# HengyiWang/spann3r

Measured on AMD Instinct MI355X. Metric: frames/sec/GPU (224px, 10-frame seq) + mem-bank cross-attn HBM GB/s, higher is better.
Workload: dtype bf16

## Files before the change

include/spann3r_hip.h:

```cpp
#ifndef SPANN3R_HIP_H
#define SPANN3R_HIP_H

#include <stdint.h>

#ifdef __cplusplus
extern "C" {
#endif

enum { SP3_F32 = 0, SP3_BF16 = 1 };
enum { SP3_ACT_NONE = 0, SP3_ACT_GELU = 1, SP3_ACT_RELU = 2 };
enum { SP3_EPI_PLAIN = 0, SP3_EPI_ROPE_VT = 1, SP3_EPI_PIXSHUF = 2, SP3_EPI_PARTIAL = 3 };
enum { SP3_LOAD_PLAIN = 0, SP3_LOAD_CONV3X3 = 1, SP3_LOAD_SOFTMAX = 2 };

const char* sp3_last_error(void);
int sp3_version(void);

typedef struct sp3_gemm_desc {
  const float* A;
  const float* A2;
  const void* W;
  void* C;
  const float* bias;
  const float* res1;
  const float* res2;
// ... 1 lines not shown
  int32_t batch;
  int32_t K1;
  int64_t lda, lda2, ldw, ldc, ldr1, ldr2;
  int64_t strideA, strideW, strideC;
  float alpha;
  int32_t wdtype;
  int32_t act;
  int32_t out_bf16;
  int32_t relu_in;
  int32_t loader;
  int32_t conv_H, conv_W, conv_C, conv_OH, conv_OW, conv_stride;
  int32_t epi;
  const float* rope_cos;
  const float* rope_sin;
  const int32_t* pos;
  int32_t rope_cols;
  void* vt;
  int32_t tokens;
  int32_t heads;
  int64_t vt_ld;
  int32_t ps_k, ps_H, ps_W, ps_C;
  int32_t tile;
  int32_t a_bf16;
  int32_t splitk;
  int32_t a_packed;
  const float* ln_stats;
  const float* ln_s;
  int32_t ln_nt;
  int32_t ln_C;
  float ln_eps;
  float* stats_out;
  void* c2;
  int32_t qkv_packed;
  int32_t out_packed;
  int32_t w_packed;
  int64_t sb_A2, sb_bias, sb_ln_stats, sb_ln_s, sb_stats_out, sb_c2, sb_vt;
  int64_t* trace;
  float* sm_stats_out;
  const float* sm_stats;
  int32_t sm_nt;
  float sm_thresh;
  float* sm_zout;
  int32_t f32x3;
  int32_t res_bf16;
  const int32_t* dyn_n;
  int32_t res2_up_H, res2_up_W;
} sp3_gemm_desc;
int sp3_gemm(const sp3_gemm_desc* desc_host, void* stream);
int sp3_gemm_n(const sp3_gemm_desc* const* descs, int n, void* stream);
int sp3_gemm_plan_n(const sp3_gemm_desc* const* descs, int n, int* tiles);
int sp3_gemm_plan(const sp3_gemm_desc* desc_host);

int sp3_layernorm(const float* x, int64_t ldx, const float* gamma, const float* beta, float eps,
                  void* out, int64_t ldo, int out_bf16, int rows, int C, void* stream);
int sp3_layernorm_packed(const float* x, int64_t ldx, const float* gamma, const float* beta, float eps,
                         void* out, int out_bf16, int rows, int C, void* stream);
int sp3_layernorm_dual(const float* x, int64_t ldx, const float* gamma, const float* beta, float eps, float* out, int64_t ldo,
                       void* out_packed_bf16, int rows, int C, int group_rows, int group_rows_pad, void* stream);
int sp3_layernorm_t(const float* x, int64_t ldx, const float* gamma, const float* beta, float eps,
                    void* out, int64_t ldo, int out_bf16, int rows, int C, void* stream);

typedef struct sp3_reduce_ln_desc {
  const float* partial;
  int64_t split_stride;
  const float* bias;
  const float* res;
  int64_t ldres;
  float* x_out;
  int64_t ldx;
  const float* g1; const float* b1; void* out1; int64_t ld1; int32_t out1_bf16;
  const float* g2; const float* b2; void* out2; int64_t ld2; int32_t out2_bf16;
  float eps;
  int32_t splits, rows, C;
  int32_t out1_packed, out2_packed;
  int32_t act;
  const float* res2;
  int64_t ldres2;
} sp3_reduce_ln_desc;
int sp3_reduce_ln(const sp3_reduce_ln_desc* desc_host, void* stream);

int sp3_rope_2d(void* tokens, int dtype, int B, int N, int H, int D, int64_t sB, int64_t sN, int64_t sH,
                const int64_t* positions, float base, float fwd, void* stream);

int sp3_attention(const void* q, int64_t sq, int64_t ldq, const void* k, int64_t sk, int64_t ldk,
                  const void* vt, int64_t vt_ld, void* out, int64_t ldo, int out_bf16,
                  int B, int heads, int Nq, int Nk, float scale, int dtype, void* stream);
int sp3_attention_ex(const void* q, int64_t sq, int64_t ldq, const void* k, int64_t sk, int64_t ldk,
                     const void* vt, int64_t vt_ld, void* out, int64_t ldo, int out_bf16, int out_packed,
                     int B, int heads, int Nq, int Nk, float scale, int dtype, void* stream);

int sp3_attention_packed(const void* qp, int q_cols, int q_col0, int npad_q, const void* kp, int k_cols, int k_col0, int npad_k,
                         const void* vtp, void* out, int64_t ldo, int out_bf16, int out_packed,
                         int B, int heads, int Nq, int Nk, float scale, int o_group, int o_group_rows, void* stream);

typedef struct sp3_attn_qproj_desc {
  const void* x_packed; int64_t x_group_stride;
  const float* ln_stats; int64_t stats_group_stride;
  const void* w_packed; int64_t w_group_stride;
  const float* ln_s; const float* bias; int64_t vec_group_stride;
  const int32_t* pos; const float* rope_cos; const float* rope_sin;
  float ln_eps; int32_t D;
  const void* kp; int32_t k_cols, k_col0, npad_k; const void* vtp;
  void* out; int64_t ldo; int32_t out_bf16, out_packed;
  int32_t B, heads, Nq, Nk; float scale; int32_t o_group, o_group_rows;
} sp3_attn_qproj_desc;
int sp3_attention_packed_qproj(const sp3_attn_qproj_desc* desc_host, void* stream);

typedef struct sp3_bank_write_desc {
  const float* feat_k;
  const float* feat_v;
  float* k_raw;
  float* v_raw;
  void* k_hat;
  void* v_hat_t;
  float* s_bank;
  float* b_bank;
  const float *gamma_k, *beta_k, *gamma_v, *beta_v, *gamma_q, *beta_q;
  float eps;
  float alpha;
  int32_t M, P, C, cap;
  int32_t wdtype;
  const int32_t* state;
} sp3_bank_write_desc;
int sp3_bank_write(const sp3_bank_write_desc* desc_host, void* stream);
int sp3_softmax_thresh(const float* S, float* P, int64_t ld, int64_t strideS, int rows, int M, int Mpad,
                       float thresh, int batch, void* P_packed, int64_t stride_packed, int packed_bf16, void* stream);
int sp3_softmax_pack(const float* S, int64_t ld, int64_t strideS, int rows, int M, float thresh, int batch, void* P_packed,
                     int64_t stride_packed, int packed_bf16, float* rowstat_ws, void* stream);
int sp3_colsum_accum(const float* P, int64_t ld, int rows, int M, float* mem_attn, void* stream);
int sp3_colsum_packed(const void* P_packed, int packed_bf16, int rows, int M, float* mem_attn, void* stream);
int sp3_colsum_softmax(const float* S, int64_t ld, int rows, int M, const float* rowz, float thresh, float* mem_attn,
                       float* mem_count, int append_P, void* stream);
int sp3_pack_stats(const float* x, int64_t ldx, int rows, int C, void* packed, int packed_bf16, float* stats, void* stream);
int sp3_gather_packed_rows(const void* src, void* dst, const int32_t* sel, int n_sel, int C, int elem_size, void* stream);
int sp3_gather_packed_cols(const void* src, void* dst, const int32_t* sel, int n_sel, int n_fill, int C, int cap,
                           int elem_size, void* stream);
int sp3_cos_sim(const float* k, const float* wm, int T, int P, int C, float* scratch, float* score, void* stream);
int sp3_bank_state_set(int32_t* state, int M, int wm, void* stream);
int sp3_prob_merge(const float* stats, float* scale, int rows, int M, int cap, const int32_t* dyn_n, void* stream);
int sp3_colsum_prob(const void* P_packed, const float* scale, int rows, int M, int cap, const int32_t* dyn_n, float* mem_attn, void* stream);
int sp3_cos_sim_state(const float* k, const float* k_raw, int Tmax, int P, int C, const int32_t* state, float* scratch, float* score,
                      void* stream);
int sp3_mem_append(float* count, float* attn, int M, int P, void* stream);
int sp3_prune_select(const float* attn, const float* count, int M, float protect, int top_k,
                     int32_t* sel, void* stream);
int sp3_gather_rows(const void* src, void* dst, const int32_t* sel, int n_sel, int C, int elem_size, void* stream);
int sp3_gather_cols(const void* src, int64_t ld_src, void* dst, int64_t ld_dst, const int32_t* sel, int n_sel,
                    int n_fill, int C, int elem_size, void* stream);
int sp3_gather_1d(const float* src, float* dst, const int32_t* sel, int n_sel, void* stream);

int sp3_conv3x3_tile(const void* x, int in_bf16, const void* w_packed, const float* bias, const float* res1,
                     const float* res2, void* out, int out_bf16, int B, int H, int W, int Cin, int Cout,
                     int relu_in, int act, void* stream);
int sp3_im2col_patch(const float* img, int64_t sb, int64_t sc, int64_t sy, int64_t sx, int B, int C, int H, int W,
                     int p, void* out, int out_bf16, int out_packed, void* stream);
int sp3_upsample2x(const float* in, float* out, int B, int H, int W, int C, int outH, int outW, void* stream);
int sp3_upsample2x_bf16(const void* in, void* out, int B, int H, int W, int C, int outH, int outW, void* stream);
int sp3_head_final(const float* feat, const float* w, const float* b, int64_t pixels, int C, float* pts,
                   float* conf, float* raw, void* stream);
int sp3_head_final_bf16(const void* feat, const float* w, const float* b, int64_t pixels, int C, float* pts, float* conf,
                        float* raw, void* stream);

int sp3_preprocess_image(const uint8_t* src, int64_t src_row_stride, int crop_l, int crop_t, int H1, int W1,
                         const int32_t* hbounds, const int32_t* hcoef, int hksize, int W2,
                         const int32_t* vbounds, const int32_t* vcoef, int vksize, int H2,
                         int crop2_l, int crop2_t, int outW, int outH, int transpose, uint8_t* tmp, float* out, void* stream);

int64_t sp3_conf_loss_ws_bytes(int n, int B);
int sp3_conf_loss_forward(const float* P, const float* Cf, const float* G, const uint8_t* V, const float* pose0, int n, int B, int HW,
                          float alpha, int fix_first, void* ws, float* out7, float* ent_out, void* stream);
int sp3_conf_loss_backward(const float* P, const float* Cf, const float* G, const uint8_t* V, const float* pose0, int n, int B, int HW,
                           float alpha, int fix_first, const void* ws, const float* grad_scale2, float* dP, float* dC, void* stream);
int64_t sp3_ssi_loss_ws_bytes(int n, int B, int HW);
int sp3_ssi_loss_forward(const float* P, const float* G, const uint8_t* V, const float* pose0, int n, int B, int HW, int fix_first,
                         int gt_scale, void* ws, float* out, void* stream);

int sp3_transpose(const float* src, int64_t ld_src, float* dst, int64_t ld_dst, int rows, int cols, void* stream);
int sp3_transpose_batched(const float* src, int64_t ld_src, int64_t stride_src, float* dst, int64_t ld_dst, int64_t stride_dst, int rows,
                          int cols, int batch, void* stream);
int sp3_transpose_pad(const float* src, int64_t ld_src, int64_t stride_src, float* dst, int64_t ld_dst, int64_t stride_dst, int rows,
                      int cols, int batch, int pad_to, void* stream);
int sp3_gelu(const float* x, float* y, int64_t n, void* stream);
int sp3_gelu_bwd(const float* x, const float* dy, float* dx, int64_t n, void* stream);
int sp3_im2col3x3(const float* x, float* col, int B, int H, int W, int C, int stride, void* stream);
int sp3_col2im3x3(const float* dcol, float* dx, int B, int H, int W, int C, int stride, void* stream);
int sp3_relu(const float* x, float* y, int64_t n, void* stream);
int sp3_relu_bwd(const float* x, const float* dy, float* dx, int64_t n, void* stream);
int sp3_upsample2x_bwd(const float* dy, float* dx, int B, int H, int W, int C, int outH, int outW, void* stream);
int sp3_postprocess(const float* raw, float* pts, float* conf, int64_t M, void* stream);
int sp3_postprocess_bwd(const float* raw, const float* dpts, const float* dconf, float* draw, int64_t M, void* stream);
int sp3_adamw(float* p, const float* g, float* m, float* v, int64_t n, float lr, float beta1, float beta2, float eps, float weight_decay,
              int step, float grad_scale, void* stream);
int sp3_mul(const float* a, const float* b, float* out, int64_t n, void* stream);
int sp3_pack_bf16(const float* src, int64_t ld, int rows, int cols, void* dst, void* dstT, void* stream);
int sp3_pack_bf16_conv3x3(const float* x, int B, int H, int W, int C, int stride, int act, void* dst, void* dstT, void* stream);
int sp3_pack_bf16_act(const float* src, int64_t ld, int rows, int cols, void* dst, void* dstT, int act, void* stream);
int sp3_pack_bf16_colsum(const float* src, int64_t ld, int rows, int cols, void* dst, void* dstT, float* colsum, int accumulate,
                         float* partial_ws, void* stream);
int64_t sp3_sumsq_blocks(int64_t n);
int64_t sp3_colsum_rows_ws(int rows, int N);
int sp3_colsum_rows(const float* x, int64_t ld, int rows, int N, float* out, int accumulate, float* scratch, void* stream);
int sp3_sumsq_partial(const float* g, int64_t n, double* partial, void* stream);
int sp3_clip_coef(const double* partial, int count, float max_norm, float extra_scale, float* out, int* step_counter, void* stream);
int sp3_adamw_flat(float* p, const float* g, float* m, float* v, int64_t n, const float* chunk_table, float lr, float beta1, float beta2,
                   float eps, int step, const float* grad_scale_dev, float grad_scale, const int* step_dev, const float* lr_dev, void* stream);
int sp3_softmax_bwd(const float* A, const float* dAd, const float* mask, float* dS, int64_t ld, int rows, int T, float alpha, void* stream);
int sp3_softmax_bwd_pad(const float* A, const float* dAd, const float* mask, float* dS, int64_t ld, int rows, int T, int Tpad, float alpha,
                        void* stream);
typedef struct sp3_head_part {
  const float* src;
  int64_t s_b, s_n, s_h;
  float* dst;
  int64_t d_b, d_n, d_h;
  float* dstT;
  const int64_t* pos;
  int32_t N;
  float fwd;
  int64_t ldT;
} sp3_head_part;
int sp3_head_shuffle(const sp3_head_part* parts, int nparts, int B, int H, int hd, float rope_base, const float* cos_tab,
                     const float* sin_tab, int tab_len, void* stream);
int sp3_attention_train_fwd(const float* q, int64_t sq, int64_t ldq, const float* k, int64_t sk, int64_t ldk, const float* vt, int64_t vt_ld,
                            float* out, int64_t ldo, float* lse, int B, int heads, int Nq, int Nk, float scale, int bf16_products, void* stream);
typedef struct sp3_attn_bwd_desc {
  const float *q, *k, *v, *dout;
  int64_t sq, ldq, sk, ldk, sv, ldv, sdo, lddo;
  const float *qT, *kT, *doT;
  int64_t ldTq, ldTk;
  const float* lse;
  float* D;
  float *dq, *dk, *dv;
  int64_t sdq, lddq, sdk, lddk, sdv, lddv;
  int32_t B, heads, Nq, Nk;
  float scale;
  int32_t bf16_products;
} sp3_attn_bwd_desc;
int sp3_attention_train_bwd(const sp3_attn_bwd_desc* d, void* stream);
int sp3_layernorm_bwd(const float* x, int64_t ldx, const float* gamma, const float* dy, int64_t ldy, const float* dx_add, int64_t ld_add,
                      float* dx, int64_t ld_dx, float* dgamma, float* dbeta, int accumulate, float* scratch, int rows, int C, float eps,
                      void* stream);

int sp3_focal_weiszfeld(const float* pts3d, int B, int H, int W, float ppx, float ppy, int iters, float focal_min, float focal_max,
                        float* focal, void* stream);
int sp3_conf_filter(const float* conf, const float* pts, const float* rgb, int64_t n, float thresh, int* scratch, int64_t* total,
                    float* out_pts, float* out_rgb, void* stream);

int sp3_pnp_dlt_accum(const float* pts, int F, int H, int W, float focal, float cx, float cy, const float* norm4, const float* Rt,
                      float thresh, int cv_mode, double* out41, void* stream);
int sp3_pnp_gn_accum(const float* pts, int F, int H, int W, float focal, float cx, float cy, const double* Rt, const float* Rt_mask,
                     float thresh, double* out29, void* stream);
int sp3_pnp_score(const float* pts, int F, int H, int W, float focal, float cx, float cy, const float* Rt, int n_hyp, float thresh,
                  int cv_mode, int* counts, void* stream);

int sp3_copy_multi(int n, const void* const* src, void* const* dst, const int64_t* bytes, void* stream);
int sp3_copy2d_f32(const float* src, int64_t lds, float* dst, int64_t ldd, int rows, int cols, void* stream);
int sp3_fill_f32(float* p, float v, int64_t n, void* stream);
int sp3_cast_f32_to_bf16(const float* src, void* dst, int64_t n, void* stream);
int sp3_spin(int64_t cycles, int64_t* ticks_100mhz, void* stream);

#ifdef __cplusplus
}
#endif
#endif
```

spann3r_amd/csrc/common.h:

```cpp
#pragma once
#include <hip/hip_runtime.h>
#include <stdint.h>
#include <stdio.h>
#include "../../include/spann3r_hip.h"

typedef __attribute__((ext_vector_type(8))) __bf16 bf16x8;
typedef __attribute__((ext_vector_type(4))) __bf16 bf16x4;
typedef __attribute__((ext_vector_type(2))) __bf16 bf16x2;
typedef __attribute__((ext_vector_type(4))) float f32x4;

#define SP3_WAVE 64

void sp3_set_error(const char* fmt, ...);

#define SP3_CHECK(cond, ...)                     \
  do {                                           \
    if (!(cond)) {                               \
      sp3_set_error(__VA_ARGS__);                \
      return 1;                                  \
    }                                            \
  } while (0)

#define SP3_LAUNCH_CHECK(what)                                              \
  do {                                                                      \
    hipError_t e_ = hipGetLastError();                                      \
    if (e_ != hipSuccess) {                                                 \
      sp3_set_error("%s: launch failed: %s", what, hipGetErrorString(e_));  \
      return 2;                                                             \
    }                                                                       \
  } while (0)

__device__ __forceinline__ float wave_sum(float v) {
#pragma unroll
  for (int o = 32; o > 0; o >>= 1) v += __shfl_xor(v, o);
  return v;
}
__device__ __forceinline__ float wave_max(float v) {
#pragma unroll
  for (int o = 32; o > 0; o >>= 1) v = fmaxf(v, __shfl_xor(v, o));
  return v;
}

__device__ __forceinline__ bf16x8 cvt8(const float4 a, const float4 b) {
  bf16x8 r;
  r[0] = (__bf16)a.x; r[1] = (__bf16)a.y; r[2] = (__bf16)a.z; r[3] = (__bf16)a.w;
  r[4] = (__bf16)b.x; r[5] = (__bf16)b.y; r[6] = (__bf16)b.z; r[7] = (__bf16)b.w;
  return r;
}

__device__ __forceinline__ float4 relu4(float4 v) {
  v.x = fmaxf(v.x, 0.f); v.y = fmaxf(v.y, 0.f); v.z = fmaxf(v.z, 0.f); v.w = fmaxf(v.w, 0.f);
  return v;
}

__device__ __forceinline__ float gelu_erf(float x) {
  const float a = fabsf(x);
  const float t = __builtin_amdgcn_rcpf(fmaf(0.2316419f, a, 1.0f));
  float p = fmaf(1.330274429f, t, -1.821255978f);
  p = fmaf(p, t, 1.781477937f);
  p = fmaf(p, t, -0.356563782f);
  p = fmaf(p, t, 0.319381530f);
  const float e = __builtin_amdgcn_exp2f(-0.72134752044448170368f * a * a);
  const float q = (p * t) * (e * 0.3989422804014327f);
  return fmaf(-a, q, fmaxf(x, 0.f));
}

#ifndef SP3_NO_WT_STORES
__device__ __forceinline__ void st_out(bf16x4* p, bf16x4 v) {
  __hip_atomic_store(reinterpret_cast<unsigned long long*>(p), __builtin_bit_cast(unsigned long long, v), __ATOMIC_RELAXED, __HIP_MEMORY_SCOPE_AGENT);
}
__device__ __forceinline__ void st_out(float2* p, float2 v) {
  __hip_atomic_store(reinterpret_cast<unsigned long long*>(p), __builtin_bit_cast(unsigned long long, v), __ATOMIC_RELAXED, __HIP_MEMORY_SCOPE_AGENT);
}
__device__ __forceinline__ void st_out(float4* p, float4 v) {
  const f32x4 t = {v.x, v.y, v.z, v.w};
  asm volatile("global_store_dwordx4 %0, %1, off sc1\n\ts_nop 1" ::"v"(p), "v"(t) : "memory");
}
__device__ __forceinline__ void st_out(bf16x8* p, bf16x8 v) {
  asm volatile("global_store_dwordx4 %0, %1, off sc1\n\ts_nop 1" ::"v"(p), "v"(v) : "memory");
}
#else
template <typename T> __device__ __forceinline__ void st_out(T* p, T v) { *p = v; }
#endif

struct Up2xTaps {
  int p00, p01, p10, p11;
  float hy, ly, hx, lx;
};
__device__ __forceinline__ Up2xTaps up2x_taps(int H, int W, int oy, int ox) {
  const int OH = 2 * H, OW = 2 * W;
  const float sh = OH > 1 ? (float)(H - 1) / (float)(OH - 1) : 0.f;
  const float sw = OW > 1 ? (float)(W - 1) / (float)(OW - 1) : 0.f;
  int y0 = (int)__fmul_rn(sh, (float)oy), x0 = (int)__fmul_rn(sw, (float)ox);
  y0 = y0 < H - 1 ? y0 : H - 1;
  x0 = x0 < W - 1 ? x0 : W - 1;
  const int y1 = y0 < H - 1 ? y0 + 1 : y0, x1 = x0 < W - 1 ? x0 + 1 : x0;
  Up2xTaps t;
  t.ly = __fmaf_rn(sh, (float)oy, -(float)y0); t.lx = __fmaf_rn(sw, (float)ox, -(float)x0);
  t.hy = 1.f - t.ly; t.hx = 1.f - t.lx;
  t.p00 = y0 * W + x0; t.p01 = y0 * W + x1; t.p10 = y1 * W + x0; t.p11 = y1 * W + x1;
  return t;
}
__device__ __forceinline__ float up2x_mix(const Up2xTaps& t, float v00, float v01, float v10, float v11) {
  const float top = __fmaf_rn(t.hx, v00, __fmul_rn(t.lx, v01)), bot = __fmaf_rn(t.hx, v10, __fmul_rn(t.lx, v11));
  return __fmaf_rn(t.hy, top, __fmul_rn(t.ly, bot));
}

__device__ __forceinline__ int64_t packed_off(int row, int k, int K, bool bf16) {
  const int lkb = bf16 ? 6 : 5, lch = bf16 ? 4 : 3;
  const int nkb = (K + (1 << lkb) - 1) >> lkb;
  const int kb = k >> lkb, kk = k & ((1 << lkb) - 1);
  const int g = kk >> lch, e = kk & ((1 << lch) - 1);
  const int h = e >> (lch - 1), eh = e & ((1 << (lch - 1)) - 1);
  return (((((int64_t)(row >> 4) * nkb + kb) * 2 + h) * 4 + g) * 16 + (row & 15)) * (1 << (lch - 1)) + eh;
}
```

spann3r_amd/csrc/conv.hip:

```cpp
#include "common.h"
#include <type_traits>
#include <cstdlib>

namespace {

constexpr int TH = 8, TW = 8;
constexpr int HP = (TH + 2) * (TW + 2);
constexpr int BM = TH * TW, BN = 64;
constexpr int MF = BM / 16, NF = BN / 16;
constexpr int SLAB_LD = BN + 4;
constexpr int DEPTH = 3;
constexpr int SP3_CONV_WIDE_MIN_WGS = 256;

struct ConvArgs {
  const void* x; const __bf16* w; const float* bias; const float* res1; const float* res2; void* out;
  int B, H, W, Cin, Cout, tiles_x, tiles_y, relu_in, act, out_bf16;
  int xcd_nb;
};

__device__ __forceinline__ bool conv_tile_of(const ConvArgs& a, int& t, int& nblk) {
  t = blockIdx.x; nblk = blockIdx.y;
  if (a.xcd_nb) {
    const unsigned L = blockIdx.x, xc = L & 7, jj = L >> 3, q = jj / (unsigned)a.xcd_nb;
    nblk = (int)(jj - q * a.xcd_nb);
    t = (int)(q * 8 + xc);
    if (t >= a.tiles_x * a.tiles_y * a.B) return false;
  }
  return true;
}

__device__ __forceinline__ bf16x8 ld_frag_lds(const char* p) { return *reinterpret_cast<const bf16x8*>(p); }

template <typename TIN>
__global__ __launch_bounds__(256) void conv3x3_tile_kernel(const ConvArgs a) {
  extern __shared__ __attribute__((aligned(16))) char lds[];
  const int tid = threadIdx.x, lane = tid & 63, wave = tid >> 6, g = lane >> 4, r = lane & 15;
  const int Cin = a.Cin;
  const int PS = Cin * 2 + 16;
  int t, nblk;
  if (!conv_tile_of(a, t, nblk)) return;
  const int tx = t % a.tiles_x; t /= a.tiles_x;
  const int ty = t % a.tiles_y;
  const int b = t / a.tiles_y;
  const int y0 = ty * TH, x0 = tx * TW, n0 = nblk * BN;

  const int upt = Cin >> 5;
  const int U = 9 * upt;
  const int nkb = (9 * Cin) >> 6;
  const __bf16* wb[NF];
#pragma unroll
  for (int n = 0; n < NF; ++n) wb[n] = a.w + ((int64_t)((n0 >> 4) + n) * nkb * 128 + lane) * 8;
  const int nu = (U - wave + 3) >> 2;
  auto w_off = [&](int i) -> int64_t {
    int u = wave + 4 * i;
    u = u < U ? u : U - 1;
    return (int64_t)(u >> 1) * (64 * 16) + (u & 1) * (64 * 8);
  };
  bf16x8 wq[DEPTH][NF];
#pragma unroll
  for (int s = 0; s < DEPTH; ++s) {
    const int64_t o = w_off(s);
#pragma unroll
    for (int n = 0; n < NF; ++n) wq[s][n] = *reinterpret_cast<const bf16x8*>(wb[n] + o);
  }

  {
    constexpr int CHK = 16 / (int)sizeof(TIN);
    const int cpp = Cin / CHK;
    const TIN* xin = reinterpret_cast<const TIN*>(a.x) + (int64_t)b * a.H * a.W * Cin;
    using Chunk = typename std::conditional<sizeof(TIN) == 4, float4, bf16x8>::type;
    auto src_of = [&](int p, int c, bool& ok) -> const Chunk* {
      const int hy = p / (TW + 2), hx = p - hy * (TW + 2);
      const int iy = y0 + hy - 1, ix = x0 + hx - 1;
      ok = p < HP && iy >= 0 && iy < a.H && ix >= 0 && ix < a.W;
      const int cy = ok ? iy : 0, cx = ok ? ix : 0;
      return reinterpret_cast<const Chunk*>(xin + ((int64_t)cy * a.W + cx) * Cin + c);
    };
    auto put = [&](int p, int c, Chunk v, bool ok) {
      char* dst = lds + p * PS + c * 2;
      if constexpr (sizeof(TIN) == 4) {
        if (!ok) v = make_float4(0.f, 0.f, 0.f, 0.f);
        if (a.relu_in) v = relu4(v);
        bf16x4 o;
        o[0] = (__bf16)v.x; o[1] = (__bf16)v.y; o[2] = (__bf16)v.z; o[3] = (__bf16)v.w;
        *reinterpret_cast<bf16x4*>(dst) = o;
      } else {
#pragma unroll
        for (int e = 0; e < 8; ++e) {
          const float f = (float)v[e];
          v[e] = (ok && (!a.relu_in || f > 0.f)) ? v[e] : (__bf16)0.f;
        }
        *reinterpret_cast<bf16x8*>(dst) = v;
      }
    };
    if ((256 % cpp) == 0) {
      const int c = (tid % cpp) * CHK, pstep = 256 / cpp;
      constexpr int NB = 13;
      for (int p0 = tid / cpp; p0 < HP; p0 += NB * pstep) {
        Chunk buf[NB];
        bool ok[NB];
#pragma unroll
        for (int q = 0; q < NB; ++q) buf[q] = *src_of(p0 + q * pstep, c, ok[q]);
#pragma unroll
        for (int q = 0; q < NB; ++q)
          if (p0 + q * pstep < HP) put(p0 + q * pstep, c, buf[q], ok[q]);
      }
    } else {
      for (int i = tid; i < HP * cpp; i += 256) {
        const int p = i / cpp, c = (i - p * cpp) * CHK;
        bool ok;
        const Chunk v = *src_of(p, c, ok);
        put(p, c, v, ok);
      }
    }
  }
  __syncthreads();

  f32x4 acc[MF][NF];
#pragma unroll
  for (int m = 0; m < MF; ++m)
#pragma unroll
    for (int n = 0; n < NF; ++n) acc[m][n] = f32x4{0.f, 0.f, 0.f, 0.f};
  int abase[MF];
#pragma unroll
  for (int m = 0; m < MF; ++m) {
    const int p = 16 * m + r;
    abase[m] = ((p / TW) * (TW + 2) + (p % TW)) * PS;
  }
  auto a_off = [&](int i) -> int {
    int u = wave + 4 * i;
    u = u < U ? u : U - 1;
    const int tap = u / upt, c32 = u - tap * upt;
    const int ky = tap / 3, kx = tap - 3 * ky;
    return (ky * (TW + 2) + kx) * PS + (((c32 >> 1) << 6) + 16 * g + ((c32 & 1) << 3)) * 2;
  };
  bf16x8 af[2][MF];
  {
    const int o = a_off(0);
#pragma unroll
    for (int m = 0; m < MF; ++m) af[0][m] = ld_frag_lds(lds + abase[m] + o);
  }
  for (int i0 = 0; i0 < nu; i0 += 2 * DEPTH) {
#pragma unroll
    for (int s2 = 0; s2 < 2 * DEPTH; ++s2) {
      const int i = i0 + s2;
      if (i < nu) {
        const int s = s2 % DEPTH, cur = s2 & 1;
        {
          const int o = a_off(i + 1);
#pragma unroll
          for (int m = 0; m < MF; ++m) af[cur ^ 1][m] = ld_frag_lds(lds + abase[m] + o);
        }
#pragma unroll
        for (int m = 0; m < MF; ++m)
#pragma unroll
          for (int n = 0; n < NF; ++n)
            acc[m][n] = __builtin_amdgcn_mfma_f32_16x16x32_bf16(af[cur][m], wq[s][n], acc[m][n], 0, 0, 0);
        {
          const int64_t o = w_off(i + DEPTH);
#pragma unroll
          for (int n = 0; n < NF; ++n) wq[s][n] = *reinterpret_cast<const bf16x8*>(wb[n] + o);
        }
      }
    }
  }
  __syncthreads();

  float* slab = reinterpret_cast<float*>(lds) + (size_t)wave * BM * SLAB_LD;
#pragma unroll
  for (int m = 0; m < MF; ++m)
#pragma unroll
    for (int n = 0; n < NF; ++n)
#pragma unroll
      for (int q = 0; q < 4; ++q) slab[(m * 16 + 4 * g + q) * SLAB_LD + n * 16 + r] = acc[m][n][q];
  __syncthreads();
  const float* sm = reinterpret_cast<const float*>(lds);
  for (int idx = tid; idx < BM * (BN / 4); idx += 256) {
    const int row = idx / (BN / 4), c4 = (idx % (BN / 4)) * 4;
    const int oy = y0 + row / TW, ox = x0 + row % TW;
    if (oy >= a.H || ox >= a.W) continue;
    float4 v = *reinterpret_cast<const float4*>(sm + row * SLAB_LD + c4);
#pragma unroll
    for (int s = 1; s < 4; ++s) {
      const float4 t4 = *reinterpret_cast<const float4*>(sm + (size_t)s * BM * SLAB_LD + row * SLAB_LD + c4);
      v.x += t4.x; v.y += t4.y; v.z += t4.z; v.w += t4.w;
    }
    const int gn = n0 + c4;
    if (a.bias) { const float4 b4 = *reinterpret_cast<const float4*>(a.bias + gn); v.x += b4.x; v.y += b4.y; v.z += b4.z; v.w += b4.w; }
    if (a.act == SP3_ACT_RELU) v = relu4(v);
    const int64_t off = (((int64_t)b * a.H + oy) * a.W + ox) * a.Cout + gn;
    if (a.out_bf16 & 2) {
      if (a.res1) { const bf16x4 q = *reinterpret_cast<const bf16x4*>(reinterpret_cast<const __bf16*>(a.res1) + off); v.x += (float)q[0]; v.y += (float)q[1]; v.z += (float)q[2]; v.w += (float)q[3]; }
      if (a.res2) { const bf16x4 q = *reinterpret_cast<const bf16x4*>(reinterpret_cast<const __bf16*>(a.res2) + off); v.x += (float)q[0]; v.y += (float)q[1]; v.z += (float)q[2]; v.w += (float)q[3]; }
    } else {
      if (a.res1) { const float4 q = *reinterpret_cast<const float4*>(a.res1 + off); v.x += q.x; v.y += q.y; v.z += q.z; v.w += q.w; }
      if (a.res2) { const float4 q = *reinterpret_cast<const float4*>(a.res2 + off); v.x += q.x; v.y += q.y; v.z += q.z; v.w += q.w; }
    }
    if (a.out_bf16 & 1) {
      bf16x4 o;
      o[0] = (__bf16)v.x; o[1] = (__bf16)v.y; o[2] = (__bf16)v.z; o[3] = (__bf16)v.w;
      st_out(reinterpret_cast<bf16x4*>(reinterpret_cast<__bf16*>(a.out) + off), o);
    } else {
      st_out(reinterpret_cast<float4*>(reinterpret_cast<float*>(a.out) + off), v);
    }
  }
}

namespace wide {
constexpr int TH = 8, TW = 16, HW = TW + 2, HP = (TH + 2) * HW;
constexpr int CH = 128, PS = CH * 2 + 16;
constexpr int MF = 8, DEPTH = 3;
constexpr int HALO_BYTES = HP * PS;
template <int NF> constexpr int lds_bytes() {
  return HALO_BYTES > 4 * 64 * (16 * NF + 4) * 4 ? HALO_BYTES : 4 * 64 * (16 * NF + 4) * 4;
}

template <typename TIN, int NF = 4, int ABL = 0>
__global__ __launch_bounds__(256, 2) void conv3x3_wide_kernel(const ConvArgs a) {
  constexpr int BN = 16 * NF, SLAB_LD = BN + 4;
  extern __shared__ __attribute__((aligned(16))) char lds[];
  const int tid = threadIdx.x, lane = tid & 63, wave = tid >> 6, g = lane >> 4, r = lane & 15;
  const int Cin = a.Cin;
  int t, nblk;
  if (!conv_tile_of(a, t, nblk)) return;
  const int tx = t % a.tiles_x; t /= a.tiles_x;
  const int ty = t % a.tiles_y;
  const int b = t / a.tiles_y;
  const int y0 = ty * TH, x0 = tx * TW, n0 = nblk * BN;
  const int nchunk = Cin / CH, upt = Cin >> 5;
  const int total = 9 * nchunk;

  typedef __attribute__((ext_vector_type(4))) uint32_t u32x4;
  const int nkb = (9 * Cin) >> 6;
  const uint32_t panel_bytes = (uint32_t)nkb * 128 * 8 * 2;
  const auto wrsrc = __builtin_amdgcn_make_buffer_rsrc(
      const_cast<char*>(reinterpret_cast<const char*>(a.w)) + (int64_t)(n0 >> 4) * panel_bytes, 0, (int)(NF * panel_bytes), 0x00020000);
  const uint32_t wlane = (uint32_t)lane * 16 + (uint32_t)(wave & 1) * 1024;
  const int wave_u = __builtin_amdgcn_readfirstlane(wave);
  auto w_off = [&](int seq) -> uint32_t {
    seq = seq < total ? seq : total - 1;
    const int c = seq / 9, tap = seq - 9 * c;
    return (uint32_t)((tap * upt + 4 * c + wave_u) >> 1) * 2048;
  };
  auto w_load = [&](int seq, bf16x8* dst) {
    const uint32_t o = w_off(seq);
#pragma unroll
    for (int n = 0; n < NF; ++n) {
      const u32x4 v = __builtin_amdgcn_raw_buffer_load_b128(wrsrc, wlane, o + n * panel_bytes, 0);
      dst[n] = *reinterpret_cast<const bf16x8*>(&v);
    }
  };
  bf16x8 wq[DEPTH][NF];
#pragma unroll
  for (int s = 0; s < DEPTH; ++s) w_load(s, wq[s]);

  f32x4 acc[MF][NF];
#pragma unroll
  for (int m = 0; m < MF; ++m)
#pragma unroll
    for (int n = 0; n < NF; ++n) acc[m][n] = f32x4{0.f, 0.f, 0.f, 0.f};
  const char* abase = lds + r * PS + (((wave >> 1) << 6) + 16 * g + ((wave & 1) << 3)) * 2;

  constexpr int CHK = 16 / (int)sizeof(TIN);
  constexpr int CPP = CH / CHK;
  constexpr int PSTEP = 256 / CPP, NB = sizeof(TIN) == 4 ? 6 : 12;
  const uint32_t img_bytes = (uint32_t)(a.H * a.W * Cin) * (uint32_t)sizeof(TIN);
  const auto rsrc = __builtin_amdgcn_make_buffer_rsrc(
      const_cast<char*>(reinterpret_cast<const char*>(a.x)) + (int64_t)b * img_bytes, 0, (int)img_bytes, 0x00020000);
  const uint32_t xlane = (uint32_t)((tid % CPP) * CHK * sizeof(TIN));
  char* hdst = lds + (tid % CPP) * CHK * 2;

  u32x4 buf[NB];
  auto issue = [&](int c, int p0) {
#pragma unroll
    for (int q = 0; q < NB; ++q) {
      const int p = p0 + q * PSTEP;
      const int hy = p / HW, hx = p - hy * HW;
      const int iy = y0 + hy - 1, ix = x0 + hx - 1;
      const bool ok = p < HP && iy >= 0 && iy < a.H && ix >= 0 && ix < a.W;
      const uint32_t off = ok ? (uint32_t)((iy * a.W + ix) * Cin + c * CH) * (uint32_t)sizeof(TIN) + xlane : 0x80000000u;
      if constexpr (ABL & 4) buf[q] = u32x4{0u, 0u, 0u, 0u};
      else buf[q] = __builtin_amdgcn_raw_buffer_load_b128(rsrc, off, 0, 0);
    }
  };
  auto commit = [&](int p0) {
#pragma unroll
    for (int q = 0; q < NB; ++q) {
      const int p = p0 + q * PSTEP;
      if (p >= HP) continue;
      char* dst = hdst + p * PS;
      if constexpr (sizeof(TIN) == 4) {
        float4 v = make_float4(__uint_as_float(buf[q][0]), __uint_as_float(buf[q][1]), __uint_as_float(buf[q][2]), __uint_as_float(buf[q][3]));
        if (a.relu_in) v = relu4(v);
        bf16x4 o;
        o[0] = (__bf16)v.x; o[1] = (__bf16)v.y; o[2] = (__bf16)v.z; o[3] = (__bf16)v.w;
        *reinterpret_cast<bf16x4*>(dst) = o;
      } else {
        u32x4 v = buf[q];
        if (a.relu_in) {
#pragma unroll
          for (int e = 0; e < 4; ++e) {
            const uint32_t neg = v[e] & 0x80008000u;
            v[e] &= ~((neg >> 15) * 0xffffu);
          }
        }
        *reinterpret_cast<u32x4*>(dst) = v;
      }
    }
  };
  for (int c = 0; c < nchunk; ++c) {
    if (c) __syncthreads();
    for (int p0 = tid / CPP; p0 < HP; p0 += NB * PSTEP) {
      issue(c, p0);
      commit(p0);
    }
    __syncthreads();

    bf16x8 af[MF];
#pragma unroll
    for (int m = 0; m < MF; ++m) af[m] = ld_frag_lds(abase + m * HW * PS);
#pragma unroll
    for (int tap = 0; tap < 9; ++tap) {
      const int s = tap % DEPTH;
      const int nt = tap + 1, nky = nt / 3, nkx = nt - 3 * nky;
#pragma unroll
      for (int m = 0; m < MF; ++m) {
#pragma unroll
        for (int n = 0; n < NF; ++n)
          acc[m][n] = __builtin_amdgcn_mfma_f32_16x16x32_bf16(af[m], wq[s][n], acc[m][n], 0, 0, 0);
        if constexpr (!(ABL & 2))
          if (tap < 8) af[m] = ld_frag_lds(abase + ((m + nky) * HW + nkx) * PS);
      }
      if constexpr (!(ABL & 1)) w_load(9 * c + tap + DEPTH, wq[s]);
    }
  }

  float* slab = reinterpret_cast<float*>(lds) + (size_t)wave * 64 * SLAB_LD;
  const float* sm = reinterpret_cast<const float*>(lds);
  if constexpr (ABL & 8) {
    float sum = 0.f;
#pragma unroll
    for (int m = 0; m < MF; ++m)
#pragma unroll
      for (int n = 0; n < NF; ++n) sum += acc[m][n][0] + acc[m][n][1] + acc[m][n][2] + acc[m][n][3];
    if (sum == 12345.678f) reinterpret_cast<float*>(a.out)[tid] = sum;
    return;
  }
#pragma unroll
  for (int h = 0; h < 2; ++h) {
    __syncthreads();
#pragma unroll
    for (int m = 0; m < 4; ++m)
#pragma unroll
      for (int n = 0; n < NF; ++n)
#pragma unroll
        for (int q = 0; q < 4; ++q) slab[(m * 16 + 4 * g + q) * SLAB_LD + n * 16 + r] = acc[4 * h + m][n][q];
    __syncthreads();
    for (int idx = tid; idx < 64 * (BN / 4); idx += 256) {
      const int row = idx / (BN / 4), c4 = (idx % (BN / 4)) * 4;
      const int oy = y0 + 4 * h + (row >> 4), ox = x0 + (row & 15);
      if (oy >= a.H || ox >= a.W) continue;
      float4 v = *reinterpret_cast<const float4*>(sm + row * SLAB_LD + c4);
#pragma unroll
      for (int s = 1; s < 4; ++s) {
        const float4 t4 = *reinterpret_cast<const float4*>(sm + (size_t)s * 64 * SLAB_LD + row * SLAB_LD + c4);
        v.x += t4.x; v.y += t4.y; v.z += t4.z; v.w += t4.w;
      }
      const int gn = n0 + c4;
      if (a.bias) { const float4 b4 = *reinterpret_cast<const float4*>(a.bias + gn); v.x += b4.x; v.y += b4.y; v.z += b4.z; v.w += b4.w; }
      if (a.act == SP3_ACT_RELU) v = relu4(v);
      const int64_t off = (((int64_t)b * a.H + oy) * a.W + ox) * a.Cout + gn;
      if (a.out_bf16 & 2) {
        if (a.res1) { const bf16x4 q = *reinterpret_cast<const bf16x4*>(reinterpret_cast<const __bf16*>(a.res1) + off); v.x += (float)q[0]; v.y += (float)q[1]; v.z += (float)q[2]; v.w += (float)q[3]; }
        if (a.res2) { const bf16x4 q = *reinterpret_cast<const bf16x4*>(reinterpret_cast<const __bf16*>(a.res2) + off); v.x += (float)q[0]; v.y += (float)q[1]; v.z += (float)q[2]; v.w += (float)q[3]; }
      } else {
        if (a.res1) { const float4 q = *reinterpret_cast<const float4*>(a.res1 + off); v.x += q.x; v.y += q.y; v.z += q.z; v.w += q.w; }
        if (a.res2) { const float4 q = *reinterpret_cast<const float4*>(a.res2 + off); v.x += q.x; v.y += q.y; v.z += q.z; v.w += q.w; }
      }
      if (a.out_bf16 & 1) {
        bf16x4 o;
        o[0] = (__bf16)v.x; o[1] = (__bf16)v.y; o[2] = (__bf16)v.z; o[3] = (__bf16)v.w;
        st_out(reinterpret_cast<bf16x4*>(reinterpret_cast<__bf16*>(a.out) + off), o);
      } else {
        st_out(reinterpret_cast<float4*>(reinterpret_cast<float*>(a.out) + off), v);
      }
    }
  }
}
}

}

extern "C" int sp3_conv3x3_tile(const void* x, int in_bf16, const void* w_packed, const float* bias, const float* res1,
                                const float* res2, void* out, int out_bf16, int B, int H, int W, int Cin, int Cout,
                                int relu_in, int act, void* stream) {
  SP3_CHECK(x && w_packed && out, "sp3_conv3x3_tile: null pointer");
  SP3_CHECK(B > 0 && H > 0 && W > 0, "sp3_conv3x3_tile: bad shape");
  SP3_CHECK(Cin % 64 == 0 && Cin >= 64 && Cout % 64 == 0 && Cout >= 64, "sp3_conv3x3_tile: Cin=%d / Cout=%d must be multiples of 64", Cin, Cout);
  SP3_CHECK(act == SP3_ACT_NONE || act == SP3_ACT_RELU, "sp3_conv3x3_tile: act %d", act);
  auto al16 = [](const void* q) { return (reinterpret_cast<uintptr_t>(q) & 15) == 0; };
  SP3_CHECK(al16(x) && al16(w_packed) && al16(bias) && al16(res1) && al16(res2) && al16(out), "sp3_conv3x3_tile: 16-byte alignment");
  ConvArgs a;
  a.x = x; a.w = reinterpret_cast<const __bf16*>(w_packed); a.bias = bias; a.res1 = res1; a.res2 = res2; a.out = out;
  a.B = B; a.H = H; a.W = W; a.Cin = Cin; a.Cout = Cout;
  a.relu_in = relu_in; a.act = act; a.out_bf16 = out_bf16 & 3;
  a.xcd_nb = 0;
  constexpr bool xcd_on = true;
  hipStream_t st = reinterpret_cast<hipStream_t>(stream);
  {
    const int want = (out_bf16 >> 2) & 3;
    const int wtx = (W + wide::TW - 1) / wide::TW, wty = (H + wide::TH - 1) / wide::TH;
    const int64_t wgs = (int64_t)wtx * wty * B * (Cout / 64);
    const bool can = Cin % wide::CH == 0;
    SP3_CHECK(want < 2 || can, "sp3_conv3x3_tile: the 8 x 16 tile needs Cin %% 128 == 0 (Cin=%d)", Cin);
    SP3_CHECK((int64_t)H * W * Cin * (in_bf16 ? 2 : 4) < (1ll << 31), "sp3_conv3x3_tile: one image of the map must stay below 2 GiB");
    const int nf = want == 2 ? 4 : want == 3 ? 2 : (want == 0 && can) ? (wgs >= SP3_CONV_WIDE_MIN_WGS ? 4 : wgs >= 80 ? 2 : 0) : 0;
    if (nf) {
      a.tiles_x = wtx; a.tiles_y = wty;
      dim3 grid(wtx * wty * B, Cout / (16 * nf));
      if (xcd_on) { a.xcd_nb = Cout / (16 * nf); grid = dim3((unsigned)(((wtx * wty * B + 7) / 8) * 8 * a.xcd_nb), 1); }
      auto launch = [&](auto kern, int lds_bytes) -> int {
        static bool raised = false;
        if (!raised && lds_bytes > 64 * 1024) {
          hipError_t e = hipFuncSetAttribute(reinterpret_cast<const void*>(kern), hipFuncAttributeMaxDynamicSharedMemorySize, lds_bytes);
          if (e != hipSuccess) { sp3_set_error("sp3_conv3x3_tile: cannot raise dynamic LDS to %d: %s", lds_bytes, hipGetErrorString(e)); return 2; }
          raised = true;
        }
        hipLaunchKernelGGL(kern, grid, dim3(256), lds_bytes, st, a);
        return 0;
      };
      int rc;
      if (nf == 4) rc = in_bf16 ? launch(wide::conv3x3_wide_kernel<__bf16, 4>, wide::lds_bytes<4>()) : launch(wide::conv3x3_wide_kernel<float, 4>, wide::lds_bytes<4>());
      else         rc = in_bf16 ? launch(wide::conv3x3_wide_kernel<__bf16, 2>, wide::lds_bytes<2>()) : launch(wide::conv3x3_wide_kernel<float, 2>, wide::lds_bytes<2>());
      if (rc) return rc;
      SP3_LAUNCH_CHECK("sp3_conv3x3_tile");
      return 0;
    }
  }
  a.tiles_x = (W + TW - 1) / TW; a.tiles_y = (H + TH - 1) / TH;
  const size_t halo = (size_t)HP * (Cin * 2 + 16), slabs = (size_t)4 * BM * SLAB_LD * sizeof(float);
  const size_t lds = halo > slabs ? halo : slabs;
  SP3_CHECK(lds <= 160 * 1024, "sp3_conv3x3_tile: Cin=%d needs %zu bytes of LDS", Cin, lds);
  dim3 grid(a.tiles_x * a.tiles_y * B, Cout / BN);
  if (xcd_on) { a.xcd_nb = Cout / BN; grid = dim3((unsigned)(((a.tiles_x * a.tiles_y * B + 7) / 8) * 8 * a.xcd_nb), 1); }
  auto launch = [&](auto kern) -> int {
    static size_t raised = 0;
    if (lds > 64 * 1024 && lds > raised) {
      raised = lds;
      hipError_t e = hipFuncSetAttribute(reinterpret_cast<const void*>(kern), hipFuncAttributeMaxDynamicSharedMemorySize, (int)lds);
      if (e != hipSuccess) { sp3_set_error("sp3_conv3x3_tile: cannot raise dynamic LDS to %zu: %s", lds, hipGetErrorString(e)); return 2; }
    }
    hipLaunchKernelGGL(kern, grid, dim3(256), lds, st, a);
    return 0;
  };
  const int rc = in_bf16 ? launch(conv3x3_tile_kernel<__bf16>) : launch(conv3x3_tile_kernel<float>);
  if (rc) return rc;
  SP3_LAUNCH_CHECK("sp3_conv3x3_tile");
  return 0;
}
```

spann3r_amd/csrc/dpt.hip:

```cpp
#include "common.h"
#include <math.h>

namespace {

__global__ __launch_bounds__(256) void im2col_patch_kernel(const float* __restrict__ img, int64_t sb, int64_t sc, int64_t sy,
                                                           int64_t sx, int C, int H, int W, int p, void* __restrict__ out,
                                                           int out_bf16, int out_packed, int64_t total) {
  const int64_t idx = (int64_t)blockIdx.x * 256 + threadIdx.x;
  if (idx >= total) return;
  const int K = C * p * p;
  const int64_t row = idx / K;
  const int k = (int)(idx - row * K);
  const int nw = W / p, nh = H / p;
  const int b = (int)(row / (nh * nw));
  const int rem = (int)(row - (int64_t)b * nh * nw);
  const int ty = rem / nw, tx = rem - ty * nw;
  const int c = k / (p * p), r2 = k - c * p * p;
  const int iy = r2 / p, ix = r2 - iy * p;
  const float val = img[b * sb + c * sc + (int64_t)(ty * p + iy) * sy + (int64_t)(tx * p + ix) * sx];
  const int64_t o = out_packed ? packed_off((int)row, k, K, out_bf16 != 0) : idx;
  if (out_bf16) reinterpret_cast<__bf16*>(out)[o] = (__bf16)val;
  else reinterpret_cast<float*>(out)[o] = val;
}

__device__ __forceinline__ float4 ld4(const float* p) { return *reinterpret_cast<const float4*>(p); }
__device__ __forceinline__ float4 ld4(const __bf16* p) {
  const bf16x4 t = *reinterpret_cast<const bf16x4*>(p);
  return make_float4((float)t[0], (float)t[1], (float)t[2], (float)t[3]);
}
__device__ __forceinline__ void st4(float* p, const float4 v) { st_out(reinterpret_cast<float4*>(p), v); }
__device__ __forceinline__ void st4(__bf16* p, const float4 v) {
  bf16x4 t;
  t[0] = (__bf16)v.x; t[1] = (__bf16)v.y; t[2] = (__bf16)v.z; t[3] = (__bf16)v.w;
  st_out(reinterpret_cast<bf16x4*>(p), t);
}

template <typename T>
__global__ __launch_bounds__(256) void upsample2x_kernel(const T* __restrict__ in, T* __restrict__ out, int H, int W,
                                                         int C, int outH, int outW, int64_t total4) {
  const int64_t idx = (int64_t)blockIdx.x * 256 + threadIdx.x;
  if (idx >= total4) return;
  const int c4 = C >> 2;
  const int cc = (int)(idx % c4);
  int64_t pix = idx / c4;
  const int ox = (int)(pix % outW);
  pix /= outW;
  const int oy = (int)(pix % outH);
  const int b = (int)(pix / outH);
  const int OH = 2 * H, OW = 2 * W;
  const float sh = OH > 1 ? (float)(H - 1) / (float)(OH - 1) : 0.f;
  const float sw = OW > 1 ? (float)(W - 1) / (float)(OW - 1) : 0.f;
  const float fy = sh * (float)oy, fx = sw * (float)ox;
  int y0 = (int)fy, x0 = (int)fx;
  y0 = y0 < H - 1 ? y0 : H - 1;
  x0 = x0 < W - 1 ? x0 : W - 1;
  const int y1 = y0 < H - 1 ? y0 + 1 : y0, x1 = x0 < W - 1 ? x0 + 1 : x0;
  const float ly = fy - (float)y0, lx = fx - (float)x0;
  const float hy = 1.f - ly, hx = 1.f - lx;
  const T* base = in + (int64_t)b * H * W * C;
  const float4 v00 = ld4(base + (((int64_t)y0 * W + x0) * c4 + cc) * 4);
  const float4 v01 = ld4(base + (((int64_t)y0 * W + x1) * c4 + cc) * 4);
  const float4 v10 = ld4(base + (((int64_t)y1 * W + x0) * c4 + cc) * 4);
  const float4 v11 = ld4(base + (((int64_t)y1 * W + x1) * c4 + cc) * 4);
  float4 o;
  o.x = hy * (hx * v00.x + lx * v01.x) + ly * (hx * v10.x + lx * v11.x);
  o.y = hy * (hx * v00.y + lx * v01.y) + ly * (hx * v10.y + lx * v11.y);
  o.z = hy * (hx * v00.z + lx * v01.z) + ly * (hx * v10.z + lx * v11.z);
  o.w = hy * (hx * v00.w + lx * v01.w) + ly * (hx * v10.w + lx * v11.w);
  st4(out + idx * 4, o);
}

__global__ __launch_bounds__(256) void upsample2x_bf16x8_kernel(const __bf16* __restrict__ in, __bf16* __restrict__ out, int H, int W,
                                                                int C, int outH, int outW) {
  const int c8 = C >> 3;
  const int t = blockIdx.x * 256 + threadIdx.x;
  if (t >= outW * c8) return;
  const int ox = t / c8, cg = t - ox * c8;
  const int oy = blockIdx.y, b = blockIdx.z;
  const int OH = 2 * H, OW = 2 * W;
  const float sh = OH > 1 ? (float)(H - 1) / (float)(OH - 1) : 0.f;
  const float sw = OW > 1 ? (float)(W - 1) / (float)(OW - 1) : 0.f;
  const float fy = sh * (float)oy, fx = sw * (float)ox;
  int y0 = (int)fy, x0 = (int)fx;
  y0 = y0 < H - 1 ? y0 : H - 1;
  x0 = x0 < W - 1 ? x0 : W - 1;
  const int y1 = y0 < H - 1 ? y0 + 1 : y0, x1 = x0 < W - 1 ? x0 + 1 : x0;
  const float ly = fy - (float)y0, lx = fx - (float)x0;
  const float hy = 1.f - ly, hx = 1.f - lx;
  const __bf16* base = in + (int64_t)b * H * W * C + cg * 8;
  const bf16x8 v00 = *reinterpret_cast<const bf16x8*>(base + ((int64_t)y0 * W + x0) * C);
  const bf16x8 v01 = *reinterpret_cast<const bf16x8*>(base + ((int64_t)y0 * W + x1) * C);
  const bf16x8 v10 = *reinterpret_cast<const bf16x8*>(base + ((int64_t)y1 * W + x0) * C);
  const bf16x8 v11 = *reinterpret_cast<const bf16x8*>(base + ((int64_t)y1 * W + x1) * C);
  bf16x8 o;
#pragma unroll
  for (int e = 0; e < 8; ++e)
    o[e] = (__bf16)(hy * (hx * (float)v00[e] + lx * (float)v01[e]) + ly * (hx * (float)v10[e] + lx * (float)v11[e]));
  st_out(reinterpret_cast<bf16x8*>(out + (((int64_t)b * outH + oy) * outW + ox) * C + cg * 8), o);
}

template <typename T>
__global__ __launch_bounds__(256) void head_final_kernel(const T* __restrict__ feat, const float* __restrict__ w,
                                                         const float* __restrict__ bias, int64_t pixels, int C,
                                                         float* __restrict__ pts, float* __restrict__ conf,
                                                         float* __restrict__ raw) {
  const int64_t gid = (int64_t)blockIdx.x * 256 + threadIdx.x;
  const int64_t pix = gid >> 3;
  const int sub = (int)(gid & 7);
  const bool valid = pix < pixels;
  const int64_t pp = valid ? pix : pixels - 1;
  float a0 = 0.f, a1 = 0.f, a2 = 0.f, a3 = 0.f;
  const T* f = feat + pp * C;
  for (int c = sub * 4; c < C; c += 32) {
    const float4 x = ld4(f + c);
    const float4 w0 = *reinterpret_cast<const float4*>(w + c);
    const float4 w1 = *reinterpret_cast<const float4*>(w + C + c);
    const float4 w2 = *reinterpret_cast<const float4*>(w + 2 * C + c);
    const float4 w3 = *reinterpret_cast<const float4*>(w + 3 * C + c);
    a0 += (x.x * w0.x + x.y * w0.y) + (x.z * w0.z + x.w * w0.w);
    a1 += (x.x * w1.x + x.y * w1.y) + (x.z * w1.z + x.w * w1.w);
    a2 += (x.x * w2.x + x.y * w2.y) + (x.z * w2.z + x.w * w2.w);
    a3 += (x.x * w3.x + x.y * w3.y) + (x.z * w3.z + x.w * w3.w);
  }
#pragma unroll
  for (int o = 1; o < 8; o <<= 1) {
    a0 += __shfl_xor(a0, o); a1 += __shfl_xor(a1, o); a2 += __shfl_xor(a2, o); a3 += __shfl_xor(a3, o);
  }
  if (valid && sub == 0) {
    const float x = a0 + bias[0], y = a1 + bias[1], z = a2 + bias[2], c = a3 + bias[3];
    if (raw) { raw[pix * 4 + 0] = x; raw[pix * 4 + 1] = y; raw[pix * 4 + 2] = z; raw[pix * 4 + 3] = c; }
    const float d = sqrtf(x * x + y * y + z * z);
    const float sc = expm1f(d) / fmaxf(d, 1e-8f);
    pts[pix * 3 + 0] = x * sc; pts[pix * 3 + 1] = y * sc; pts[pix * 3 + 2] = z * sc;
    conf[pix] = 1.0f + expf(c);
  }
}

template <int LP, int PPT>
__global__ __launch_bounds__(256) void head_final_bf16x8_kernel(const __bf16* __restrict__ feat, const float* __restrict__ w,
                                                                const float* __restrict__ bias, int64_t pixels, float* __restrict__ pts,
                                                                float* __restrict__ conf, float* __restrict__ raw) {
  constexpr int C = 8 * LP, PPB = 256 / LP;
  const int li = threadIdx.x % LP, pl = threadIdx.x / LP;
  float wr[4][8];
#pragma unroll
  for (int f = 0; f < 4; ++f) {
    const float4 a = *reinterpret_cast<const float4*>(w + f * C + li * 8), b = *reinterpret_cast<const float4*>(w + f * C + li * 8 + 4);
    wr[f][0] = a.x; wr[f][1] = a.y; wr[f][2] = a.z; wr[f][3] = a.w; wr[f][4] = b.x; wr[f][5] = b.y; wr[f][6] = b.z; wr[f][7] = b.w;
  }
  const float b0 = bias[0], b1 = bias[1], b2 = bias[2], b3 = bias[3];
  const int64_t p0 = (int64_t)blockIdx.x * PPB * PPT + pl;
  bf16x8 x[PPT];
#pragma unroll
  for (int q = 0; q < PPT; ++q) {
    int64_t pix = p0 + (int64_t)q * PPB;
    pix = pix < pixels ? pix : pixels - 1;
    x[q] = *reinterpret_cast<const bf16x8*>(feat + pix * C + li * 8);
  }
#pragma unroll
  for (int q = 0; q < PPT; ++q) {
    const int64_t pix = p0 + (int64_t)q * PPB;
    float a[4];
#pragma unroll
    for (int f = 0; f < 4; ++f) {
      float t0 = 0.f, t1 = 0.f;
#pragma unroll
      for (int e = 0; e < 4; ++e) { t0 = fmaf((float)x[q][e], wr[f][e], t0); t1 = fmaf((float)x[q][4 + e], wr[f][4 + e], t1); }
      a[f] = t0 + t1;
    }
#pragma unroll
    for (int o = 1; o < LP; o <<= 1) {
      a[0] += __shfl_xor(a[0], o); a[1] += __shfl_xor(a[1], o); a[2] += __shfl_xor(a[2], o); a[3] += __shfl_xor(a[3], o);
    }
    if (li == 0 && pix < pixels) {
      const float X = a[0] + b0, Y = a[1] + b1, Z = a[2] + b2, Cc = a[3] + b3;
      if (raw) *reinterpret_cast<float4*>(raw + pix * 4) = make_float4(X, Y, Z, Cc);
      const float d = sqrtf(X * X + Y * Y + Z * Z);
      const float sc = expm1f(d) / fmaxf(d, 1e-8f);
      pts[pix * 3 + 0] = X * sc; pts[pix * 3 + 1] = Y * sc; pts[pix * 3 + 2] = Z * sc;
      conf[pix] = 1.0f + expf(Cc);
    }
  }
}

}

#define ST(s) reinterpret_cast<hipStream_t>(s)

extern "C" int sp3_im2col_patch(const float* img, int64_t sb, int64_t sc, int64_t sy, int64_t sx, int B, int C, int H, int W,
                                int p, void* out, int out_bf16, int out_packed, void* stream) {
  SP3_CHECK(img && out && B > 0 && C > 0 && p > 0, "sp3_im2col_patch: bad arguments");
  SP3_CHECK(H % p == 0 && W % p == 0, "Input image size (%d,%d) is not a multiple of patch size (%d)", H, W, p);
  const int64_t total = (int64_t)B * (H / p) * (W / p) * C * p * p;
  hipLaunchKernelGGL(im2col_patch_kernel, dim3((unsigned)((total + 255) / 256)), dim3(256), 0, ST(stream), img, sb, sc, sy, sx,
                     C, H, W, p, out, out_bf16, out_packed, total);
  SP3_LAUNCH_CHECK("sp3_im2col_patch");
  return 0;
}

extern "C" int sp3_upsample2x(const float* in, float* out, int B, int H, int W, int C, int outH, int outW, void* stream) {
  SP3_CHECK(in && out && B > 0 && H > 0 && W > 0 && C > 0 && C % 4 == 0, "sp3_upsample2x: bad arguments");
  SP3_CHECK(outH > 0 && outH <= 2 * H && outW > 0 && outW <= 2 * W, "sp3_upsample2x: bad crop");
  const int64_t total4 = (int64_t)B * outH * outW * (C / 4);
  hipLaunchKernelGGL(upsample2x_kernel<float>, dim3((unsigned)((total4 + 255) / 256)), dim3(256), 0, ST(stream), in, out, H, W, C,
                     outH, outW, total4);
  SP3_LAUNCH_CHECK("sp3_upsample2x");
  return 0;
}

extern "C" int sp3_upsample2x_bf16(const void* in, void* out, int B, int H, int W, int C, int outH, int outW, void* stream) {
  SP3_CHECK(in && out && B > 0 && H > 0 && W > 0 && C > 0 && C % 4 == 0, "sp3_upsample2x_bf16: bad arguments");
  SP3_CHECK(outH > 0 && outH <= 2 * H && outW > 0 && outW <= 2 * W, "sp3_upsample2x_bf16: bad crop");
  if (C % 8 == 0 && outH <= 65535 && B <= 65535) {
    hipLaunchKernelGGL(upsample2x_bf16x8_kernel, dim3((unsigned)((outW * (C / 8) + 255) / 256), outH, B), dim3(256), 0, ST(stream),
                       reinterpret_cast<const __bf16*>(in), reinterpret_cast<__bf16*>(out), H, W, C, outH, outW);
    SP3_LAUNCH_CHECK("sp3_upsample2x_bf16");
    return 0;
  }
  const int64_t total4 = (int64_t)B * outH * outW * (C / 4);
  hipLaunchKernelGGL(upsample2x_kernel<__bf16>, dim3((unsigned)((total4 + 255) / 256)), dim3(256), 0, ST(stream),
                     reinterpret_cast<const __bf16*>(in), reinterpret_cast<__bf16*>(out), H, W, C, outH, outW, total4);
  SP3_LAUNCH_CHECK("sp3_upsample2x_bf16");
  return 0;
}

extern "C" int sp3_head_final(const float* feat, const float* w, const float* b, int64_t pixels, int C, float* pts, float* conf,
                              float* raw, void* stream) {
  SP3_CHECK(feat && w && b && pts && conf && pixels > 0 && C > 0 && C % 32 == 0, "sp3_head_final: bad arguments");
  const int64_t threads = pixels * 8;
  hipLaunchKernelGGL(head_final_kernel<float>, dim3((unsigned)((threads + 255) / 256)), dim3(256), 0, ST(stream), feat, w, b, pixels, C,
                     pts, conf, raw);
  SP3_LAUNCH_CHECK("sp3_head_final");
  return 0;
}

extern "C" int sp3_head_final_bf16(const void* feat, const float* w, const float* b, int64_t pixels, int C, float* pts, float* conf,
                                   float* raw, void* stream) {
  SP3_CHECK(feat && w && b && pts && conf && pixels > 0 && C > 0 && C % 32 == 0, "sp3_head_final_bf16: bad arguments");
  if (C == 128 && (reinterpret_cast<uintptr_t>(feat) & 15) == 0 && (reinterpret_cast<uintptr_t>(w) & 15) == 0 && (!raw || (reinterpret_cast<uintptr_t>(raw) & 15) == 0)) {
    constexpr int LP = 16, PPT = 4, PPB = 256 / LP;
    hipLaunchKernelGGL((head_final_bf16x8_kernel<LP, PPT>), dim3((unsigned)((pixels + PPB * PPT - 1) / (PPB * PPT))), dim3(256), 0, ST(stream),
                       reinterpret_cast<const __bf16*>(feat), w, b, pixels, pts, conf, raw);
    SP3_LAUNCH_CHECK("sp3_head_final_bf16");
    return 0;
  }
  const int64_t threads = pixels * 8;
  hipLaunchKernelGGL(head_final_kernel<__bf16>, dim3((unsigned)((threads + 255) / 256)), dim3(256), 0, ST(stream),
                     reinterpret_cast<const __bf16*>(feat), w, b, pixels, C, pts, conf, raw);
  SP3_LAUNCH_CHECK("sp3_head_final_bf16");
  return 0;
}
```

spann3r_amd/engine.py:

```python
import math
import os

import torch

from . import ops
from .lib import ACT_NONE, ACT_GELU, ACT_RELU
from .config import Spann3RConfig


def _rope_tables(max_pos, base, device):
    half = 32
    inv_freq = 1.0 / (base ** (torch.arange(0, half, 2).float() / half))
    t = torch.arange(max_pos, dtype=torch.float32)
    ang = torch.einsum("i,j->ij", t, inv_freq)
    return ang.cos().contiguous().to(device), ang.sin().contiguous().to(device)


def _rope_tables_narrow(max_pos, base, head_dim, device):
    D = head_dim // 2
    nf = D // 2
    assert nf <= 16 and head_dim % 4 == 0
    inv_freq = 1.0 / (base ** (torch.arange(0, D, 2).float() / D))
    t = torch.arange(max_pos, dtype=torch.float32)
    ang = torch.einsum("i,j->ij", t, inv_freq)
# ... 416 lines not shown
    def decoder_grouped(self, f1, f2, B, nh, nw, f1p=None, f2p=None):
        self.activate()
        cfg, w = self.cfg, self.w
        E, D, Hh = cfg.enc_dim, cfg.dec_dim, cfg.dec_heads
        P = nh * nw
        R = B * P
        npad = (P + 63) // 64 * 64
        nt = D // 32
        pos = self.positions(B, nh, nw)[1]
        depth = cfg.dec_depth
        es = 2 if self.adt == torch.bfloat16 else 4
        x = [self.ws("decg_x%d" % l, (2, R, D)) for l in range(depth + 1)]
        xp = [self.wspg("decg_xp%d" % j, R, D) for j in (0, 1)]
        st = [self.ws("decg_st%d" % j, (2, R, nt, 2)) for j in (0, 1)]
        xq, stq = self.wspg("decg_xq", R, D), self.ws("decg_stq", (2, R, nt, 2))
        ao, h = self.wspg("decg_ao", R, D), self.wspg("decg_h", R, D * cfg.mlp_ratio)
        qkp = self.ws("decg_qkp", ops.packed_shape(2 * B * npad, 2 * D, self.wdt), self.wdt, zero=True)
        vtp = self.ws("decg_vtp", (2 * B * Hh * npad * 64,), self.wdt, zero=True)
        cqp = self.ws("decg_cqp", ops.packed_shape(2 * B * npad, D, self.wdt), self.wdt, zero=True)
        ckp = self.ws("decg_ckp", ops.packed_shape(2 * B * npad, D, self.wdt), self.wdt, zero=True)
        cvtp = self.ws("decg_cvtp", (2 * B * Hh * npad * 64,), self.wdt, zero=True)
        sb_st, sb_vt = R * nt * 8, B * Hh * npad * 64 * 2
        Rp = xp[0].rows_pad
        if f1p is not None and f2p is not None:
            dA = f2p.data_ptr() - f1p.data_ptr()
            assert dA % 16 == 0
            ops.gemm(f1p, w["dec_embed.w"], x[0], M=R, N=D, K=E, lda=E, ldc=D, bias=w["dec_embed.b"], stats_out=st[0], c2=xp[0],
                     batch=2, strideA=dA // 2, strideC=R * D, sb={"stats_out": sb_st, "c2": xp[0].stride * es})
        else:
            dA = f2.data_ptr() - f1.data_ptr()
            assert dA % 16 == 0 and f1.dtype == f2.dtype == torch.float32
            ops.gemm(f1, w["dec_embed.w"], x[0], M=R, N=D, K=E, lda=E, ldc=D, bias=w["dec_embed.b"], stats_out=st[0], c2=xp[0],
                     batch=2, strideA=dA // 4, strideC=R * D, sb={"stats_out": sb_st, "c2": xp[0].stride * es})
        rope = dict(pos=pos, cos=self.cos, sin=self.sin, tokens=P, heads=Hh, qkv_packed=True, batch=2)
        for i in range(depth):
            cur, nx = i % 2, (i + 1) % 2
            g = "decg_%d." % i
            last = i == depth - 1
            xi, xo = x[i], x[i + 1]

            def upd(A, K, pre, res, stats, c2):
                sb = {"bias": D * 4}
                if stats is not None:
                    sb["stats_out"], sb["c2"] = sb_st, c2.stride * es
                ops.gemm(A, w[g + pre + ".w"], xo, M=R, N=D, K=K, lda=K, ldc=D, bias=w[g + pre + ".b"], res1=res, ldr1=D,
                         stats_out=stats, c2=c2, batch=2, strideA=A.stride, strideW=w[g + pre + ".w"].stride, strideC=R * D, sb=sb)

            with ops.pair():
                ops.proj_rope_vt(xp[cur], w[g + "qkv.w"], w[g + "qkv.b"], qkp, 0, vtp, npad, M=R, N=3 * D, K=D, lda=D, rope_cols=2 * D,
                                 ln=ops.LnFold(st[cur], D, w[g + "qkv.s"], 1e-6, sb_stats=sb_st, sb_s=3 * D * 4),
                                 strideA=xp[cur].stride, strideW=w[g + "qkv.w"].stride, strideC=B * npad * 2 * D,
                                 sb={"bias": 3 * D * 4, "vt": sb_vt}, **rope)
                ops.proj_rope_vt(xp[cur].at(1), w[g + "ckv.w"], w[g + "ckv.b"], ckp, 0, cvtp, npad, M=R, N=2 * D, K=D, lda=D, rope_cols=D,
                                 ln=ops.LnFold(st[cur][1], D, w[g + "ckv.s"], 1e-6, sb_stats=-sb_st, sb_s=2 * D * 4),
                                 strideA=-xp[cur].stride, strideW=w[g + "ckv.w"].stride, strideC=B * npad * D,
                                 sb={"bias": 2 * D * 4, "vt": sb_vt}, **rope)
            ops.attention_packed(qkp, 2 * D, 0, npad, qkp, 2 * D, D, npad, vtp, ao, D, B=2 * B, heads=Hh, Nq=P, Nk=P,
                                 scale=64 ** -0.5, o_group=B, o_group_rows=Rp)
            upd(ao, D, "proj", xi, stq, xq)
            if self.fuse_cross_q and P < 512 and D == 768 and ops.LEAN:
                ops.attention_packed_qproj(xq, stq, w[g + "cq.w"], w[g + "cq.s"], w[g + "cq.b"], pos, self.cos, self.sin, ckp, D, 0, npad, cvtp,
                                           ao, D, B=2 * B, heads=Hh, Nq=P, Nk=P, scale=64 ** -0.5, o_group=B, o_group_rows=Rp, eps=1e-6,
                                           stats_group_stride=sb_st // 4, vec_group_stride=D)
            else:
                ops.proj_rope_vt(xq, w[g + "cq.w"], w[g + "cq.b"], cqp, 0, None, npad, M=R, N=D, K=D, lda=D, rope_cols=D,
                                 ln=ops.LnFold(stq, D, w[g + "cq.s"], 1e-6, sb_stats=sb_st, sb_s=D * 4),
                                 strideA=xq.stride, strideW=w[g + "cq.w"].stride, strideC=B * npad * D, sb={"bias": D * 4}, **rope)
                ops.attention_packed(cqp, D, 0, npad, ckp, D, 0, npad, cvtp, ao, D, B=2 * B, heads=Hh, Nq=P, Nk=P,
                                     scale=64 ** -0.5, o_group=B, o_group_rows=Rp)
            upd(ao, D, "cproj", xo, stq, xq)
            Hd = D * cfg.mlp_ratio
            ops.gemm(xq, w[g + "fc1.w"], h, M=R, N=Hd, K=D, lda=D, ldc=Hd, bias=w[g + "fc1.b"], act=ACT_GELU,
                     ln=ops.LnFold(stq, D, w[g + "fc1.s"], 1e-6, sb_stats=sb_st, sb_s=Hd * 4),
                     batch=2, strideA=xq.stride, strideW=w[g + "fc1.w"].stride, strideC=h.stride, sb={"bias": Hd * 4})
            if last:
                upd(h, Hd, "fc2", xo, None, None)
            else:
                upd(h, Hd, "fc2", xo, st[nx], xp[nx])
        normed = self.ws("decg_normed", (2, R, D))
        ops.layernorm(x[depth], w["dec_norm.w"], w["dec_norm.b"], 1e-6, normed, rows=2 * R, C_=D,
                      dual=self.wspg("decg_normed_packed", R, D) if self.adt == torch.bfloat16 else None, group_rows=R)
        outs = {}
        for s_ in (0, 1):
            outs[s_] = [(f1, f2)[s_]] + [x[l][s_].view(B, P, D) for l in range(1, depth)] + [normed[s_].view(B, P, D)]
        return outs[0], outs[1]

    def key_aux(self, R):
        E = self.cfg.enc_dim
        return self.wspg("keyg_packed", R, E), self.ws("keyg_stats", (2, R, E // 32, 2))

    def encode_feat_keys_grouped(self, feat1, feat2, normed1, normed2, R, out1, out2, feat1p=None, feat2p=None):
        self.activate()
        cfg, w = self.cfg, self.w
        E, D, Kd = cfg.enc_dim, cfg.dec_dim, cfg.key_dim
        dF, dN, dO = feat2.data_ptr() - feat1.data_ptr(), normed2.data_ptr() - normed1.data_ptr(), out2.data_ptr() - out1.data_ptr()
        assert dF % 16 == 0 and dN % 16 == 0 and dO % 16 == 0
        es = 2 if self.adt == torch.bfloat16 else 4
        h = self.wspg("keyg_hidden", R, Kd)
        packed = None
        if feat1p is not None and feat2p is not None and self.adt == torch.bfloat16 and ops.LEAN:
            np_ = self.wspg("decg_normed_packed", R, D)
            dFp = feat2p.data_ptr() - feat1p.data_ptr()
            assert dFp % 16 == 0
            packed = dict(A2=np_, lda2=D, K1=E, batch=2, strideA=dFp // 2, strideW=w["keyg.0.w"].stride, strideC=h.stride,
                          sb={"bias": Kd * 4, "A2": np_.stride * 2})
            ok = self._splitA_plan.get(R)
            if ok is None:
                ok = self._splitA_plan[R] = ops.gemm(feat1p, w["keyg.0.w"], h, M=R, N=Kd, K=Kd, lda=E, ldc=Kd, bias=w["keyg.0.b"],
                                                     act=ACT_GELU, plan_only=True, **packed) >= 30
            if not ok:
                packed = None
        if packed is not None:
            ops.gemm(feat1p, w["keyg.0.w"], h, M=R, N=Kd, K=Kd, lda=E, ldc=Kd, bias=w["keyg.0.b"], act=ACT_GELU, **packed)
        else:
            ops.gemm(feat1, w["keyg.0.w"], h, M=R, N=Kd, K=Kd, lda=E, ldc=Kd, bias=w["keyg.0.b"], act=ACT_GELU, A2=normed1, lda2=D, K1=E,
                     batch=2, strideA=dF // 4, strideW=w["keyg.0.w"].stride, strideC=h.stride, sb={"bias": Kd * 4, "A2": dN})
        kp, kst = self.key_aux(R)
        ops.gemm(h, w["keyg.2.w"], out1, M=R, N=E, K=Kd, lda=Kd, ldc=E, bias=w["keyg.2.b"], stats_out=kst, c2=kp,
                 batch=2, strideA=h.stride, strideW=w["keyg.2.w"].stride, strideC=dO // 4,
                 sb={"bias": E * 4, "stats_out": R * (E // 32) * 8, "c2": kp.stride * es})
        return kp.at(1), kst[1]

    def encode_feat_key(self, feat, dec_last, R, num, out, aux=False):
        self.activate()
        cfg, w = self.cfg, self.w
        E, D, Kd = cfg.enc_dim, cfg.dec_dim, cfg.key_dim
        h = self.wsp("key_hidden%d" % num, R, Kd)
        pre = "key%d." % num
        ops.gemm(feat, w[pre + "0.w"], h, M=R, N=Kd, K=Kd, lda=E, ldc=Kd, bias=w[pre + "0.b"], act=ACT_GELU,
                 A2=dec_last, lda2=D, K1=E)
        if aux:
            kp, kst = self.key_aux(R)
            ops.gemm(h, w[pre + "2.w"], out, M=R, N=E, K=Kd, lda=Kd, ldc=E, bias=w[pre + "2.b"], stats_out=kst[num - 1],
                     c2=kp.at(num - 1))
            return kp.at(num - 1), kst[num - 1]
        ops.gemm(h, w[pre + "2.w"], out, M=R, N=E, K=Kd, lda=Kd, ldc=E, bias=w[pre + "2.b"])
        return out

    def _conv_ws(self, head):
        return self.ws("conv_splitk_ws" + str(head), (1 << 23,))

    def _rcu_c1(self, x, pre, B, H, W_, tag=""):
        w, F = self.w, self.cfg.dpt_feat
        t = self.ws("rcu_tmp" + tag, (B * H * W_, F), self.mdt)
        ops.conv3x3(x, w[pre + "c1.w"], t, B=B, H=H, W_=W_, Cin=F, Cout=F, bias=w[pre + "c1.b"], relu_in=True, act=ACT_RELU,
                    splitk_ws=self._conv_ws(tag[:1]))
        return t

    def _rcu(self, x, pre, B, H, W_, out, extra_res=None, tag="", c1_done=False, extra_up=None):
        w, F = self.w, self.cfg.dpt_feat
        t = self.ws("rcu_tmp" + tag, (B * H * W_, F), self.mdt)
        if not c1_done:
            self._rcu_c1(x, pre, B, H, W_, tag)
        ops.conv3x3(t, w[pre + "c2.w"], out, B=B, H=H, W_=W_, Cin=F, Cout=F, bias=w[pre + "c2.b"], res1=x, res2=extra_res,
                    splitk_ws=self._conv_ws(tag[:1]), res2_up=extra_up)
        return out

    def _fusion(self, pre, B, H, W_, x0, x1, tag, crop=None, c1_done=False, x0_up=None, fold_up=False):
        w, F = self.w, self.cfg.dpt_feat
        M = B * H * W_
        cur = x0
        if x1 is not None:
            s = self.ws("fus_sum_" + tag, (M, F), self.mdt)
            self._rcu(x1, pre + "u1", B, H, W_, s, extra_res=x0, tag=tag, c1_done=c1_done, extra_up=x0_up)
            cur = s
        r = self.ws("fus_rcu2_" + tag, (M, F), self.mdt)
        self._rcu(cur, pre + "u2", B, H, W_, r, tag=tag, c1_done=c1_done and x1 is None)
        oc = self.ws("fus_oc_" + tag, (M, F), self.mdt)
        ops.gemm(r, w[pre + "out.w"], oc, M=M, N=F, K=F, lda=F, ldc=F, bias=w[pre + "out.b"])
        OH, OW = (2 * H, 2 * W_) if crop is None else crop
        if fold_up:
            return oc, OH, OW
        up = self.ws("fus_up_" + tag, (B * OH * OW, F), self.mdt)
        ops.upsample2x(oc, up, B=B, H=H, W_=W_, C_=F, outH=OH, outW=OW)
        return up, OH, OW

    def dpt_head(self, dec, B, nh, nw, num, want_raw=False):
        self.activate()
        cfg, w = self.cfg, self.w
        F, Lc = cfg.dpt_feat, cfg.dpt_last
        pre = "dpt%d." % num
        R = B * nh * nw
        hk = cfg.hooks
        dims = (cfg.enc_dim, cfg.dec_dim, cfg.dec_dim, cfg.dec_dim)
        ld = (96, 192, 384, 768)
        mdt = self.mdt
        t = [self.ws("dpt%d_pp%d" % (num, i), (R, ld[i]), mdt) for i in range(4)]
        import contextlib
        lv = ops.HEAD_LEVELS
        group = ops.level if len({dec[hk[i]].dtype for i in range(4)}) == 1 else contextlib.nullcontext
        with (group if lv else contextlib.nullcontext)():
            for i0 in (0, 2):
                with (contextlib.nullcontext if lv else group)():
                    for i in (i0, i0 + 1):
                        ops.gemm(dec[hk[i]], w[pre + "pp%d.w" % i], t[i], M=R, N=ld[i], K=dims[i], lda=dims[i], ldc=ld[i], bias=w[pre + "pp%d.b" % i])
        c0 = 128 if self.wdt == torch.bfloat16 else ld[0]
        l0 = self.ws("dpt%d_l0" % num, (B * 16 * nh * nw, c0), mdt)
        l1 = self.ws("dpt%d_l1" % num, (B * 4 * nh * nw, ld[1]), mdt)
        with group():
            ops.conv_transpose_ks(t[0], w[pre + "pp0t.w"], l0, B=B, H=nh, W_=nw, Cin=ld[0], Cout=c0, ks=4, bias=w[pre + "pp0t.b"])
            ops.conv_transpose_ks(t[1], w[pre + "pp1t.w"], l1, B=B, H=nh, W_=nw, Cin=ld[1], Cout=ld[1], ks=2, bias=w[pre + "pp1t.b"])
        l2 = t[2]
        h3, w3 = (nh - 1) // 2 + 1, (nw - 1) // 2 + 1
        l3 = self.ws("dpt%d_l3" % num, (B * h3 * w3, ld[3]), mdt)
        sk = self._conv_ws(num)
        geo = ((4 * nh, 4 * nw), (2 * nh, 2 * nw), (nh, nw), (h3, w3))
        srcs = (l0, l1, l2, l3)
        rn = [self.ws("dpt%d_rn%d" % (num, i), (B * geo[i][0] * geo[i][1], F), mdt) for i in range(4)]

        def layer_rn(i):
            ops.conv3x3(srcs[i], w[pre + "rn%d.w" % i], rn[i], B=B, H=geo[i][0], W_=geo[i][1], Cin=(c0 if i == 0 else ld[i]), Cout=F, splitk_ws=sk)

        def pp3c():
            ops.conv3x3(t[3], w[pre + "pp3c.w"], l3, B=B, H=nh, W_=nw, Cin=ld[3], Cout=ld[3], stride=2, bias=w[pre + "pp3c.b"], splitk_ws=sk)

        refs = [(pre + "ref%d." % (4 - j), "%d_%d" % (num, 4 - j)) for j in range(4)]
        if lv:
            with ops.level():
                pp3c()
                layer_rn(2)
            with ops.level():
                layer_rn(0)
                layer_rn(1)
                layer_rn(3)
                self._rcu_c1(rn[2], refs[1][0] + "u1", B, geo[2][0], geo[2][1], refs[1][1])
            with ops.level():
                self._rcu_c1(rn[3], refs[0][0] + "u2", B, geo[3][0], geo[3][1], refs[0][1])
                self._rcu_c1(rn[1], refs[2][0] + "u1", B, geo[1][0], geo[1][1], refs[2][1])
                self._rcu_c1(rn[0], refs[3][0] + "u1", B, geo[0][0], geo[0][1], refs[3][1])
        else:
            pp3c()
            for i in range(4):
                layer_rn(i)
        path, up, Hc, Wc = rn[3], None, h3, w3
        for j in range(4):
            Hn, Wn = geo[3 - j]
            fold = lv and j < 3 and ops.conv3x3_takes_res2_up(w[refs[j + 1][0] + "u1c2.w"], mdt, B, *geo[2 - j])
            nxt, OH_, OW_ = self._fusion(refs[j][0], B, Hn, Wn, path, rn[3 - j] if j else None, refs[j][1], crop=(nh, nw) if j == 0 else None,
                                         c1_done=lv, x0_up=up, fold_up=fold)
            path, up = nxt, ((Hn, Wn) if fold else None)
        p1, H1, W1 = path, OH_, OW_
        a = self.ws("dpt%d_h0" % num, (B * H1 * W1, Lc), mdt)
        ops.conv3x3(p1, w[pre + "h0.w"], a, B=B, H=H1, W_=W1, Cin=F, Cout=Lc, bias=w[pre + "h0.b"])
        OH, OW = 2 * H1, 2 * W1
        u = self.ws("dpt%d_h0up" % num, (B * OH * OW, Lc), mdt)
        ops.upsample2x(a, u, B=B, H=H1, W_=W1, C_=Lc)
        c = self.ws("dpt%d_h2" % num, (B * OH * OW, Lc), mdt)
        ops.conv3x3(u, w[pre + "h2.w"], c, B=B, H=OH, W_=OW, Cin=Lc, Cout=Lc, bias=w[pre + "h2.b"], act=ACT_RELU)
        pts = self.ws("dpt_pts%d" % num, (B, OH, OW, 3))
        conf = self.ws("dpt_conf%d" % num, (B, OH, OW))
        raw = self.ws("dpt_raw%d" % num, (B, OH, OW, 4)) if want_raw else None
        ops.head_final(c, w[pre + "h4.w"], w[pre + "h4.b"], B * OH * OW, Lc, pts, conf, raw)
        return pts, conf, raw

    def encode_cur_value_feat(self, tok, out, res, pos32=None):
        self.activate()
        cfg, w = self.cfg, self.w
        B, P, Cv = tok.shape
        assert Cv == cfg.val_dim
        R, E = B * P, cfg.enc_dim
        zero_pos = self.ws("valf_zero_pos", (R, 2), torch.int32, zero=True)
        rope_tab = None
        if cfg.mem_pos_enc:
            assert pos32 is not None and self.rope_narrow is not None
            zero_pos, rope_tab = pos32, self.rope_narrow
        x = self.ws("valf_x", (R, Cv))
        xpA, xpB = self.wsp("valf_xpA", R, Cv), self.wsp("valf_xpB", R, Cv)
        stA, stB = self.stats("valf_stA", R, Cv), self.stats("valf_stB", R, Cv)
        ops.copy2d(tok.reshape(R, Cv), Cv, x, Cv, R, Cv)
        ops.pack_stats(x, xpA, stA, rows=R, C_=Cv)
        for i in range(cfg.val_depth):
            self._block(x, xpA, stA, xpB, stB, R, B, P, Cv, cfg.enc_heads, "val%d." % i, zero_pos, tag="_valf",
                        head_dim=Cv // cfg.enc_heads, rope_tab=rope_tab)
        ops.gemm(xpA, w["value_out.w"], out, M=R, N=E, K=Cv, lda=Cv, ldc=E, bias=w["value_out.b"], res1=res, ldr1=E,
                 ln=ops.LnFold(stA, Cv, w["value_out.s"], 1e-6))
        return out

    def encode_cur_value(self, pts3d, out, res):
        self.activate()
        cfg, w = self.cfg, self.w
        B, H, W_, _ = pts3d.shape
        p, E = cfg.patch, cfg.enc_dim
        nh, nw = H // p, W_ // p
        P = nh * nw
        R = B * P
        _, pos32, zero_pos = self.positions(B, nh, nw)
        col = self.wsp("im2col_val", R, 3 * p * p)
        sb, sy, sx, sc = pts3d.stride()
        ops.im2col_patch(pts3d, col, B=B, C_=3, H=H, W_=W_, p=p, strides=(sb, sc, sy, sx))
        x, xp, st = self._vit(col, R, B, P, "pospatch", "val", cfg.val_depth, pos32 if cfg.mem_pos_enc else zero_pos, tag="_val")
        ops.gemm(xp, w["value_out.w"], out, M=R, N=E, K=E, lda=E, ldc=E, bias=w["value_out.b"], res1=res, ldr1=E,
                 ln=ops.LnFold(st, E, w["value_out.s"], 1e-6))
        return out
```

spann3r_amd/lib.py:

```python
import ctypes as C
import os

import torch

_HERE = os.path.dirname(os.path.abspath(__file__))
LIB_PATH = os.environ.get("SP3_LIB_PATH") or os.path.join(_HERE, "libspann3r_hip.so")

F32, BF16 = 0, 1
ACT_NONE, ACT_GELU, ACT_RELU = 0, 1, 2
EPI_PLAIN, EPI_ROPE_VT, EPI_PIXSHUF, EPI_PARTIAL = 0, 1, 2, 3
LOAD_PLAIN, LOAD_CONV3X3, LOAD_SOFTMAX = 0, 1, 2


class GemmDesc(C.Structure):
    _fields_ = [
        ("A", C.c_void_p), ("A2", C.c_void_p), ("W", C.c_void_p), ("C", C.c_void_p), ("bias", C.c_void_p),
        ("res1", C.c_void_p), ("res2", C.c_void_p),
        ("M", C.c_int32), ("N", C.c_int32), ("K", C.c_int32), ("batch", C.c_int32),
        ("K1", C.c_int32),
        ("lda", C.c_int64), ("lda2", C.c_int64), ("ldw", C.c_int64), ("ldc", C.c_int64),
        ("ldr1", C.c_int64), ("ldr2", C.c_int64),
        ("strideA", C.c_int64), ("strideW", C.c_int64), ("strideC", C.c_int64),
        ("alpha", C.c_float), ("wdtype", C.c_int32), ("act", C.c_int32), ("out_bf16", C.c_int32),
        ("relu_in", C.c_int32), ("loader", C.c_int32),
        ("conv_H", C.c_int32), ("conv_W", C.c_int32), ("conv_C", C.c_int32),
        ("conv_OH", C.c_int32), ("conv_OW", C.c_int32), ("conv_stride", C.c_int32),
        ("epi", C.c_int32),
        ("rope_cos", C.c_void_p), ("rope_sin", C.c_void_p), ("pos", C.c_void_p),
        ("rope_cols", C.c_int32), ("vt", C.c_void_p), ("tokens", C.c_int32), ("heads", C.c_int32),
        ("vt_ld", C.c_int64),
        ("ps_k", C.c_int32), ("ps_H", C.c_int32), ("ps_W", C.c_int32), ("ps_C", C.c_int32),
        ("tile", C.c_int32), ("a_bf16", C.c_int32), ("splitk", C.c_int32), ("a_packed", C.c_int32),
        ("ln_stats", C.c_void_p), ("ln_s", C.c_void_p), ("ln_nt", C.c_int32), ("ln_C", C.c_int32), ("ln_eps", C.c_float),
        ("stats_out", C.c_void_p), ("c2", C.c_void_p), ("qkv_packed", C.c_int32), ("out_packed", C.c_int32), ("w_packed", C.c_int32),
        ("sb_A2", C.c_int64), ("sb_bias", C.c_int64), ("sb_ln_stats", C.c_int64), ("sb_ln_s", C.c_int64),
        ("sb_stats_out", C.c_int64), ("sb_c2", C.c_int64), ("sb_vt", C.c_int64),
        ("trace", C.c_void_p),
        ("sm_stats_out", C.c_void_p), ("sm_stats", C.c_void_p), ("sm_nt", C.c_int32), ("sm_thresh", C.c_float), ("sm_zout", C.c_void_p),
        ("f32x3", C.c_int32), ("res_bf16", C.c_int32), ("dyn_n", C.c_void_p),
        ("res2_up_H", C.c_int32), ("res2_up_W", C.c_int32),
    ]


class HeadPart(C.Structure):
    _fields_ = [
        ("src", C.c_void_p), ("s_b", C.c_int64), ("s_n", C.c_int64), ("s_h", C.c_int64),
        ("dst", C.c_void_p), ("d_b", C.c_int64), ("d_n", C.c_int64), ("d_h", C.c_int64),
        ("dstT", C.c_void_p), ("pos", C.c_void_p), ("N", C.c_int32), ("fwd", C.c_float), ("ldT", C.c_int64),
    ]


class AttnBwdDesc(C.Structure):
    _fields_ = ([(n, C.c_void_p) for n in ("q", "k", "v", "dout")]
                + [(n, C.c_int64) for n in ("sq", "ldq", "sk", "ldk", "sv", "ldv", "sdo", "lddo")]
                + [(n, C.c_void_p) for n in ("qT", "kT", "doT")] + [("ldTq", C.c_int64), ("ldTk", C.c_int64)]
                + [("lse", C.c_void_p), ("D", C.c_void_p), ("dq", C.c_void_p), ("dk", C.c_void_p), ("dv", C.c_void_p)]
                + [(n, C.c_int64) for n in ("sdq", "lddq", "sdk", "lddk", "sdv", "lddv")]
                + [("B", C.c_int32), ("heads", C.c_int32), ("Nq", C.c_int32), ("Nk", C.c_int32), ("scale", C.c_float), ("bf16_products", C.c_int32)])


class AttnQProjDesc(C.Structure):
    _fields_ = [
        ("x_packed", C.c_void_p), ("x_group_stride", C.c_int64), ("ln_stats", C.c_void_p), ("stats_group_stride", C.c_int64),
        ("w_packed", C.c_void_p), ("w_group_stride", C.c_int64), ("ln_s", C.c_void_p), ("bias", C.c_void_p), ("vec_group_stride", C.c_int64),
        ("pos", C.c_void_p), ("rope_cos", C.c_void_p), ("rope_sin", C.c_void_p), ("ln_eps", C.c_float), ("D", C.c_int32),
        ("kp", C.c_void_p), ("k_cols", C.c_int32), ("k_col0", C.c_int32), ("npad_k", C.c_int32), ("vtp", C.c_void_p),
        ("out", C.c_void_p), ("ldo", C.c_int64), ("out_bf16", C.c_int32), ("out_packed", C.c_int32),
        ("B", C.c_int32), ("heads", C.c_int32), ("Nq", C.c_int32), ("Nk", C.c_int32), ("scale", C.c_float),
        ("o_group", C.c_int32), ("o_group_rows", C.c_int32),
    ]


class ReduceLnDesc(C.Structure):
    _fields_ = [
        ("partial", C.c_void_p), ("split_stride", C.c_int64), ("bias", C.c_void_p), ("res", C.c_void_p),
        ("ldres", C.c_int64), ("x_out", C.c_void_p), ("ldx", C.c_int64),
        ("g1", C.c_void_p), ("b1", C.c_void_p), ("out1", C.c_void_p), ("ld1", C.c_int64), ("out1_bf16", C.c_int32),
        ("g2", C.c_void_p), ("b2", C.c_void_p), ("out2", C.c_void_p), ("ld2", C.c_int64), ("out2_bf16", C.c_int32),
        ("eps", C.c_float), ("splits", C.c_int32), ("rows", C.c_int32), ("C", C.c_int32),
        ("out1_packed", C.c_int32), ("out2_packed", C.c_int32),
            ("act", C.c_int32), ("res2", C.c_void_p), ("ldres2", C.c_int64),
    ]


class BankWriteDesc(C.Structure):
    _fields_ = [
        ("feat_k", C.c_void_p), ("feat_v", C.c_void_p), ("k_raw", C.c_void_p), ("v_raw", C.c_void_p),
        ("k_hat", C.c_void_p), ("v_hat_t", C.c_void_p), ("s_bank", C.c_void_p), ("b_bank", C.c_void_p),
        ("gamma_k", C.c_void_p), ("beta_k", C.c_void_p), ("gamma_v", C.c_void_p), ("beta_v", C.c_void_p),
        ("gamma_q", C.c_void_p), ("beta_q", C.c_void_p),
        ("eps", C.c_float), ("alpha", C.c_float),
        ("M", C.c_int32), ("P", C.c_int32), ("C", C.c_int32), ("cap", C.c_int32), ("wdtype", C.c_int32), ("state", C.c_void_p),
    ]


_lib = None

_PROTOS = {
    "sp3_gemm": [C.POINTER(GemmDesc), C.c_void_p],
    "sp3_gemm_n": [C.POINTER(C.POINTER(GemmDesc)), C.c_int, C.c_void_p],
    "sp3_gemm_plan_n": [C.POINTER(C.POINTER(GemmDesc)), C.c_int, C.POINTER(C.c_int)],
    "sp3_gemm_plan": [C.POINTER(GemmDesc)],
    "sp3_layernorm": [C.c_void_p, C.c_int64, C.c_void_p, C.c_void_p, C.c_float, C.c_void_p, C.c_int64, C.c_int,
                      C.c_int, C.c_int, C.c_void_p],
    "sp3_reduce_ln": [C.POINTER(ReduceLnDesc), C.c_void_p],
    "sp3_layernorm_dual": [C.c_void_p, C.c_int64, C.c_void_p, C.c_void_p, C.c_float, C.c_void_p, C.c_int64, C.c_void_p, C.c_int, C.c_int,
                           C.c_int, C.c_int, C.c_void_p],
    "sp3_layernorm_packed": [C.c_void_p, C.c_int64, C.c_void_p, C.c_void_p, C.c_float, C.c_void_p, C.c_int,
                             C.c_int, C.c_int, C.c_void_p],
    "sp3_attention_ex": [C.c_void_p, C.c_int64, C.c_int64, C.c_void_p, C.c_int64, C.c_int64, C.c_void_p, C.c_int64,
                         C.c_void_p, C.c_int64, C.c_int, C.c_int, C.c_int, C.c_int, C.c_int, C.c_int, C.c_float, C.c_int,
                         C.c_void_p],
    "sp3_layernorm_t": [C.c_void_p, C.c_int64, C.c_void_p, C.c_void_p, C.c_float, C.c_void_p, C.c_int64, C.c_int,
                        C.c_int, C.c_int, C.c_void_p],
    "sp3_rope_2d": [C.c_void_p, C.c_int, C.c_int, C.c_int, C.c_int, C.c_int, C.c_int64, C.c_int64, C.c_int64,
                    C.c_void_p, C.c_float, C.c_float, C.c_void_p],
    "sp3_attention": [C.c_void_p, C.c_int64, C.c_int64, C.c_void_p, C.c_int64, C.c_int64, C.c_void_p, C.c_int64,
                      C.c_void_p, C.c_int64, C.c_int, C.c_int, C.c_int, C.c_int, C.c_int, C.c_float, C.c_int, C.c_void_p],
    "sp3_attention_packed": [C.c_void_p, C.c_int, C.c_int, C.c_int, C.c_void_p, C.c_int, C.c_int, C.c_int, C.c_void_p,
                             C.c_void_p, C.c_int64, C.c_int, C.c_int, C.c_int, C.c_int, C.c_int, C.c_int, C.c_float, C.c_int, C.c_int,
                             C.c_void_p],
    "sp3_attention_packed_qproj": [C.POINTER(AttnQProjDesc), C.c_void_p],
    "sp3_softmax_thresh": [C.c_void_p, C.c_void_p, C.c_int64, C.c_int64, C.c_int, C.c_int, C.c_int, C.c_float,
                           C.c_int, C.c_void_p, C.c_int64, C.c_int, C.c_void_p],
    "sp3_softmax_pack": [C.c_void_p, C.c_int64, C.c_int64, C.c_int, C.c_int, C.c_float, C.c_int, C.c_void_p, C.c_int64, C.c_int, C.c_void_p,
                         C.c_void_p],
    "sp3_colsum_packed": [C.c_void_p, C.c_int, C.c_int, C.c_int, C.c_void_p, C.c_void_p],
    "sp3_colsum_softmax": [C.c_void_p, C.c_int64, C.c_int, C.c_int, C.c_void_p, C.c_float, C.c_void_p, C.c_void_p, C.c_int, C.c_void_p],
    "sp3_bank_write": [C.POINTER(BankWriteDesc), C.c_void_p],
    "sp3_pack_stats": [C.c_void_p, C.c_int64, C.c_int, C.c_int, C.c_void_p, C.c_int, C.c_void_p, C.c_void_p],
    "sp3_gather_packed_rows": [C.c_void_p, C.c_void_p, C.c_void_p, C.c_int, C.c_int, C.c_int, C.c_void_p],
    "sp3_gather_packed_cols": [C.c_void_p, C.c_void_p, C.c_void_p, C.c_int, C.c_int, C.c_int, C.c_int, C.c_int, C.c_void_p],
    "sp3_colsum_accum": [C.c_void_p, C.c_int64, C.c_int, C.c_int, C.c_void_p, C.c_void_p],
    "sp3_cos_sim": [C.c_void_p, C.c_void_p, C.c_int, C.c_int, C.c_int, C.c_void_p, C.c_void_p, C.c_void_p],
    "sp3_mem_append": [C.c_void_p, C.c_void_p, C.c_int, C.c_int, C.c_void_p],
    "sp3_bank_state_set": [C.c_void_p, C.c_int, C.c_int, C.c_void_p],
    "sp3_prob_merge": [C.c_void_p, C.c_void_p, C.c_int, C.c_int, C.c_int, C.c_void_p, C.c_void_p],
    "sp3_colsum_prob": [C.c_void_p, C.c_void_p, C.c_int, C.c_int, C.c_int, C.c_void_p, C.c_void_p, C.c_void_p],
    "sp3_cos_sim_state": [C.c_void_p, C.c_void_p, C.c_int, C.c_int, C.c_int, C.c_void_p, C.c_void_p, C.c_void_p, C.c_void_p],
    "sp3_prune_select": [C.c_void_p, C.c_void_p, C.c_int, C.c_float, C.c_int, C.c_void_p, C.c_void_p],
    "sp3_gather_rows": [C.c_void_p, C.c_void_p, C.c_void_p, C.c_int, C.c_int, C.c_int, C.c_void_p],
    "sp3_gather_cols": [C.c_void_p, C.c_int64, C.c_void_p, C.c_int64, C.c_void_p, C.c_int, C.c_int, C.c_int,
                        C.c_int, C.c_void_p],
    "sp3_gather_1d": [C.c_void_p, C.c_void_p, C.c_void_p, C.c_int, C.c_void_p],
    "sp3_im2col_patch": [C.c_void_p, C.c_int64, C.c_int64, C.c_int64, C.c_int64, C.c_int, C.c_int, C.c_int, C.c_int,
                         C.c_int, C.c_void_p, C.c_int, C.c_int, C.c_void_p],
    "sp3_conv3x3_tile": [C.c_void_p, C.c_int, C.c_void_p, C.c_void_p, C.c_void_p, C.c_void_p, C.c_void_p, C.c_int, C.c_int, C.c_int,
                         C.c_int, C.c_int, C.c_int, C.c_int, C.c_int, C.c_void_p],
    "sp3_upsample2x": [C.c_void_p, C.c_void_p, C.c_int, C.c_int, C.c_int, C.c_int, C.c_int, C.c_int, C.c_void_p],
    "sp3_head_final": [C.c_void_p, C.c_void_p, C.c_void_p, C.c_int64, C.c_int, C.c_void_p, C.c_void_p, C.c_void_p,
                       C.c_void_p],
    "sp3_upsample2x_bf16": [C.c_void_p, C.c_void_p, C.c_int, C.c_int, C.c_int, C.c_int, C.c_int, C.c_int, C.c_void_p],
    "sp3_head_final_bf16": [C.c_void_p, C.c_void_p, C.c_void_p, C.c_int64, C.c_int, C.c_void_p, C.c_void_p, C.c_void_p,
                            C.c_void_p],
    "sp3_fill_f32": [C.c_void_p, C.c_float, C.c_int64, C.c_void_p],
    "sp3_cast_f32_to_bf16": [C.c_void_p, C.c_void_p, C.c_int64, C.c_void_p],
    "sp3_copy2d_f32": [C.c_void_p, C.c_int64, C.c_void_p, C.c_int64, C.c_int, C.c_int, C.c_void_p],
    "sp3_spin": [C.c_int64, C.c_void_p, C.c_void_p],
    "sp3_conf_loss_forward": [C.c_void_p, C.c_void_p, C.c_void_p, C.c_void_p, C.c_void_p, C.c_int, C.c_int, C.c_int, C.c_float, C.c_int,
                              C.c_void_p, C.c_void_p, C.c_void_p, C.c_void_p],
    "sp3_conf_loss_backward": [C.c_void_p, C.c_void_p, C.c_void_p, C.c_void_p, C.c_void_p, C.c_int, C.c_int, C.c_int, C.c_float, C.c_int,
                               C.c_void_p, C.c_void_p, C.c_void_p, C.c_void_p, C.c_void_p],
    "sp3_transpose": [C.c_void_p, C.c_int64, C.c_void_p, C.c_int64, C.c_int, C.c_int, C.c_void_p],
    "sp3_transpose_batched": [C.c_void_p, C.c_int64, C.c_int64, C.c_void_p, C.c_int64, C.c_int64, C.c_int, C.c_int, C.c_int, C.c_void_p],
    "sp3_transpose_pad": [C.c_void_p, C.c_int64, C.c_int64, C.c_void_p, C.c_int64, C.c_int64, C.c_int, C.c_int, C.c_int, C.c_int, C.c_void_p],
    "sp3_softmax_bwd_pad": [C.c_void_p, C.c_void_p, C.c_void_p, C.c_void_p, C.c_int64, C.c_int, C.c_int, C.c_int, C.c_float, C.c_void_p],
    "sp3_head_shuffle": [C.c_void_p, C.c_int, C.c_int, C.c_int, C.c_int, C.c_float, C.c_void_p, C.c_void_p, C.c_int, C.c_void_p],
    "sp3_attention_train_fwd": [C.c_void_p, C.c_int64, C.c_int64, C.c_void_p, C.c_int64, C.c_int64, C.c_void_p, C.c_int64, C.c_void_p, C.c_int64,
                                C.c_void_p, C.c_int, C.c_int, C.c_int, C.c_int, C.c_float, C.c_int, C.c_void_p],
    "sp3_attention_train_bwd": [C.c_void_p, C.c_void_p],
    "sp3_gelu": [C.c_void_p, C.c_void_p, C.c_int64, C.c_void_p],
    "sp3_gelu_bwd": [C.c_void_p, C.c_void_p, C.c_void_p, C.c_int64, C.c_void_p],
    "sp3_im2col3x3": [C.c_void_p, C.c_void_p, C.c_int, C.c_int, C.c_int, C.c_int, C.c_int, C.c_void_p],
    "sp3_col2im3x3": [C.c_void_p, C.c_void_p, C.c_int, C.c_int, C.c_int, C.c_int, C.c_int, C.c_void_p],
    "sp3_relu": [C.c_void_p, C.c_void_p, C.c_int64, C.c_void_p],
    "sp3_relu_bwd": [C.c_void_p, C.c_void_p, C.c_void_p, C.c_int64, C.c_void_p],
    "sp3_upsample2x_bwd": [C.c_void_p, C.c_void_p, C.c_int, C.c_int, C.c_int, C.c_int, C.c_int, C.c_int, C.c_void_p],
    "sp3_postprocess": [C.c_void_p, C.c_void_p, C.c_void_p, C.c_int64, C.c_void_p],
    "sp3_postprocess_bwd": [C.c_void_p, C.c_void_p, C.c_void_p, C.c_void_p, C.c_int64, C.c_void_p],
    "sp3_adamw": [C.c_void_p, C.c_void_p, C.c_void_p, C.c_void_p, C.c_int64, C.c_float, C.c_float, C.c_float, C.c_float, C.c_float, C.c_int,
                  C.c_float, C.c_void_p],
    "sp3_mul": [C.c_void_p, C.c_void_p, C.c_void_p, C.c_int64, C.c_void_p],
    "sp3_pack_bf16": [C.c_void_p, C.c_int64, C.c_int, C.c_int, C.c_void_p, C.c_void_p, C.c_void_p],
    "sp3_pack_bf16_conv3x3": [C.c_void_p, C.c_int, C.c_int, C.c_int, C.c_int, C.c_int, C.c_int, C.c_void_p, C.c_void_p, C.c_void_p],
    "sp3_pack_bf16_act": [C.c_void_p, C.c_int64, C.c_int, C.c_int, C.c_void_p, C.c_void_p, C.c_int, C.c_void_p],
    "sp3_pack_bf16_colsum": [C.c_void_p, C.c_int64, C.c_int, C.c_int, C.c_void_p, C.c_void_p, C.c_void_p, C.c_int, C.c_void_p, C.c_void_p],
    "sp3_colsum_rows": [C.c_void_p, C.c_int64, C.c_int, C.c_int, C.c_void_p, C.c_int, C.c_void_p, C.c_void_p],
    "sp3_sumsq_partial": [C.c_void_p, C.c_int64, C.c_void_p, C.c_void_p],
    "sp3_clip_coef": [C.c_void_p, C.c_int, C.c_float, C.c_float, C.c_void_p, C.c_void_p, C.c_void_p],
    "sp3_adamw_flat": [C.c_void_p, C.c_void_p, C.c_void_p, C.c_void_p, C.c_int64, C.c_void_p, C.c_float, C.c_float, C.c_float, C.c_float,
                       C.c_int, C.c_void_p, C.c_float, C.c_void_p, C.c_void_p, C.c_void_p],
    "sp3_softmax_bwd": [C.c_void_p, C.c_void_p, C.c_void_p, C.c_void_p, C.c_int64, C.c_int, C.c_int, C.c_float, C.c_void_p],
    "sp3_layernorm_bwd": [C.c_void_p, C.c_int64, C.c_void_p, C.c_void_p, C.c_int64, C.c_void_p, C.c_int64, C.c_void_p, C.c_int64,
                          C.c_void_p, C.c_void_p, C.c_int, C.c_void_p, C.c_int, C.c_int, C.c_float, C.c_void_p],
    "sp3_focal_weiszfeld": [C.c_void_p, C.c_int, C.c_int, C.c_int, C.c_float, C.c_float, C.c_int, C.c_float, C.c_float, C.c_void_p, C.c_void_p],
    "sp3_conf_filter": [C.c_void_p, C.c_void_p, C.c_void_p, C.c_int64, C.c_float, C.c_void_p, C.c_void_p, C.c_void_p, C.c_void_p, C.c_void_p],
    "sp3_copy_multi": [C.c_int, C.c_void_p, C.c_void_p, C.c_void_p, C.c_void_p],
    "sp3_pnp_dlt_accum": [C.c_void_p, C.c_int, C.c_int, C.c_int, C.c_float, C.c_float, C.c_float, C.c_void_p, C.c_void_p, C.c_float, C.c_int,
                          C.c_void_p, C.c_void_p],
    "sp3_pnp_gn_accum": [C.c_void_p, C.c_int, C.c_int, C.c_int, C.c_float, C.c_float, C.c_float, C.c_void_p, C.c_void_p, C.c_float, C.c_void_p, C.c_void_p],
    "sp3_pnp_score": [C.c_void_p, C.c_int, C.c_int, C.c_int, C.c_float, C.c_float, C.c_float, C.c_void_p, C.c_int, C.c_float, C.c_int, C.c_void_p, C.c_void_p],
    "sp3_ssi_loss_forward": [C.c_void_p, C.c_void_p, C.c_void_p, C.c_void_p, C.c_int, C.c_int, C.c_int, C.c_int, C.c_int, C.c_void_p, C.c_void_p,
                             C.c_void_p],
    "sp3_preprocess_image": [C.c_void_p, C.c_int64, C.c_int, C.c_int, C.c_int, C.c_int, C.c_void_p, C.c_void_p, C.c_int, C.c_int,
                             C.c_void_p, C.c_void_p, C.c_int, C.c_int, C.c_int, C.c_int, C.c_int, C.c_int, C.c_int, C.c_void_p,
                             C.c_void_p, C.c_void_p],
}
EXPORTS = sorted(list(_PROTOS) + ["sp3_last_error", "sp3_version", "sp3_conf_loss_ws_bytes", "sp3_ssi_loss_ws_bytes", "sp3_sumsq_blocks", "sp3_colsum_rows_ws"])


def load():
    global _lib
    if _lib is not None:
        return _lib
    if not os.path.exists(LIB_PATH):
        raise RuntimeError("libspann3r_hip.so not built: run `python -c 'import __graft_entry__ as g; g.build()'` "
                           "(there is no CPU fallback for the hot path)")
    lib = C.CDLL(LIB_PATH)
    lib.sp3_last_error.restype = C.c_char_p
    lib.sp3_last_error.argtypes = []
    lib.sp3_version.restype = C.c_int
    lib.sp3_conf_loss_ws_bytes.restype = C.c_int64
    lib.sp3_conf_loss_ws_bytes.argtypes = [C.c_int, C.c_int]
    lib.sp3_ssi_loss_ws_bytes.restype = C.c_int64
    lib.sp3_ssi_loss_ws_bytes.argtypes = [C.c_int, C.c_int, C.c_int]
    lib.sp3_sumsq_blocks.restype = C.c_int64
    lib.sp3_sumsq_blocks.argtypes = [C.c_int64]
    lib.sp3_colsum_rows_ws.restype = C.c_int64
    lib.sp3_colsum_rows_ws.argtypes = [C.c_int, C.c_int]
    for name, argtypes in _PROTOS.items():
        fn = getattr(lib, name)
        fn.restype = C.c_int
        fn.argtypes = argtypes
    _lib = lib
    return lib


def check(rc, what):
    if rc != 0:
        msg = load().sp3_last_error().decode(errors="replace")
        raise RuntimeError("%s failed (%d): %s" % (what, rc, msg))


_raw_stream = getattr(torch._C, "_cuda_getCurrentRawStream", None)
_raw_device = getattr(torch._C, "_cuda_getDevice", None)


def stream_ptr():
    if _raw_stream is not None and _raw_device is not None:
        return _raw_stream(_raw_device())
    return torch.cuda.current_stream().cuda_stream


def ptr(t):
    return 0 if t is None else t.data_ptr()
```

spann3r_amd/model.py:

```python
import argparse
import collections
import os
import weakref

import torch
import torch.nn as nn

from . import ops
from .config import Spann3RConfig, FULL
from .engine import Engine
from .weights import param_spec, alias_of, synth_state_dict


def _build_param_tree(root: nn.Module, spec):
    made = {}
    for key, shape in spec.items():
        parts = key.split(".")
        mod = root
        for name in parts[:-1]:
            if not hasattr(mod, name) or not isinstance(getattr(mod, name), nn.Module):
                mod.add_module(name, nn.Module())
            mod = getattr(mod, name)
        src = alias_of(key)
        if src is not None:
# ... 557 lines not shown
            for j, t in enumerate(self.seq_dec2):
                dec[hk[j + 1]] = t[c0 * B * P:c1 * B * P]
            key = ("head2", c0, c1)

            def fn(dec=dec, key=key, nb=(c1 - c0) * B):
                pts, conf, _ = self.eng.dpt_head(dec, nb, self.hh, self.hw, 2)
                self.head2_out[key] = (pts, conf)
            self._graphed(key, fn, use_graphs)
            pts, conf = self.head2_out[key]
            pts, conf = pts.clone(), conf.clone()
            for j in range(c1 - c0):
                outs.append((pts[j * B:(j + 1) * B], conf[j * B:(j + 1) * B]))
        return outs

    def begin_outputs(self, n_steps):
        self._out_slabs, self._out_steps, self._out_i = None, n_steps, 0
        if self.mem is not None and self.mem.state is None and not self.length_keys_eager:
            per_step = 1 if self.model.single_graph_step else 2
            if n_steps * per_step > self.MAX_GRAPHS - 4:
                self.length_keys_eager = True
                self._drop_graphs(lambda k: k in self.length_keys)

    def _step_outputs(self, srcs):
        if getattr(self, "_out_steps", 0) <= 0 or self._out_i >= self._out_steps:
            return [torch.empty_like(t) for t in srcs]
        if self._out_slabs is None or len(self._out_slabs) != len(srcs):
            self._out_slabs = [t.new_empty((self._out_steps,) + tuple(t.shape)) for t in srcs]
        i, self._out_i = self._out_i, self._out_i + 1
        return [slab[i] for slab in self._out_slabs]

    def pair_copies(self, i):
        B = self.B
        pairs = [(self.feats[i * B:(i + 2) * B], self.featpair)]
        if self.feats_p is not None:
            st = self.feats_p.stride
            pairs.append((self.feats_p.data.view(-1)[i * st:(i + 2) * st], self.featpair_p.data.view(-1)[:2 * st]))
        return pairs

    def load_pair(self, i):
        ops.copy_multi(self.pair_copies(i))

    def _drop_graphs(self, pred):
        for k in [k for k in self.graphs if pred(k)]:
            self.graph_bytes -= self.graphs.pop(k)[1]

    MAX_GRAPHS = 16
    MAX_GRAPH_BYTES = 1 << 30

    def _graphed(self, key, fn, use_graphs, per_length=False):
        if per_length and use_graphs and not self.length_keys_eager and key not in self.graphs and key in self.seen \
                and len(self.graphs) >= self.MAX_GRAPHS - 2:
            self.length_keys_eager = True
            self._drop_graphs(lambda k: k in self.length_keys)
        if per_length:
            self.length_keys.add(key)
        if not use_graphs or (per_length and self.length_keys_eager):
            fn()
        elif key in self.graphs:
            self.graphs.move_to_end(key)
            self.graphs[key][0].replay()
        elif key in self.seen:
            if getattr(self, "_pool", None) is None or not self.graphs:
                self._pool = torch.cuda.graph_pool_handle()
            if getattr(self, "_capture_stream", None) is None:
                self._capture_stream = torch.cuda.Stream()
            before = torch.cuda.memory_allocated()
            g = torch.cuda.CUDAGraph()
            import gc
            gc_was = gc.isenabled()
            gc.disable()
            main = torch.cuda.current_stream()
            cap = self._capture_stream
            cap.wait_stream(main)
            try:
                with torch.cuda.stream(cap):
                    g.capture_begin(self._pool, capture_error_mode="thread_local")
                    try:
                        fn()
                    finally:
                        g.capture_end()
            finally:
                if gc_was:
                    gc.enable()
            main.wait_stream(cap)
            nbytes = max(0, torch.cuda.memory_allocated() - before)
            self.graphs[key] = (g, nbytes)
            self.graph_bytes += nbytes
            while len(self.graphs) > self.MAX_GRAPHS or (self.graph_bytes > self.MAX_GRAPH_BYTES and len(self.graphs) > 1):
                _, (old, ob) = self.graphs.popitem(last=False)
                self.graph_bytes -= ob
                del old
            g.replay()
        else:
            self.seen.add(key)
            fn()

    def _part1(self, first, has_next):
        eng, mem, B, P, E = self.eng, self.mem, self.B, self.P, self.E
        main = torch.cuda.current_stream()
        st = eng.side_streams()
        packed = self.packed_feats and self.model.packed_features and self.batched and self.feats_p is not None
        p1 = p2 = f1p = None
        if packed:
            p1, p2 = self.featpair_p.at(0), self.featpair_p.at(1)
        if first:
            if not self.batched:
                eng.encode_image(self.img_pair, out=self.featpair)
            f1, f1p = self.feat1, p1
        else:
            if not self.batched:
                ops.copy2d(self.feat2, E, self.feat1, E, B * P, E)
                ops.copy2d(self.feat_pre, E, self.feat2, E, B * P, E)
            mem.memory_read(self.k2, self.fuse, *(self.k2_aux if B == 1 else (None, None)), defer_attn=True,
                            out_packed=self.fuse_p if packed else None)
            f1 = self.fuse
            f1p = self.fuse_p if (packed and mem.wrote_packed) else None
        if has_next:
            st[3].wait_stream(main)
            with torch.cuda.stream(st[3]):
                eng.encode_image(self.img_next, out=self.feat_pre, tag="_pre")
        if eng.packed_attn and self.model.grouped_decoder:
            dec1, dec2 = eng.decoder_grouped(f1, self.feat2, B, self.nh, self.nw, f1p=f1p, f2p=p2 if f1p is not None else None)
            self.k2_aux = eng.encode_feat_keys_grouped(self.feat1, self.feat2, dec1[-1], dec2[-1], B * P, self.k1, self.k2,
                                                       feat1p=p1, feat2p=p2)
        else:
            if self.model.decoder_streams:
                dec1, dec2 = eng.decoder(f1, self.feat2, B, self.nh, self.nw, self.nh, self.nw, streams=st)
                st[2].wait_stream(main)
                with torch.cuda.stream(st[2]):
                    self.k2_aux = eng.encode_feat_key(self.feat2, dec2[-1], B * P, 2, self.k2, aux=True)
                eng.encode_feat_key(self.feat1, dec1[-1], B * P, 1, self.k1)
                main.wait_stream(st[2])
            else:
                dec1, dec2 = eng.decoder(f1, self.feat2, B, self.nh, self.nw, self.nh, self.nw, streams=None)
                self.k2_aux = eng.encode_feat_key(self.feat2, dec2[-1], B * P, 2, self.k2, aux=True)
                eng.encode_feat_key(self.feat1, dec1[-1], B * P, 1, self.k1)
        if not self.training and mem.sim_needed():
            mem.sim_scores(self.k1, to_host=self._scores_to_host and mem.state is not None)
        if has_next:
            main.wait_stream(st[3])
        self.dec = (dec1, dec2)
        self.dec2_hooks = [dec2[h] for h in self.model.cfg.hooks[1:]]

    def _part2(self):
        eng, mem, B = self.eng, self.mem, self.B
        dec1, dec2 = self.dec
        main = torch.cuda.current_stream()
        st = eng.side_streams()
        pts2 = conf2 = None
        if not self.defer2:
            st[2].wait_stream(main)
            with torch.cuda.stream(st[2]):
                pts2, conf2, _ = eng.dpt_head(dec2, B, self.hh, self.hw, 2)
        pts1, conf1, _ = eng.dpt_head(dec1, B, self.hh, self.hw, 1)
        if eng.cfg.use_feat:
            eng.encode_cur_value_feat(dec1[-1], self.v, self.k1,
                                      pos32=eng.positions(B, self.nh, self.nw)[1] if eng.cfg.mem_pos_enc else None)
        else:
            eng.encode_cur_value(pts1.swapaxes(1, 2) if self.swap else pts1, self.v, self.k1)
        mem.stage_write(self.k1, self.v)
        if not self.defer2:
            main.wait_stream(st[2])
        self.out = (pts1, conf1, pts2, conf2)

    def run(self, first, has_next, use_graphs, post_copies=()):
        mem = self.mem
        has_next = has_next and not self.batched
        gk = mem.graph_key()
        per_length = gk[0] not in ("s", "p")
        key = gk + (mem._cur, has_next, self.batched, self.defer2, self.model.grouped_decoder, self.model.packed_features)
        if not use_graphs and ops._prof is not None:
            ops._prof.step_begin()
        need_sim = not self.training and mem.sim_needed()
        if self.model.single_graph_step and use_graphs and ops._prof is None:
            if need_sim:
                mem.arm_score_poll()

            def whole():
                self._scores_to_host = need_sim
                try:
                    self._part1(first, has_next)
                finally:
                    self._scores_to_host = False
                if need_sim and mem.state is None:
                    mem.copy_scores_in_graph()
                self._part2()
            self._graphed(("whole", first, need_sim) + key, whole, use_graphs, per_length)
            if not first:
                mem.note_deferred_read()
        else:
            self._graphed(("first" if first else "step",) + key, lambda: self._part1(first, has_next), use_graphs, per_length)
            if not first:
                mem.note_deferred_read()
            if need_sim:
                mem.fetch_scores_async()
            self._graphed(("tail",) + key, self._part2, use_graphs, per_length)
        pts1, conf1, pts2, conf2 = self.out
        srcs = (pts1, conf1) + (() if pts2 is None else (pts2, conf2))
        outs = self._step_outputs(srcs)
        copies = list(zip(srcs, outs))
        copies += list(post_copies() if callable(post_copies) else post_copies)
        for c0 in range(0, len(copies), 8):
            ops.copy_multi(copies[c0:c0 + 8])
        res1 = {"pts3d": outs[0], "conf": outs[1]}
        res2 = {} if pts2 is None else {"pts3d": outs[2], "conf": outs[3]}
        if self.swap:
            res1 = {k: v.swapaxes(1, 2) for k, v in res1.items()}
            res2 = {k: v.swapaxes(1, 2) for k, v in res2.items()}
        if self.training:
            mem.commit()
            mem._push_state()
        else:
            mem.finish_staged(mem.sim_verdict() if need_sim else False)
        return res1, res2


class Spann3R(nn.Module):

    def __init__(self, dus3r_name="./checkpoints/DUSt3R_ViTLarge_BaseDecoder_512_dpt.pth",
                 use_feat=False, mem_pos_enc=False, memory_dropout=0.15, cfg: Spann3RConfig = None,
                 init_weights=True):
        super().__init__()
        self.use_feat = use_feat
        self.mem_pos_enc = mem_pos_enc
        self.mem_dropout = nn.Dropout(memory_dropout)
        ckpt = None
        if dus3r_name is not None and not os.path.isfile(dus3r_name):
            raise FileNotFoundError("DUSt3R checkpoint %r not found (pass dus3r_name=None to build without one)" % dus3r_name)
        if dus3r_name is not None:
            torch.serialization.add_safe_globals([argparse.Namespace])
            ckpt = torch.load(dus3r_name, map_location="cpu", weights_only=True)
            cfg = Spann3RConfig.from_ctor_string(ckpt["args"].model)
        self.cfg = cfg or FULL
        if mem_pos_enc != self.cfg.mem_pos_enc or use_feat != self.cfg.use_feat:
            import dataclasses
            self.cfg = dataclasses.replace(self.cfg, mem_pos_enc=bool(mem_pos_enc), use_feat=bool(use_feat))
        self.add_module("dust3r", _Dust3RFacade(self))
        self._params = _build_param_tree(self, param_spec(self.cfg))
        if init_weights:
            with torch.no_grad():
                for k, v in synth_state_dict(0, self.cfg).items():
                    if alias_of(k) is None:
                        self._params[k].copy_(v)
        if ckpt is not None:
            sd = {("dust3r." + k): v for k, v in ckpt["model"].items()}
            if not any(k.startswith("dust3r.dec_blocks2") for k in sd):
                for k, v in list(sd.items()):
                    if k.startswith("dust3r.dec_blocks."):
                        sd[k.replace("dust3r.dec_blocks.", "dust3r.dec_blocks2.")] = v
            own = self.state_dict()
            missing = [k for k in own if k.startswith("dust3r.") and k not in sd and alias_of(k) is None]
            unexpected = [k for k in sd if k not in own]
            print("<checkpoint %s: missing keys %s, unexpected keys %s>" % (dus3r_name, missing, unexpected))
            with torch.no_grad():
                for k, v in sd.items():
                    if k in own:
                        own[k].copy_(v)
                if not self.cfg.use_feat:
                    self._params["pos_patch_embed.proj.weight"].copy_(self._params["dust3r.patch_embed.proj.weight"])
                    self._params["pos_patch_embed.proj.bias"].copy_(self._params["dust3r.patch_embed.proj.bias"])
        self.precision = "fp32"
        self._engine = None
        self._engine_key = None
        self._pinned = None
        self._runners = {}
        self.use_graphs = True
        self.batch_encode = True
        self.defer_head2 = True
        self.grouped_decoder = True
        self.single_graph_step = True
        self.packed_features = True
        self.decoder_streams = True
        self.force_general = False
        self.max_runners = 4

    f16x3_range_guard = True

    def set_precision(self, precision):
        assert precision in ("fp32", "f32x3", "f32x6", "f16x3", "bf16")
        self.precision = precision
        return self

    def _versions(self):
        return tuple(p._version for p in self._params.values())

    @property
    def engine(self) -> Engine:
        if self._pinned is not None:
            return self._pinned.activate()
        dev = self._params["norm_q.weight"].device
        if dev.type != "cuda":
            raise RuntimeError("spann3r_amd.Spann3R runs on an MI355X only: call .to('cuda') first "
                               "(there is no CPU fallback; the CPU reference lives in oracle/ for tests)")
        key = (dev, self.precision, self._versions(), ops.WEIGHTS_EPOCH)
        if self._engine is None or self._engine_key != key:
            self._engine = Engine(self.cfg, dict(self._params), dev, self.precision)
            self._engine_key = key
            self._runners = {}
        return self._engine.activate()

    def _runner(self, key, make):
        run = self._runners.pop(key, None)
        if run is None:
            run = make()
            while len(self._runners) >= self.max_runners:
                self._runners.pop(next(iter(self._runners)))
        self._runners[key] = run
        return run

    @staticmethod
    def _true_shape(view):
        img = view["img"]
# ... 345 lines not shown
```

spann3r_amd/ops.py:

```python
import ctypes as C

import torch

from . import lib as L
from .lib import GemmDesc, F32, BF16, ACT_NONE, ACT_GELU, ACT_RELU


_prof = None


class Profiler:

    def __init__(self, blocker_ms=12.0):
        self.rec = []
        self.regions = []
        self.blocker_cycles = int(blocker_ms * 2.4e6)

    def step_begin(self):
        torch.cuda._sleep(self.blocker_cycles)

    def region_begin(self):
        return (self.begin(), len(self.rec))

    def region_end(self, key, e0, nbytes, info=None):
        e1 = torch.cuda.Event(enable_timing=True)
        e1.record()
        e0, n0 = e0
        self.regions.append((key, e0, e1, float(nbytes), info, len(self.rec) - n0))

    def region_summary(self):
        torch.cuda.synchronize()
        ov = getattr(self, "bracket_ms", 0.0)
        out = []
        for k, e0, e1, b, i, inner in self.regions:
            raw = e0.elapsed_time(e1)
            out.append(dict(key=k, ms=max(raw - ov * (inner + 1), 1e-4), raw_ms=raw, launches=inner, bytes=b, info=i))
        return out

    def begin(self):
        e = torch.cuda.Event(enable_timing=True)
        e.record()
        return e

    def end(self, key, e0, flops, nbytes):
        e1 = torch.cuda.Event(enable_timing=True)
        e1.record()
        self.rec.append((key, e0, e1, float(flops), float(nbytes)))

    def calibrate(self, n=40):
        ticks = torch.zeros(n, dtype=torch.int64, device="cuda")
        torch.cuda.synchronize()
        self.step_begin()
        ev = []
        for i in range(n):
            e0 = torch.cuda.Event(enable_timing=True)
            e1 = torch.cuda.Event(enable_timing=True)
            e0.record()
            L.check(L.load().sp3_spin(12000, ticks[i:].data_ptr(), L.stream_ptr()), "sp3_spin")
            e1.record()
            ev.append((e0, e1))
        torch.cuda.synchronize()
        dur_ms = (ticks.cpu().double() * 1e-5).tolist()
        t = sorted(a.elapsed_time(b) - d for (a, b), d in zip(ev, dur_ms))
        self.bracket_ms = max(t[len(t) // 2], 0.0)
        return self.bracket_ms

    def summary(self):
        torch.cuda.synchronize()
        agg = {}
        ov = getattr(self, "bracket_ms", 0.0)
        for key, e0, e1, fl, by in self.rec:
            a = agg.setdefault(key, dict(launches=0, ms=0.0, flops=0.0, bytes=0.0))
            a["launches"] += 1
            a["ms"] += max(e0.elapsed_time(e1) - ov, 1e-4)
            a["flops"] += fl
            a["bytes"] += by
        return agg


def set_profiler(p):
    global _prof
    _prof = p


_TILE_NAMES = {0: "32x32xk4", 1: "64x64", 2: "64x128", 3: "64x64xk4", 4: "32x64xk4", 18: "16x64xk4", 5: "128x128lds", 6: "128x64lds", 7: "112x64lds",
               8: "208x64lds", 9: "112x32lds", 10: "112x64lds2w", 11: "112x64lds8w", 12: "208x64lds8w", 13: "112x64wreg8",
               14: "112x64wreg4", 15: "208x64wreg8", 16: "112x64wreg4l6", 17: "112x64wreg8l4",
               20: "256x128pipe", 21: "128x128pipe", 22: "128x64pipe", 23: "64x64pipe", 24: "64x32pipe", 25: "32x32pipe",
               30: "lean-rope-k1024-48x64xk8", 31: "lean-rope-k768-32x32xk4", 32: "lean-packed-k1024-64x64xk8", 33: "lean-packed-k768-32x32xk4",
               34: "lean-stream-k1024-32x32xk8", 35: "lean-stream-k4096-32x32xk8r4", 36: "lean-stream-k768-48x32xk6",
               37: "lean-stream-k3072-48x32xk8", 38: "lean-stream-k1792-64x32xk7",
               39: "lean-stream-k1024-48x32xk8", 40: "lean-conv-16x16xk12", 41: "lean-conv-32x32xk8", 42: "lean-packed-splitA-k1792-64x32xk7", 43: "lean-score-k1024-32x32xk8", 44: "lean-softmax-pv-16x64xk8",
               45: "lean-prob-k1024-256x128", 46: "lean-prob-pv-256x128",
               50: "lean-rope-k1024-256x128", 51: "lean-rope-k1024-128x128", 52: "lean-rope-k768-128x128", 53: "lean-packed-k1024-256x128",
               54: "lean-packed-k1024-128x128", 55: "lean-packed-k768-128x128", 56: "lean-stream-k1024-128x64", 57: "lean-stream-k4096-128x64",
               58: "lean-stream-k768-128x64", 59: "lean-stream-k3072-128x64", 60: "lean-stream-k1792-128x64",
               61: "lean-stream-k1024-256x128", 62: "lean-stream-k4096-256x128", 63: "lean-rope-k768-256x128", 64: "lean-packed-k768-256x128", 65: "lean-rope-k768-128x64", 66: "lean-packed-splitA-k1792-128x128", 67: "lean-packed-splitA-k1792-256x128"}


import os as _os
import threading as _threading
PROF_SHAPES = _os.environ.get("SP3_PROF_SHAPES", "0")[:1] == "1"
LEAN = _os.environ.get("SP3_LEAN_GEMM", "1")[:1] != "0"

HEAD_LEVELS = _os.environ.get("SP3_HEAD_LEVELS", "1")[:1] != "0"
_held = None


def level_block_map(problems):
    start = [0]
    for tile, M, N in problems:
        bm = 16 if tile == 40 else 32
        start.append(start[-1] + 8 * ((M + bm - 1) // bm) * ((N // bm + 7) // 8))

    def f(w):
        p = max(i for i in range(len(problems)) if w >= start[i])
        tile, M, N = problems[p]
        bm = 16 if tile == 40 else 32
        mt = (M + bm - 1) // bm
        local = w - start[p]
        j = local >> 3
        return p, j % mt, (j // mt) * 8 + (local & 7)
    return start[-1], f


def level_order(problems):
    cost = [(K // 64) * (2 if tile == 40 else 3) for tile, K in problems]
    return sorted(range(len(problems)), key=lambda i: -cost[i])


class level:

    def __enter__(self):
        global _held
        assert _held is None
        _held = []
        return self

    def __exit__(self, et, ev, tb):
        global _held
        held, _held = _held, None
        if et is not None:
            return False
        conv = [x[0].loader == L.LOAD_CONV3X3 for x in held]
        if any(conv) and not all(conv):
            raise RuntimeError("ops.level(): small-map convolutions and other GEMMs do not share a launch")
        for i in range(0, len(held), 4):
            self._send(held[i:i + 4], any(conv))
        return False

    @staticmethod
    def _send(group, is_conv):
        if len(group) == 1:
            _gemm_launch(group[0][0], "sp3_gemm", group[0][1])
            return
        ds = [g[0] for g in group]
        arr = (C.POINTER(GemmDesc) * len(ds))(*[C.pointer(d) for d in ds])
        e0 = _prof.begin() if _prof is not None else None
        L.check(L.load().sp3_gemm_n(arr, len(ds), L.stream_ptr()), "sp3_gemm_n")
        if _prof is not None:
            tiles = (C.c_int * len(ds))()
            L.check(L.load().sp3_gemm_plan_n(arr, len(ds), tiles), "sp3_gemm_plan_n")
            cost = [_gemm_cost(d) for d in ds]
            a = ds[0]
            head = "<A%s,W%s,%s," % ("bf16" if a.a_bf16 else "f32", "f32" if a.wdtype == F32 else "bf16", group[0][1])
            if len(ds) == 2 and not is_conv:
                key = "gemm2" + head + _TILE_NAMES[tiles[0]] + ">"
            else:
                key = "gemm_n" + head + "+".join(sorted({_TILE_NAMES[t] for t in tiles})) + " x%d>" % len(ds)
            _prof.end(key, e0, sum(c[0] for c in cost), sum(c[1] for c in cost))


pair = level


def _gemm_cost(d):
    b = max(d.batch, 1)
    wsz = 4 if d.wdtype == F32 else 2
    asz, csz = (2 if d.a_bf16 else 4), (2 if d.out_bf16 else 4)
    a_elems = d.M * d.K if d.loader != L.LOAD_CONV3X3 else d.M * d.conv_stride * d.conv_stride * d.conv_C
    return 2.0 * d.M * d.N * d.K * b, b * (asz * a_elems + wsz * d.N * d.K + csz * d.M * d.N)


def _gemm_launch(d, what, loader_name):
    if _held is not None:
        _held.append((d, loader_name))
        return
    if _prof is None:
        L.check(L.load().sp3_gemm(C.byref(d), L.stream_ptr()), what)
        return
    e0 = _prof.begin()
    L.check(L.load().sp3_gemm(C.byref(d), L.stream_ptr()), what)
    flops, nbytes = _gemm_cost(d)
    tile = d.tile if d.tile >= 0 else L.load().sp3_gemm_plan(C.byref(d))
    tname = ("32x32xk4" if tile == 1 else "16x64xk4") if (d.loader == L.LOAD_SOFTMAX and tile < 30) else _TILE_NAMES[tile]
    key = "gemm<A%s,W%s,%s,%s>" % ("bf16" if d.a_bf16 else "f32", "f32" if d.wdtype == F32 else "bf16", loader_name, tname)
    if PROF_SHAPES:
        key += " %dx%dx%d x%d%s" % (d.M, d.N, d.K, max(d.batch, 1), " splitA" if d.A2 else "")
    _prof.end(key, e0, flops, nbytes)


def _timed(key, flops, nbytes, fn, *args):
    if _prof is None:
        return fn(*args)
    e0 = _prof.begin()
    r = fn(*args)
    _prof.end(key, e0, flops, nbytes)
    return r


def packed_shape(rows, K, dtype):
    KB, CH = (64, 16) if dtype == torch.bfloat16 else (32, 8)
    return ((rows + 15) // 16, (K + KB - 1) // KB, 2, 4, 16, CH // 2)


class PackedAct:

    def __init__(self, M, K, dtype, device, data=None):
        self.M, self.K, self.dtype = M, K, dtype
        self.data = torch.zeros(packed_shape(M, K, dtype), dtype=dtype, device=device) if data is None else data
        self.is_cuda = self.data.is_cuda

    @staticmethod
    def from_dense(x):
        M, K = x.shape
        KB, CH = (64, 16) if x.dtype == torch.bfloat16 else (32, 8)
        nb, nkb = (M + 15) // 16, (K + KB - 1) // KB
        pad = torch.zeros(nb * 16, nkb * KB, dtype=x.dtype, device=x.device)
        pad[:M, :K] = x
        return PackedAct(M, K, x.dtype, x.device, pad.view(nb, 16, nkb, 4, 2, CH // 2).permute(0, 2, 4, 3, 1, 5).contiguous())

    def to_dense(self):
        nb, nkb, _, _, _, ch2 = self.data.shape
        return self.data.permute(0, 4, 1, 3, 2, 5).reshape(nb * 16, nkb * 8 * ch2)[:self.M, :self.K]

    def data_ptr(self):
        return self.data.data_ptr()

    @staticmethod
    def group(G, M, K, dtype, device, alloc=None):
        KB = 64 if dtype == torch.bfloat16 else 32
        Mp, Kp = (M + 15) // 16 * 16, (K + KB - 1) // KB * KB
        t = PackedAct(G * Mp, K, dtype, device, data=None if alloc is None else alloc(packed_shape(G * Mp, K, dtype), dtype, zero=True))
        t.M, t.G, t.rows_pad, t.stride = M, G, Mp, Mp * Kp
        return t

    def at(self, g):
        v = PackedAct(self.M, self.K, self.dtype, self.data.device, data=self.data.view(-1)[g * self.stride:])
        v.stride = self.stride
        return v


class PackedWeight:

    def __init__(self, w2d, halves=False):
        N, K = w2d.shape
        self.N, self.K, self.dtype = N, K, w2d.dtype
        KB, CH = (64, 16) if w2d.dtype == torch.bfloat16 else (32, 8)
# ... 96 lines not shown
    if t.dtype == torch.float32:
        return F32
    if t.dtype == torch.bfloat16:
        return BF16
    raise TypeError("weights must be float32 or bfloat16, got %s" % t.dtype)


def _f32(t, name):
    if t is not None and (t.dtype != torch.float32 or not t.is_cuda):
        raise TypeError("%s must be a float32 CUDA(HIP) tensor" % name)


def _is_packed(t):
    return int(isinstance(t, PackedAct))


def _act(t, name):
    if not t.is_cuda or t.dtype not in (torch.float32, torch.bfloat16):
        raise TypeError("%s must be a float32/bfloat16 CUDA(HIP) tensor" % name)
    return int(t.dtype == torch.bfloat16)


def gemm(A, W, out, *, M, N, K, lda, ldc, bias=None, res1=None, ldr1=0, res2=None, ldr2=0, act=ACT_NONE, alpha=1.0,
         relu_in=False, tile=-1, batch=1, strideA=0, strideW=0, strideC=0, ldw=0,
         A2=None, lda2=0, K1=0, splitk=0, ln=None, stats_out=None, c2=None, sb=None, trace=None,
         sm_stats_out=None, softmax=None, plan_only=False, dyn_n=None):
    d = GemmDesc()
    d.a_bf16 = _act(A, "A")
    d.a_packed = _is_packed(A)
    d.out_packed = _is_packed(out)
    out_bf16 = out.dtype == torch.bfloat16
    _w(d, W)
    d.A, d.A2, d.C = A.data_ptr(), L.ptr(A2), out.data_ptr()
    d.bias, d.res1, d.res2 = L.ptr(bias), L.ptr(res1), L.ptr(res2)
    d.M, d.N, d.K, d.batch, d.K1 = M, N, K, batch, K1
    d.lda, d.lda2, d.ldw, d.ldc, d.ldr1, d.ldr2 = lda, lda2, ldw, ldc, ldr1, ldr2
    d.strideA, d.strideW, d.strideC = strideA, strideW, strideC
    d.alpha, d.act, d.out_bf16, d.relu_in = alpha, act, int(out_bf16), int(relu_in)
    d.loader, d.epi, d.tile = L.LOAD_PLAIN, L.EPI_PLAIN, tile
    if splitk >= 1:
        d.epi, d.splitk = L.EPI_PARTIAL, splitk
    _ln(d, ln)
    d.stats_out, d.c2 = L.ptr(stats_out), L.ptr(c2)
    d.trace = L.ptr(trace)
    d.sm_stats_out = L.ptr(sm_stats_out)
    d.dyn_n = L.ptr(dyn_n)
    if softmax is not None:
        st, thresh, zout = softmax
        d.loader, d.sm_stats, d.sm_nt, d.sm_thresh, d.sm_zout = L.LOAD_SOFTMAX, st.data_ptr(), (K + 31) // 32, float(thresh), L.ptr(zout)
    if sb:
        _group(d, batch, strideA, strideW, strideC, sb)
    if plan_only:
        return int(L.load().sp3_gemm_plan(C.byref(d)))
    _gemm_launch(d, "sp3_gemm", "softmax" if softmax is not None else "plain")
    return out


def reduce_ln(partial, splits, rows, C_, *, bias=None, res=None, ldres=0, x_out=None, ldx=0,
              ln1=None, out1=None, ld1=0, ln2=None, out2=None, ld2=0, eps=1e-6, act=ACT_NONE, res2=None, ldres2=0):
    d = L.ReduceLnDesc()
    d.partial, d.split_stride, d.splits, d.rows, d.C = partial.data_ptr(), rows * C_, splits, rows, C_
    d.bias, d.res, d.ldres = L.ptr(bias), L.ptr(res), ldres or C_
    d.x_out, d.ldx = L.ptr(x_out), ldx or C_
    d.act, d.res2, d.ldres2 = act, L.ptr(res2), ldres2 or C_
    if out1 is not None:
        d.g1, d.b1, d.out1, d.ld1, d.out1_bf16 = ln1[0].data_ptr(), ln1[1].data_ptr(), out1.data_ptr(), ld1 or C_, int(out1.dtype == torch.bfloat16)
        d.out1_packed = _is_packed(out1)
    if out2 is not None:
        d.g2, d.b2, d.out2, d.ld2, d.out2_bf16 = ln2[0].data_ptr(), ln2[1].data_ptr(), out2.data_ptr(), ld2 or C_, int(out2.dtype == torch.bfloat16)
        d.out2_packed = _is_packed(out2)
    d.eps = eps
    nln = (out1 is not None) + (out2 is not None)
    _timed("reduce_ln", (splits + 8.0 * nln) * rows * C_, 4.0 * rows * C_ * (splits + 2 + nln),
           lambda: L.check(L.load().sp3_reduce_ln(C.byref(d), L.stream_ptr()), "sp3_reduce_ln"))


def conv3x3(x, Wp, out, *, B, H, W_, Cin, Cout, stride=1, bias=None, res1=None, res2=None, act=ACT_NONE,
            relu_in=False, tile=-1, force_tile_kernel=False, splitk_ws=None, tile_px=None, res2_up=None):
    OH, OW = (H - 1) // stride + 1, (W_ - 1) // stride + 1
    if (tile < 0 and stride == 1 and isinstance(Wp, PackedWeight) and Wp.dtype == torch.bfloat16
            and Cin % 64 == 0 and Cout % 64 == 0 and Cin <= 768 and (force_tile_kernel or B * H * W_ >= 2048)):
        if res2_up is not None:
            raise ValueError("conv3x3: a half-resolution res2 is read by the lean small-map kernels only (B*H*W=%d)" % (B * H * W_))
        _act(x, "x")
        rbf = [t.dtype == torch.bfloat16 for t in (res1, res2) if t is not None]
        if rbf and (any(rbf) != all(rbf) or (any(rbf) and out.dtype != torch.bfloat16)):
            raise TypeError("conv3x3: residual maps must share one dtype (bf16 only next to a bf16 output)")
        oflag = int(out.dtype == torch.bfloat16) | (2 if any(rbf) else 0) | ({None: 0, "8x8": 1, "8x16": 2, "8x16n32": 3}[tile_px] << 2)
        _timed("conv3x3_tile", 2.0 * B * H * W_ * Cout * 9 * Cin,
               B * H * W_ * (x.element_size() * Cin + out.element_size() * Cout) + 2.0 * 9 * Cin * Cout,
               lambda: L.check(L.load().sp3_conv3x3_tile(
                   x.data_ptr(), int(x.dtype == torch.bfloat16), Wp.data_ptr(), L.ptr(bias), L.ptr(res1), L.ptr(res2),
                   out.data_ptr(), oflag, B, H, W_, Cin, Cout, int(relu_in), act,
                   L.stream_ptr()), "sp3_conv3x3_tile"))
        return out
    d = GemmDesc()
    d.a_bf16 = _act(x, "x")
    d.out_bf16 = int(out.dtype == torch.bfloat16)
    _w(d, Wp)
    M = B * OH * OW
    lean = -1
    if tile < 0 and isinstance(Wp, PackedWeight):
        p = GemmDesc()
        p.a_bf16, p.out_bf16 = d.a_bf16, d.out_bf16
        _w(p, Wp)
        p.A, p.C, p.bias, p.res1, p.res2 = x.data_ptr(), out.data_ptr(), L.ptr(bias), L.ptr(res1), L.ptr(res2)
        p.M, p.N, p.K, p.batch = M, Cout, 9 * Cin, 1
        p.lda, p.ldc, p.ldr1, p.ldr2 = Cin, Cout, Cout, Cout
        p.alpha, p.act, p.relu_in = 1.0, act, int(relu_in)
        p.loader, p.epi, p.tile = L.LOAD_CONV3X3, L.EPI_PLAIN, -1
        p.conv_H, p.conv_W, p.conv_C, p.conv_OH, p.conv_OW, p.conv_stride = H, W_, Cin, OH, OW, stride
        rbf = [t.dtype == torch.bfloat16 for t in (res1, res2) if t is not None]
        if rbf and any(rbf) != all(rbf):
            raise TypeError("conv3x3: residual maps must share one dtype")
        p.res_bf16 = int(any(rbf))
        if res2_up is not None:
            p.res2_up_H, p.res2_up_W = res2_up
        lean = L.load().sp3_gemm_plan(C.byref(p))
        if lean >= 30:
            _gemm_launch(p, "sp3_gemm(conv3x3)", "conv3x3")
            return out
    if res2_up is not None:
        raise ValueError("conv3x3: a half-resolution res2 is read by the lean small-map kernels only (B*H*W=%d)" % (B * H * W_))
    if any(t is not None and t.dtype == torch.bfloat16 for t in (res1, res2)):
        raise TypeError("conv3x3: bf16 residual maps are served by the lean small-map and the LDS-tiled kernels only "
                        "(B*H*W=%d, Cin=%d, Cout=%d, stride %d)" % (B * H * W_, Cin, Cout, stride))
    S = conv_splitk(M, Cout, 9 * Cin, Wp.dtype) if (splitk_ws is not None and tile < 0 and out.dtype == torch.float32) else 1
    if S > 1 and splitk_ws.numel() < S * M * Cout:
        raise ValueError("conv3x3: splitk_ws holds %d floats, needs %d" % (splitk_ws.numel(), S * M * Cout))
    d.A, d.C = x.data_ptr(), (splitk_ws if S > 1 else out).data_ptr()
    if S == 1:
        d.bias, d.res1, d.res2 = L.ptr(bias), L.ptr(res1), L.ptr(res2)
    d.M, d.N, d.K, d.batch = M, Cout, 9 * Cin, 1
    d.lda, d.ldc, d.ldr1, d.ldr2 = Cin, Cout, Cout, Cout
    d.alpha, d.act, d.relu_in = 1.0, (act if S == 1 else ACT_NONE), int(relu_in)
    d.loader, d.epi, d.tile = L.LOAD_CONV3X3, (L.EPI_PLAIN if S == 1 else L.EPI_PARTIAL), (tile if S == 1 else 0)
    d.splitk = S if S > 1 else 0
    d.conv_H, d.conv_W, d.conv_C, d.conv_OH, d.conv_OW, d.conv_stride = H, W_, Cin, OH, OW, stride
    global _held
    held, _held = _held, None
    try:
        _gemm_launch(d, "sp3_gemm(conv3x3)", "conv3x3")
    finally:
        _held = held
    if S > 1:
        reduce_ln(splitk_ws, S, M, Cout, bias=bias, res=res1, ldres=Cout, x_out=out, ldx=Cout, act=act, res2=res2, ldres2=Cout)
    return out


def conv3x3_takes_res2_up(Wp, map_dtype, B, H, W_):
    return LEAN and isinstance(Wp, PackedWeight) and Wp.dtype == torch.bfloat16 and map_dtype == torch.bfloat16 and B * H * W_ < 2048


def conv_splitk(M, N, K, wdtype):
    tiles = ((M + 31) // 32) * ((N + 31) // 32)
    nkb = K // (64 if wdtype == torch.bfloat16 else 32)
    s = 1
    while tiles * s * 2 <= 512 and nkb // (s * 2) >= 4 and s < 8:
        s *= 2
    return s


def conv_transpose_ks(x, Wp, out, *, B, H, W_, Cin, Cout, ks, bias=None, tile=-1):
    d = GemmDesc()
    d.a_bf16 = _act(x, "x")
    d.out_bf16 = int(out.dtype == torch.bfloat16)
    _w(d, Wp)
    d.A, d.C, d.bias = x.data_ptr(), out.data_ptr(), L.ptr(bias)
    d.M, d.N, d.K, d.batch = B * H * W_, ks * ks * Cout, Cin, 1
    d.lda, d.ldc = Cin, Cout
    d.alpha = 1.0
    d.loader, d.epi, d.tile = L.LOAD_PLAIN, L.EPI_PIXSHUF, tile
    d.ps_k, d.ps_H, d.ps_W, d.ps_C = ks, H, W_, Cout
    _gemm_launch(d, "sp3_gemm(conv_transpose)", "plain")
    return out


def proj_rope_vt(A, W, bias, out_qk, ldc, vt, vt_ld, *, M, N, K, lda, rope_cols, pos, cos, sin, tokens, heads, tile=-1,
                 qkv_packed=False, ln=None, batch=1, strideA=0, strideW=0, strideC=0, sb=None):
    d = GemmDesc()
    d.a_bf16 = _act(A, "A")
    d.a_packed = _is_packed(A)
    _w(d, W)
    d.A, d.C, d.bias = A.data_ptr(), L.ptr(out_qk), L.ptr(bias)
    d.M, d.N, d.K, d.batch = M, N, K, 1
    d.lda, d.ldc = lda, ldc
    d.alpha = 1.0
    d.loader, d.epi, d.tile = L.LOAD_PLAIN, L.EPI_ROPE_VT, tile
    d.rope_cos, d.rope_sin, d.pos, d.rope_cols = cos.data_ptr(), sin.data_ptr(), pos.data_ptr(), rope_cols
    d.vt, d.vt_ld, d.tokens, d.heads = L.ptr(vt), vt_ld, tokens, heads
    d.qkv_packed = int(qkv_packed)
    _ln(d, ln)
    if out_qk is None:
        d.C = vt.data_ptr()
    if batch > 1:
        _group(d, batch, strideA, strideW, strideC, sb)
    _gemm_launch(d, "sp3_gemm(rope_vt)", "plain")


def layernorm(x, gamma, beta, eps, out, *, rows, C_, ldx=None, ldo=None, transposed=False, dual=None, group_rows=0):
    _f32(x, "x")
    ldx = C_ if ldx is None else ldx
    ldo = C_ if ldo is None else ldo
    if dual is not None:
        assert dual.dtype == torch.bfloat16 and not transposed and not _is_packed(out)
        pad = getattr(dual, "rows_pad", (group_rows + 15) // 16 * 16)
        _timed("layernorm", 8.0 * rows * C_, rows * C_ * 10.0,
               lambda: L.check(L.load().sp3_layernorm_dual(x.data_ptr(), ldx, gamma.data_ptr(), beta.data_ptr(), eps, out.data_ptr(), ldo,
                                                           dual.data_ptr(), rows, C_, group_rows or rows, pad, L.stream_ptr()),
                               "sp3_layernorm_dual"))
        return out
    if _is_packed(out):
        _timed("layernorm", 8.0 * rows * C_, rows * C_ * 6.0,
               lambda: L.check(L.load().sp3_layernorm_packed(x.data_ptr(), ldx, gamma.data_ptr(), beta.data_ptr(), eps,
                                                             out.data_ptr(), int(out.dtype == torch.bfloat16), rows, C_,
                                                             L.stream_ptr()), "sp3_layernorm_packed"))
        return out
    fn = L.load().sp3_layernorm_t if transposed else L.load().sp3_layernorm
    _timed("layernorm_t" if transposed else "layernorm", 8.0 * rows * C_, rows * C_ * (4.0 + out.element_size()),
           lambda: L.check(fn(x.data_ptr(), ldx, gamma.data_ptr(), beta.data_ptr(), eps, out.data_ptr(), ldo,
                              int(out.dtype == torch.bfloat16), rows, C_, L.stream_ptr()), "sp3_layernorm"))
    return out


def rope_2d(tokens, positions, base, fwd):
    if tokens.dim() != 4:
        raise RuntimeError("tokens must have 4 dimensions")
    if positions.dim() != 3:
        raise RuntimeError("positions must have 3 dimensions")
    if tokens.size(0) != positions.size(0):
        raise RuntimeError("batch size differs between tokens & positions")
    if tokens.size(1) != positions.size(1):
        raise RuntimeError("seq_length differs between tokens & positions")
    if positions.size(2) != 2:
        raise RuntimeError("positions.shape[2] must be equal to 2")
    if tokens.is_cuda != positions.is_cuda:
        raise RuntimeError("tokens and positions are not on the same device")
    if not tokens.is_cuda:
        raise RuntimeError("spann3r_amd rope_2d is the MI355X kernel: tokens must be on the GPU (no CPU fallback)")
    if tokens.stride(3) != 1:
        raise RuntimeError("tokens are not contiguous")
    if not positions.is_contiguous() or positions.dtype != torch.int64:
        raise RuntimeError("positions are not contiguous int64")
    B, N, H, D = tokens.shape
    dt = wdtype_of(tokens)
    L.check(L.load().sp3_rope_2d(tokens.data_ptr(), dt, B, N, H, D, tokens.stride(0), tokens.stride(1), tokens.stride(2),
                                 positions.data_ptr(), float(base), float(fwd), L.stream_ptr()), "sp3_rope_2d")
    return tokens


def attention(q, sq, ldq, k, sk, ldk, vt, vt_ld, out, ldo, *, B, heads, Nq, Nk, scale):
    es = vt.element_size()
    _timed("attention<%s>" % ("f32" if es == 4 else "bf16"), 4.0 * B * heads * Nq * Nk * 64,
           B * heads * 64.0 * (es * (Nq + 2 * Nk) + 4 * Nq),
           lambda: L.check(L.load().sp3_attention_ex(q.data_ptr(), sq, ldq, k.data_ptr(), sk, ldk, vt.data_ptr(), vt_ld,
                                                     out.data_ptr(), ldo, int(out.dtype == torch.bfloat16), _is_packed(out),
                                                     B, heads, Nq, Nk, float(scale), (2 if (get_product_mode() == 1 and es == 4) else 3 if (get_product_mode() == 4 and es == 4) else wdtype_of(vt)),
                                                     L.stream_ptr()),
                           "sp3_attention"))
    return out


def attention_packed(qp, q_cols, q_col0, npad_q, kp, k_cols, k_col0, npad_k, vtp, out, ldo, *, B, heads, Nq, Nk, scale,
                     o_group=0, o_group_rows=0):
    _timed("attention_packed<bf16>", 4.0 * B * heads * Nq * Nk * 64, B * heads * 64.0 * (2 * (Nq + 2 * Nk) + 4 * Nq),
           lambda: L.check(L.load().sp3_attention_packed(qp.data_ptr(), q_cols, q_col0, npad_q, kp.data_ptr(), k_cols, k_col0,
                                                         npad_k, vtp.data_ptr(), out.data_ptr(), ldo,
                                                         int(out.dtype == torch.bfloat16), _is_packed(out), B, heads, Nq, Nk,
                                                         float(scale), o_group, o_group_rows, L.stream_ptr()),
                           "sp3_attention_packed"))
    return out


def attention_packed_qproj(xq, stats, Wq, ln_s, bias, pos, cos, sin, kp, k_cols, k_col0, npad_k, vtp, out, ldo, *, B, heads, Nq, Nk, scale,
                           o_group, o_group_rows, eps=1e-6, stats_group_stride=0, vec_group_stride=0):
    d = L.AttnQProjDesc()
    D = heads * 64
    d.x_packed, d.x_group_stride = xq.data_ptr(), getattr(xq, "stride", 0)
    d.ln_stats, d.stats_group_stride = stats.data_ptr(), stats_group_stride
    d.w_packed, d.w_group_stride = Wq.data_ptr(), getattr(Wq, "stride", 0)
    d.ln_s, d.bias, d.vec_group_stride = ln_s.data_ptr(), bias.data_ptr(), vec_group_stride
    d.pos, d.rope_cos, d.rope_sin, d.ln_eps, d.D = pos.data_ptr(), cos.data_ptr(), sin.data_ptr(), eps, D
    d.kp, d.k_cols, d.k_col0, d.npad_k, d.vtp = kp.data_ptr(), k_cols, k_col0, npad_k, vtp.data_ptr()
    d.out, d.ldo, d.out_bf16, d.out_packed = out.data_ptr(), ldo, int(out.dtype == torch.bfloat16), _is_packed(out)
    d.B, d.heads, d.Nq, d.Nk, d.scale, d.o_group, d.o_group_rows = B, heads, Nq, Nk, float(scale), o_group, o_group_rows
    _timed("attention_packed_qproj<bf16>", 4.0 * B * heads * Nq * Nk * 64 + 2.0 * B * Nq * D * D,
           B * heads * 64.0 * (2 * (2 * Nk) + 4 * Nq) + 2.0 * B * Nq * D + 2.0 * (B // max(o_group, 1)) * D * D,
           lambda: L.check(L.load().sp3_attention_packed_qproj(C.byref(d), L.stream_ptr()), "sp3_attention_packed_qproj"))
    return out


def softmax_thresh(S, P, *, ld, rows, M, Mpad, thresh, batch=1, strideS=0, packed=None, stride_packed=0):
    pbf = packed is not None and packed.dtype == torch.bfloat16
    _timed("softmax_thresh", 8.0 * batch * rows * M, (4.0 + (0.0 if P is None else 4.0) + (0.0 if packed is None else packed.element_size())) * batch * rows * M,
           lambda: L.check(L.load().sp3_softmax_thresh(S.data_ptr(), L.ptr(P), ld, strideS, rows, M, Mpad, float(thresh),
                                                       batch, L.ptr(packed), stride_packed, int(pbf), L.stream_ptr()), "sp3_softmax_thresh"))


def softmax_pack(S, packed, rowstat, *, ld, rows, M, thresh, batch=1, strideS=0, stride_packed=0):
    _timed("softmax_pack", 8.0 * batch * rows * M, (4.0 + packed.element_size()) * batch * rows * M,
           lambda: L.check(L.load().sp3_softmax_pack(S.data_ptr(), ld, strideS, rows, M, float(thresh), batch, packed.data_ptr(), stride_packed,
                                                     int(packed.dtype == torch.bfloat16), rowstat.data_ptr(), L.stream_ptr()), "sp3_softmax_pack"))


def colsum_accum(P, ld, rows, M, mem_attn):
    L.check(L.load().sp3_colsum_accum(P.data_ptr(), ld, rows, M, mem_attn.data_ptr(), L.stream_ptr()), "sp3_colsum_accum")
# ... 21 lines not shown
def colsum_softmax(S, ld, rows, M, rowz, thresh, mem_attn, mem_count=None, append_P=0):
    _timed("colsum_softmax", 4.0 * rows * M, 4.0 * rows * M,
           lambda: L.check(L.load().sp3_colsum_softmax(S.data_ptr(), ld, rows, M, rowz.data_ptr(), float(thresh), mem_attn.data_ptr(),
                                                       L.ptr(mem_count), append_P, L.stream_ptr()), "sp3_colsum_softmax"))


def bank_write(feat_k, feat_v, bank, M, P, C_, cap, norms, alpha, eps=1e-5, state=None):
    d = L.BankWriteDesc()
    d.state = L.ptr(state)
    d.feat_k, d.feat_v = feat_k.data_ptr(), feat_v.data_ptr()
    d.k_raw, d.v_raw, d.k_hat, d.v_hat_t = bank["k_raw"].data_ptr(), bank["v_raw"].data_ptr(), bank["k_hat"].data_ptr(), bank["v_hat_t"].data_ptr()
    d.s_bank, d.b_bank = bank["s_bank"].data_ptr(), bank["b_bank"].data_ptr()
    d.gamma_k, d.beta_k, d.gamma_v, d.beta_v, d.gamma_q, d.beta_q = [t.data_ptr() for t in norms]
    d.eps, d.alpha, d.M, d.P, d.C, d.cap, d.wdtype = eps, alpha, M, P, C_, cap, wdtype_of(bank["k_hat"])
    es = bank["k_hat"].element_size()
    _timed("bank_write", 20.0 * P * C_, P * C_ * (16.0 + 2 * es),
           lambda: L.check(L.load().sp3_bank_write(C.byref(d), L.stream_ptr()), "sp3_bank_write"))


def pack_stats(x, packed, stats, *, rows, C_, ldx=None):
    _f32(x, "x")
    L.check(L.load().sp3_pack_stats(x.data_ptr(), C_ if ldx is None else ldx, rows, C_, packed.data_ptr(),
                                    int(packed.dtype == torch.bfloat16), stats.data_ptr(), L.stream_ptr()), "sp3_pack_stats")


_pack_ws = {}


def _pack_colsum_ws(device, nby, nbx):
    ws = _pack_ws.get(str(device))
    need = nby * nbx * 64
    if ws is None or ws.numel() < need:
        ws = torch.empty(max(need, 1 << 18), device=device)
        _pack_ws[str(device)] = ws
    return ws


def pack_bf16(x2d, want=True, want_t=False, colsum=None, accumulate=False, act=0):
    rows, cols = x2d.shape
    _f32(x2d, "x")
    if x2d.stride(1) != 1:
        x2d = x2d.contiguous()
    alloc = lambda r, c: torch.empty(packed_shape(r, c, torch.bfloat16), dtype=torch.bfloat16, device=x2d.device)
    a = PackedAct(rows, cols, torch.bfloat16, x2d.device, data=alloc(rows, cols)) if want else None
    t = PackedAct(cols, rows, torch.bfloat16, x2d.device, data=alloc(cols, rows)) if want_t else None
    if act:
        assert colsum is None
        _timed("pack_bf16", 0.0, rows * cols * (4.0 + 2.0 * (bool(want) + bool(want_t))),
               lambda: L.check(L.load().sp3_pack_bf16_act(x2d.data_ptr(), x2d.stride(0), rows, cols, L.ptr(a), L.ptr(t), int(act), L.stream_ptr()), "sp3_pack_bf16_act"))
        return a, t
    if colsum is not None:
        pw = _pack_colsum_ws(x2d.device, (rows + 63) // 64, (cols + 63) // 64)
        _timed("pack_bf16", 0.0, rows * cols * (4.0 + 2.0 * (bool(want) + bool(want_t))),
               lambda: L.check(L.load().sp3_pack_bf16_colsum(x2d.data_ptr(), x2d.stride(0), rows, cols, L.ptr(a), L.ptr(t), colsum.data_ptr(), int(accumulate),
                                                             pw.data_ptr(), L.stream_ptr()), "sp3_pack_bf16_colsum"))
        return a, t
    _timed("pack_bf16", 0.0, rows * cols * (4.0 + 2.0 * (bool(want) + bool(want_t))),
           lambda: L.check(L.load().sp3_pack_bf16(x2d.data_ptr(), x2d.stride(0), rows, cols, L.ptr(a), L.ptr(t), L.stream_ptr()), "sp3_pack_bf16"))
    return a, t


def pack_bf16_conv3x3(x, stride, want=True, want_t=False, act=0):
    B, H, W_, C_ = x.shape
    _f32(x, "x")
    assert x.is_contiguous()
    OH, OW = (H - 1) // stride + 1, (W_ - 1) // stride + 1
    rows, cols = B * OH * OW, 9 * C_
    alloc = lambda r, c: torch.empty(packed_shape(r, c, torch.bfloat16), dtype=torch.bfloat16, device=x.device)
    a = PackedAct(rows, cols, torch.bfloat16, x.device, data=alloc(rows, cols)) if want else None
    t = PackedAct(cols, rows, torch.bfloat16, x.device, data=alloc(cols, rows)) if want_t else None
    _timed("pack_bf16_conv3x3", 0.0, rows * cols * 2.0 * (bool(want) + bool(want_t)) + x.numel() * 4.0,
           lambda: L.check(L.load().sp3_pack_bf16_conv3x3(x.data_ptr(), B, H, W_, C_, stride, int(act), L.ptr(a), L.ptr(t), L.stream_ptr()), "sp3_pack_bf16_conv3x3"))
    return a, t


def gather_packed_rows(src, dst, sel, n_sel, C_):
    L.check(L.load().sp3_gather_packed_rows(src.data_ptr(), dst.data_ptr(), sel.data_ptr(), n_sel, C_, src.element_size(),
                                            L.stream_ptr()), "sp3_gather_packed_rows")


def gather_packed_cols(src, dst, sel, n_sel, n_fill, C_, cap):
    L.check(L.load().sp3_gather_packed_cols(src.data_ptr(), dst.data_ptr(), sel.data_ptr(), n_sel, n_fill, C_, cap, src.element_size(),
                                            L.stream_ptr()), "sp3_gather_packed_cols")


def prob_merge(stats, scale, rows, M, cap, dyn_n=None):
    L.check(L.load().sp3_prob_merge(stats.data_ptr(), scale.data_ptr(), rows, M, cap, L.ptr(dyn_n), L.stream_ptr()), "sp3_prob_merge")


def colsum_prob(p_packed, scale, rows, M, cap, mem_attn, dyn_n=None):
    _timed("colsum_prob", 2.0 * rows * M, 2.0 * rows * M,
           lambda: L.check(L.load().sp3_colsum_prob(p_packed.data_ptr(), scale.data_ptr(), rows, M, cap, L.ptr(dyn_n), mem_attn.data_ptr(), L.stream_ptr()),
                           "sp3_colsum_prob"))


def bank_state_set(state, M, wm):
    L.check(L.load().sp3_bank_state_set(state.data_ptr(), int(M), int(wm), L.stream_ptr()), "sp3_bank_state_set")


def cos_sim_state(k, k_raw, Tmax, P, C_, state, score, scratch):
    assert scratch.numel() >= Tmax * P and scratch.dtype == torch.float32 and state.dtype == torch.int32
    L.check(L.load().sp3_cos_sim_state(k.data_ptr(), k_raw.data_ptr(), Tmax, P, C_, state.data_ptr(), scratch.data_ptr(), score.data_ptr(),
                                       L.stream_ptr()), "sp3_cos_sim_state")


def cos_sim(k, wm, T, P, C_, score, scratch):
    assert scratch.numel() >= T * P and scratch.dtype == torch.float32
    L.check(L.load().sp3_cos_sim(k.data_ptr(), wm.data_ptr(), T, P, C_, scratch.data_ptr(), score.data_ptr(), L.stream_ptr()),
            "sp3_cos_sim")


def mem_append(count, attn, M, P):
    L.check(L.load().sp3_mem_append(count.data_ptr(), attn.data_ptr(), M, P, L.stream_ptr()), "sp3_mem_append")


def prune_select(attn, count, M, protect, top_k, sel):
    L.check(L.load().sp3_prune_select(attn.data_ptr(), count.data_ptr(), M, float(protect), top_k, sel.data_ptr(),
                                      L.stream_ptr()), "sp3_prune_select")


def gather_rows(src, dst, sel, n_sel, C_):
    L.check(L.load().sp3_gather_rows(src.data_ptr(), dst.data_ptr(), sel.data_ptr(), n_sel, C_, src.element_size(),
                                     L.stream_ptr()), "sp3_gather_rows")


def gather_cols(src, ld_src, dst, ld_dst, sel, n_sel, n_fill, C_):
    L.check(L.load().sp3_gather_cols(src.data_ptr(), ld_src, dst.data_ptr(), ld_dst, sel.data_ptr(), n_sel, n_fill, C_,
                                     src.element_size(), L.stream_ptr()), "sp3_gather_cols")


def gather_1d(src, dst, sel, n_sel):
    L.check(L.load().sp3_gather_1d(src.data_ptr(), dst.data_ptr(), sel.data_ptr(), n_sel, L.stream_ptr()), "sp3_gather_1d")


def im2col_patch(img, out, *, B, C_, H, W_, p, strides):
    _f32(img, "img")
    sb, sc, sy, sx = strides
    L.check(L.load().sp3_im2col_patch(img.data_ptr(), sb, sc, sy, sx, B, C_, H, W_, p, out.data_ptr(),
                                      int(out.dtype == torch.bfloat16), _is_packed(out), L.stream_ptr()), "sp3_im2col_patch")
    return out


def upsample2x(x, out, *, B, H, W_, C_, outH=None, outW=None):
    outH = 2 * H if outH is None else outH
    outW = 2 * W_ if outW is None else outW
    if x.dtype != out.dtype or x.dtype not in (torch.float32, torch.bfloat16):
        raise TypeError("upsample2x: fp32 or bf16 maps, input and output alike")
    fn = L.load().sp3_upsample2x_bf16 if x.dtype == torch.bfloat16 else L.load().sp3_upsample2x
    _timed("upsample2x", 8.0 * B * outH * outW * C_, float(x.element_size()) * B * C_ * (H * W_ + outH * outW),
           lambda: L.check(fn(x.data_ptr(), out.data_ptr(), B, H, W_, C_, outH, outW, L.stream_ptr()), "sp3_upsample2x"))
    return out


def head_final(feat, w, b, pixels, C_, pts, conf, raw=None):
    fn = L.load().sp3_head_final_bf16 if feat.dtype == torch.bfloat16 else L.load().sp3_head_final
    _timed("head_final", 8.0 * pixels * C_, pixels * (float(feat.element_size()) * C_ + 16.0),
           lambda: L.check(fn(feat.data_ptr(), w.data_ptr(), b.data_ptr(), pixels, C_, pts.data_ptr(),
                              conf.data_ptr(), L.ptr(raw), L.stream_ptr()), "sp3_head_final"))


def fill(t, v):
    L.check(L.load().sp3_fill_f32(t.data_ptr(), float(v), t.numel(), L.stream_ptr()), "sp3_fill_f32")


def copy2d(src, lds, dst, ldd, rows, cols):
    L.check(L.load().sp3_copy2d_f32(src.data_ptr(), lds, dst.data_ptr(), ldd, rows, cols, L.stream_ptr()), "sp3_copy2d_f32")
```

Measured before the change: 640.2.

## Fuse bilinear upsampling into conv3x3 tiles and emit value patches from head

Adds an upsampling input mode to the wide conv3x3 kernel. It stages a half-resolution window in LDS and builds the doubled halo on the fly, and it can also read a half-resolution residual with bilinear taps in the epilogue. This removes the separate upsample2x passes and their full-resolution intermediates in the DPT head tail. The head's final kernel can also write the im2col patch operand for the value encoder directly, so the separate im2col pass is skipped. The cost is extra LDS per block, more ALU work in staging, and new code paths gated by an env knob.

Result: no change. 637.7, median of 6 (-0.4%).

```diff
diff --git a/include/spann3r_hip.h b/include/spann3r_hip.h
--- a/include/spann3r_hip.h
+++ b/include/spann3r_hip.h
@@ -177,6 +177,11 @@
 int sp3_conv3x3_tile(const void* x, int in_bf16, const void* w_packed, const float* bias, const float* res1,
                      const float* res2, void* out, int out_bf16, int B, int H, int W, int Cin, int Cout,
                      int relu_in, int act, void* stream);
+int sp3_conv3x3_tile_up(const void* x, int in_bf16, const void* w_packed, const float* bias, const float* res1,
+                        const float* res2, void* out, int out_bf16, int B, int H, int W, int Cin, int Cout,
+                        int relu_in, int act, int x_up_H, int x_up_W, int res2_up_H, int res2_up_W, void* stream);
+int sp3_conv3x3_tile_kind(int B, int H, int W, int Cin, int Cout, int want);
+int sp3_up2x_window(int n, int crop, int o, int t0, int len, int* i0, int* i1, float* l, float* h, int* first, int* count);
 int sp3_im2col_patch(const float* img, int64_t sb, int64_t sc, int64_t sy, int64_t sx, int B, int C, int H, int W,
                      int p, void* out, int out_bf16, int out_packed, void* stream);
 int sp3_upsample2x(const float* in, float* out, int B, int H, int W, int C, int outH, int outW, void* stream);
@@ -185,6 +190,8 @@
                    float* conf, float* raw, void* stream);
 int sp3_head_final_bf16(const void* feat, const float* w, const float* b, int64_t pixels, int C, float* pts, float* conf,
                         float* raw, void* stream);
+int sp3_head_final_bf16_patches(const void* feat, const float* w, const float* b, int B, int H, int W, int C, float* pts,
+                                float* conf, float* raw, void* col, int col_bf16, int p, int swap, void* stream);
 
 int sp3_preprocess_image(const uint8_t* src, int64_t src_row_stride, int crop_l, int crop_t, int H1, int W1,
                          const int32_t* hbounds, const int32_t* hcoef, int hksize, int W2,
diff --git a/spann3r_amd/csrc/common.h b/spann3r_amd/csrc/common.h
--- a/spann3r_amd/csrc/common.h
+++ b/spann3r_amd/csrc/common.h
@@ -87,18 +87,33 @@
   int p00, p01, p10, p11;
   float hy, ly, hx, lx;
 };
+struct Up2xAxis {
+  int i0, i1;
+  float h, l;
+};
+#ifdef __HIP_DEVICE_COMPILE__
+#define SP3_FMUL_RN(a, b) __fmul_rn(a, b)
+#define SP3_FMAF_RN(a, b, c) __fmaf_rn(a, b, c)
+#else
+#define SP3_FMUL_RN(a, b) ((float)(a) * (float)(b))
+#define SP3_FMAF_RN(a, b, c) __builtin_fmaf(a, b, c)
+#endif
+__host__ __device__ __forceinline__ float up2x_scale(int n) { return 2 * n > 1 ? (float)(n - 1) / (float)(2 * n - 1) : 0.f; }
+__host__ __device__ __forceinline__ Up2xAxis up2x_axis(int n, float s, int o) {
+  Up2xAxis a;
+  a.i0 = (int)SP3_FMUL_RN(s, (float)o);
+  a.i0 = a.i0 < n - 1 ? a.i0 : n - 1;
+  a.i1 = a.i0 < n - 1 ? a.i0 + 1 : a.i0;
+  a.l = SP3_FMAF_RN(s, (float)o, -(float)a.i0);
+  a.h = 1.f - a.l;
+  return a;
+}
+__host__ __device__ __forceinline__ Up2xAxis up2x_axis(int n, int o) { return up2x_axis(n, up2x_scale(n), o); }
 __device__ __forceinline__ Up2xTaps up2x_taps(int H, int W, int oy, int ox) {
-  const int OH = 2 * H, OW = 2 * W;
-  const float sh = OH > 1 ? (float)(H - 1) / (float)(OH - 1) : 0.f;
-  const float sw = OW > 1 ? (float)(W - 1) / (float)(OW - 1) : 0.f;
-  int y0 = (int)__fmul_rn(sh, (float)oy), x0 = (int)__fmul_rn(sw, (float)ox);
-  y0 = y0 < H - 1 ? y0 : H - 1;
-  x0 = x0 < W - 1 ? x0 : W - 1;
-  const int y1 = y0 < H - 1 ? y0 + 1 : y0, x1 = x0 < W - 1 ? x0 + 1 : x0;
+  const Up2xAxis y = up2x_axis(H, oy), x = up2x_axis(W, ox);
   Up2xTaps t;
-  t.ly = __fmaf_rn(sh, (float)oy, -(float)y0); t.lx = __fmaf_rn(sw, (float)ox, -(float)x0);
-  t.hy = 1.f - t.ly; t.hx = 1.f - t.lx;
-  t.p00 = y0 * W + x0; t.p01 = y0 * W + x1; t.p10 = y1 * W + x0; t.p11 = y1 * W + x1;
+  t.ly = y.l; t.hy = y.h; t.lx = x.l; t.hx = x.h;
+  t.p00 = y.i0 * W + x.i0; t.p01 = y.i0 * W + x.i1; t.p10 = y.i1 * W + x.i0; t.p11 = y.i1 * W + x.i1;
   return t;
 }
 __device__ __forceinline__ float up2x_mix(const Up2xTaps& t, float v00, float v01, float v10, float v11) {
diff --git a/spann3r_amd/csrc/conv.hip b/spann3r_amd/csrc/conv.hip
--- a/spann3r_amd/csrc/conv.hip
+++ b/spann3r_amd/csrc/conv.hip
@@ -16,6 +16,8 @@
   const void* x; const __bf16* w; const float* bias; const float* res1; const float* res2; void* out;
   int B, H, W, Cin, Cout, tiles_x, tiles_y, relu_in, act, out_bf16;
   int xcd_nb;
+  int up_H, up_W;
+  int res2_up_H, res2_up_W;
 };
 
 __device__ __forceinline__ bool conv_tile_of(const ConvArgs& a, int& t, int& nblk) {
@@ -211,12 +213,16 @@
 constexpr int CH = 128, PS = CH * 2 + 16;
 constexpr int MF = 8, DEPTH = 3;
 constexpr int HALO_BYTES = HP * PS;
-template <int NF> constexpr int lds_bytes() {
-  return HALO_BYTES > 4 * 64 * (16 * NF + 4) * 4 ? HALO_BYTES : 4 * 64 * (16 * NF + 4) * 4;
-}
-
-template <typename TIN, int NF = 4, int ABL = 0>
+constexpr int UP_WR = 7, UP_WC = 11, UP_PS = CH * 2;
+constexpr int UP_BYTES = UP_WR * UP_WC * UP_PS;
+template <int NF, bool UP = false> constexpr int lds_bytes() {
+  constexpr int stage = HALO_BYTES + (UP ? UP_BYTES : 0), slabs = 4 * 64 * (16 * NF + 4) * 4;
+  return stage > slabs ? stage : slabs;
+}
+
+template <typename TIN, int NF = 4, int ABL = 0, bool UP = false>
 __global__ __launch_bounds__(256, 2) void conv3x3_wide_kernel(const ConvArgs a) {
+  static_assert(!UP || sizeof(TIN) == 2, "the upsampling input mode reads bf16 maps");
   constexpr int BN = 16 * NF, SLAB_LD = BN + 4;
   extern __shared__ __attribute__((aligned(16))) char lds[];
   const int tid = threadIdx.x, lane = tid & 63, wave = tid >> 6, g = lane >> 4, r = lane & 15;
@@ -264,7 +270,7 @@
   constexpr int CHK = 16 / (int)sizeof(TIN);
   constexpr int CPP = CH / CHK;
   constexpr int PSTEP = 256 / CPP, NB = sizeof(TIN) == 4 ? 6 : 12;
-  const uint32_t img_bytes = (uint32_t)(a.H * a.W * Cin) * (uint32_t)sizeof(TIN);
+  const uint32_t img_bytes = (uint32_t)((UP ? a.up_H * a.up_W : a.H * a.W) * Cin) * (uint32_t)sizeof(TIN);
   const auto rsrc = __builtin_amdgcn_make_buffer_rsrc(
       const_cast<char*>(reinterpret_cast<const char*>(a.x)) + (int64_t)b * img_bytes, 0, (int)img_bytes, 0x00020000);
   const uint32_t xlane = (uint32_t)((tid % CPP) * CHK * sizeof(TIN));
@@ -308,11 +314,69 @@
       }
     }
   };
+  const float up_sh = UP ? __int_as_float(__builtin_amdgcn_readfirstlane(__float_as_int(up2x_scale(a.up_H)))) : 0.f;
+  const float up_sw = UP ? __int_as_float(__builtin_amdgcn_readfirstlane(__float_as_int(up2x_scale(a.up_W)))) : 0.f;
+  const int wy0 = UP ? __builtin_amdgcn_readfirstlane(up2x_axis(a.up_H, up_sh, y0 > 0 ? y0 - 1 : 0).i0) : 0;
+  const int wx0 = UP ? __builtin_amdgcn_readfirstlane(up2x_axis(a.up_W, up_sw, x0 > 0 ? x0 - 1 : 0).i0) : 0;
+  auto stage_up = [&](int c) {
+    char* win = lds + HALO_BYTES;
+    constexpr int NW = (UP_WR * UP_WC + PSTEP - 1) / PSTEP;
+    u32x4 wbuf[NW];
+#pragma unroll
+    for (int q = 0; q < NW; ++q) {
+      const int p = tid / CPP + q * PSTEP;
+      const int wr = p / UP_WC, sy = wy0 + wr, sx = wx0 + (p - wr * UP_WC);
+      const bool ok = p < UP_WR * UP_WC && sy < a.up_H && sx < a.up_W;
+      const uint32_t off = ok ? (uint32_t)((sy * a.up_W + sx) * Cin + c * CH) * 2u + xlane : 0x80000000u;
+      wbuf[q] = __builtin_amdgcn_raw_buffer_load_b128(rsrc, off, 0, 0);
+    }
+#pragma unroll
+    for (int q = 0; q < NW; ++q) {
+      const int p = tid / CPP + q * PSTEP;
+      if (p < UP_WR * UP_WC) *reinterpret_cast<u32x4*>(win + p * UP_PS + xlane) = wbuf[q];
+    }
+    __syncthreads();
+    const char* wsrc = win + xlane;
+#pragma unroll 1
+    for (int q = 0; q < NB; ++q) {
+      const int p = tid / CPP + q * PSTEP;
+      if (p >= HP) break;
+      const int hy = p / HW, hx = p - hy * HW;
+      const int iy = y0 + hy - 1, ix = x0 + hx - 1;
+      u32x4 o = u32x4{0u, 0u, 0u, 0u};
+      if (iy >= 0 && iy < a.H && ix >= 0 && ix < a.W) {
+        const Up2xAxis ay = up2x_axis(a.up_H, up_sh, iy), ax = up2x_axis(a.up_W, up_sw, ix);
+        Up2xTaps t;
+        t.hy = ay.h; t.ly = ay.l; t.hx = ax.h; t.lx = ax.l;
+        const int r0 = min(max(ay.i0 - wy0, 0), UP_WR - 1), r1 = min(max(ay.i1 - wy0, 0), UP_WR - 1);
+        const int c0 = min(max(ax.i0 - wx0, 0), UP_WC - 1), c1 = min(max(ax.i1 - wx0, 0), UP_WC - 1);
+        const u32x4 v00 = *reinterpret_cast<const u32x4*>(wsrc + (r0 * UP_WC + c0) * UP_PS), v01 = *reinterpret_cast<const u32x4*>(wsrc + (r0 * UP_WC + c1) * UP_PS);
+        const u32x4 v10 = *reinterpret_cast<const u32x4*>(wsrc + (r1 * UP_WC + c0) * UP_PS), v11 = *reinterpret_cast<const u32x4*>(wsrc + (r1 * UP_WC + c1) * UP_PS);
+#pragma unroll
+        for (int e = 0; e < 4; ++e) {
+          bf16x2 m;
+          m[0] = (__bf16)up2x_mix(t, __uint_as_float(v00[e] << 16), __uint_as_float(v01[e] << 16), __uint_as_float(v10[e] << 16), __uint_as_float(v11[e] << 16));
+          m[1] = (__bf16)up2x_mix(t, __uint_as_float(v00[e] & 0xffff0000u), __uint_as_float(v01[e] & 0xffff0000u),
+                                  __uint_as_float(v10[e] & 0xffff0000u), __uint_as_float(v11[e] & 0xffff0000u));
+          o[e] = __builtin_bit_cast(uint32_t, m);
+          if (a.relu_in) {
+            const uint32_t neg = o[e] & 0x80008000u;
+            o[e] &= ~((neg >> 15) * 0xffffu);
+          }
+        }
+      }
+      *reinterpret_cast<u32x4*>(hdst + p * PS) = o;
+    }
+  };
   for (int c = 0; c < nchunk; ++c) {
     if (c) __syncthreads();
-    for (int p0 = tid / CPP; p0 < HP; p0 += NB * PSTEP) {
-      issue(c, p0);
-      commit(p0);
+    if constexpr (UP) {
+      stage_up(c);
+    } else {
+      for (int p0 = tid / CPP; p0 < HP; p0 += NB * PSTEP) {
+        issue(c, p0);
+        commit(p0);
+      }
     }
     __syncthreads();
 
@@ -372,7 +436,16 @@
       const int64_t off = (((int64_t)b * a.H + oy) * a.W + ox) * a.Cout + gn;
       if (a.out_bf16 & 2) {
         if (a.res1) { const bf16x4 q = *reinterpret_cast<const bf16x4*>(reinterpret_cast<const __bf16*>(a.res1) + off); v.x += (float)q[0]; v.y += (float)q[1]; v.z += (float)q[2]; v.w += (float)q[3]; }
-        if (a.res2) { const bf16x4 q = *reinterpret_cast<const bf16x4*>(reinterpret_cast<const __bf16*>(a.res2) + off); v.x += (float)q[0]; v.y += (float)q[1]; v.z += (float)q[2]; v.w += (float)q[3]; }
+        if (a.res2 && a.res2_up_H) {
+          const Up2xTaps up = up2x_taps(a.res2_up_H, a.res2_up_W, oy, ox);
+          const __bf16* src = reinterpret_cast<const __bf16*>(a.res2) + (int64_t)b * a.res2_up_H * a.res2_up_W * a.Cout + gn;
+          const bf16x4 u00 = *reinterpret_cast<const bf16x4*>(src + (int64_t)up.p00 * a.Cout), u01 = *reinterpret_cast<const bf16x4*>(src + (int64_t)up.p01 * a.Cout);
+          const bf16x4 u10 = *reinterpret_cast<const bf16x4*>(src + (int64_t)up.p10 * a.Cout), u11 = *reinterpret_cast<const bf16x4*>(src + (int64_t)up.p11 * a.Cout);
+          v.x += (float)(__bf16)up2x_mix(up, (float)u00[0], (float)u01[0], (float)u10[0], (float)u11[0]);
+          v.y += (float)(__bf16)up2x_mix(up, (float)u00[1], (float)u01[1], (float)u10[1], (float)u11[1]);
+          v.z += (float)(__bf16)up2x_mix(up, (float)u00[2], (float)u01[2], (float)u10[2], (float)u11[2]);
+          v.w += (float)(__bf16)up2x_mix(up, (float)u00[3], (float)u01[3], (float)u10[3], (float)u11[3]);
+        } else if (a.res2) { const bf16x4 q = *reinterpret_cast<const bf16x4*>(reinterpret_cast<const __bf16*>(a.res2) + off); v.x += (float)q[0]; v.y += (float)q[1]; v.z += (float)q[2]; v.w += (float)q[3]; }
       } else {
         if (a.res1) { const float4 q = *reinterpret_cast<const float4*>(a.res1 + off); v.x += q.x; v.y += q.y; v.z += q.z; v.w += q.w; }
         if (a.res2) { const float4 q = *reinterpret_cast<const float4*>(a.res2 + off); v.x += q.x; v.y += q.y; v.z += q.z; v.w += q.w; }
@@ -391,9 +464,50 @@
 
 }
 
+static int conv_tile_nf(int want, int B, int H, int W, int Cin, int Cout) {
+  const int wtx = (W + wide::TW - 1) / wide::TW, wty = (H + wide::TH - 1) / wide::TH;
+  const int64_t wgs = (int64_t)wtx * wty * B * (Cout / 64);
+  const bool can = Cin % wide::CH == 0;
+  return want == 2 ? 4 : want == 3 ? 2 : (want == 0 && can) ? (wgs >= SP3_CONV_WIDE_MIN_WGS ? 4 : wgs >= 80 ? 2 : 0) : 0;
+}
+
+extern "C" int sp3_conv3x3_tile_kind(int B, int H, int W, int Cin, int Cout, int want) {
+  if (B <= 0 || H <= 0 || W <= 0 || Cin < 64 || Cin % 64 || Cout < 64 || Cout % 64 || want < 0 || want > 3) return -1;
+  if (want >= 2 && Cin % wide::CH) return -1;
+  return conv_tile_nf(want, B, H, W, Cin, Cout);
+}
+
+static int conv3x3_tile_impl(const char* who, const void* x, int in_bf16, const void* w_packed, const float* bias, const float* res1,
+                             const float* res2, void* out, int out_bf16, int B, int H, int W, int Cin, int Cout, int relu_in, int act,
+                             int x_up_H, int x_up_W, int res2_up_H, int res2_up_W, void* stream);
+
+extern "C" int sp3_up2x_window(int n, int crop, int o, int t0, int len, int* i0, int* i1, float* l, float* h, int* first, int* count) {
+  SP3_CHECK(n > 0 && crop > 0 && crop <= 2 * n && o >= 0 && o < crop && t0 >= 0 && t0 < crop && (len == wide::TH || len == wide::TW) && i0 && i1 && l && h && first && count,
+            "sp3_up2x_window: bad arguments");
+  const float s = up2x_scale(n);
+  const Up2xAxis a = up2x_axis(n, s, o);
+  *i0 = a.i0; *i1 = a.i1; *l = a.l; *h = a.h;
+  *first = up2x_axis(n, s, t0 > 0 ? t0 - 1 : 0).i0;
+  *count = up2x_axis(n, s, t0 + len < crop ? t0 + len : crop - 1).i1 - *first + 1;
+  return 0;
+}
+
 extern "C" int sp3_conv3x3_tile(const void* x, int in_bf16, const void* w_packed, const float* bias, const float* res1,
                                 const float* res2, void* out, int out_bf16, int B, int H, int W, int Cin, int Cout,
                                 int relu_in, int act, void* stream) {
+  return conv3x3_tile_impl("sp3_conv3x3_tile", x, in_bf16, w_packed, bias, res1, res2, out, out_bf16, B, H, W, Cin, Cout, relu_in, act, 0, 0, 0, 0, stream);
+}
+
+extern "C" int sp3_conv3x3_tile_up(const void* x, int in_bf16, const void* w_packed, const float* bias, const float* res1,
+                                   const float* res2, void* out, int out_bf16, int B, int H, int W, int Cin, int Cout,
+                                   int relu_in, int act, int x_up_H, int x_up_W, int res2_up_H, int res2_up_W, void* stream) {
+  return conv3x3_tile_impl("sp3_conv3x3_tile_up", x, in_bf16, w_packed, bias, res1, res2, out, out_bf16, B, H, W, Cin, Cout, relu_in, act,
+                           x_up_H, x_up_W, res2_up_H, res2_up_W, stream);
+}
+
+static int conv3x3_tile_impl(const char* who, const void* x, int in_bf16, const void* w_packed, const float* bias, const float* res1,
+                             const float* res2, void* out, int out_bf16, int B, int H, int W, int Cin, int Cout, int relu_in, int act,
+                             int x_up_H, int x_up_W, int res2_up_H, int res2_up_W, void* stream) {
   SP3_CHECK(x && w_packed && out, "sp3_conv3x3_tile: null pointer");
   SP3_CHECK(B > 0 && H > 0 && W > 0, "sp3_conv3x3_tile: bad shape");
   SP3_CHECK(Cin % 64 == 0 && Cin >= 64 && Cout % 64 == 0 && Cout >= 64, "sp3_conv3x3_tile: Cin=%d / Cout=%d must be multiples of 64", Cin, Cout);
@@ -405,16 +519,20 @@
   a.B = B; a.H = H; a.W = W; a.Cin = Cin; a.Cout = Cout;
   a.relu_in = relu_in; a.act = act; a.out_bf16 = out_bf16 & 3;
   a.xcd_nb = 0;
+  a.up_H = x_up_H; a.up_W = x_up_W; a.res2_up_H = res2 ? res2_up_H : 0; a.res2_up_W = res2 ? res2_up_W : 0;
   constexpr bool xcd_on = true;
   hipStream_t st = reinterpret_cast<hipStream_t>(stream);
   {
     const int want = (out_bf16 >> 2) & 3;
     const int wtx = (W + wide::TW - 1) / wide::TW, wty = (H + wide::TH - 1) / wide::TH;
-    const int64_t wgs = (int64_t)wtx * wty * B * (Cout / 64);
-    const bool can = Cin % wide::CH == 0;
-    SP3_CHECK(want < 2 || can, "sp3_conv3x3_tile: the 8 x 16 tile needs Cin %% 128 == 0 (Cin=%d)", Cin);
+    SP3_CHECK(want < 2 || Cin % wide::CH == 0, "sp3_conv3x3_tile: the 8 x 16 tile needs Cin %% 128 == 0 (Cin=%d)", Cin);
     SP3_CHECK((int64_t)H * W * Cin * (in_bf16 ? 2 : 4) < (1ll << 31), "sp3_conv3x3_tile: one image of the map must stay below 2 GiB");
-    const int nf = want == 2 ? 4 : want == 3 ? 2 : (want == 0 && can) ? (wgs >= SP3_CONV_WIDE_MIN_WGS ? 4 : wgs >= 80 ? 2 : 0) : 0;
+    const int nf = conv_tile_nf(want, B, H, W, Cin, Cout);
+    SP3_CHECK((x_up_H != 0) == (x_up_W != 0) && x_up_H >= 0 && (res2_up_H != 0) == (res2_up_W != 0) && res2_up_H >= 0, "%s: bad half-resolution size", who);
+    SP3_CHECK(!x_up_H || (nf && in_bf16), "%s: a half-resolution x is read by the 8 x 16 tiles on bf16 maps only (B=%d H=%d W=%d Cin=%d)", who, B, H, W, Cin);
+    SP3_CHECK(!x_up_H || (H <= 2 * x_up_H && W <= 2 * x_up_W), "%s: %d x %d is no crop of the doubled %d x %d map", who, H, W, x_up_H, x_up_W);
+    SP3_CHECK(!a.res2_up_H || (nf && (out_bf16 & 3) == 3), "%s: a half-resolution res2 is read by the 8 x 16 tiles with bf16 maps only (B=%d H=%d W=%d)", who, B, H, W);
+    SP3_CHECK(!a.res2_up_H || (H <= 2 * res2_up_H && W <= 2 * res2_up_W), "%s: %d x %d is no crop of the doubled %d x %d map", who, H, W, res2_up_H, res2_up_W);
     if (nf) {
       a.tiles_x = wtx; a.tiles_y = wty;
       dim3 grid(wtx * wty * B, Cout / (16 * nf));
@@ -430,8 +548,9 @@
         return 0;
       };
       int rc;
-      if (nf == 4) rc = in_bf16 ? launch(wide::conv3x3_wide_kernel<__bf16, 4>, wide::lds_bytes<4>()) : launch(wide::conv3x3_wide_kernel<float, 4>, wide::lds_bytes<4>());
-      else         rc = in_bf16 ? launch(wide::conv3x3_wide_kernel<__bf16, 2>, wide::lds_bytes<2>()) : launch(wide::conv3x3_wide_kernel<float, 2>, wide::lds_bytes<2>());
+      if (x_up_H)       rc = nf == 4 ? launch(wide::conv3x3_wide_kernel<__bf16, 4, 0, true>, wide::lds_bytes<4, true>()) : launch(wide::conv3x3_wide_kernel<__bf16, 2, 0, true>, wide::lds_bytes<2, true>());
+      else if (nf == 4) rc = in_bf16 ? launch(wide::conv3x3_wide_kernel<__bf16, 4>, wide::lds_bytes<4>()) : launch(wide::conv3x3_wide_kernel<float, 4>, wide::lds_bytes<4>());
+      else              rc = in_bf16 ? launch(wide::conv3x3_wide_kernel<__bf16, 2>, wide::lds_bytes<2>()) : launch(wide::conv3x3_wide_kernel<float, 2>, wide::lds_bytes<2>());
       if (rc) return rc;
       SP3_LAUNCH_CHECK("sp3_conv3x3_tile");
       return 0;
diff --git a/spann3r_amd/csrc/dpt.hip b/spann3r_amd/csrc/dpt.hip
--- a/spann3r_amd/csrc/dpt.hip
+++ b/spann3r_amd/csrc/dpt.hip
@@ -136,10 +136,14 @@
   }
 }
 
+struct PatchOut {
+  void* col;
+  int bf16, H, W, p, swap;
+};
 template <int LP, int PPT>
 __global__ __launch_bounds__(256) void head_final_bf16x8_kernel(const __bf16* __restrict__ feat, const float* __restrict__ w,
                                                                 const float* __restrict__ bias, int64_t pixels, float* __restrict__ pts,
-                                                                float* __restrict__ conf, float* __restrict__ raw) {
+                                                                float* __restrict__ conf, float* __restrict__ raw, const PatchOut po) {
   constexpr int C = 8 * LP, PPB = 256 / LP;
   const int li = threadIdx.x % LP, pl = threadIdx.x / LP;
   float wr[4][8];
@@ -177,8 +181,24 @@
       if (raw) *reinterpret_cast<float4*>(raw + pix * 4) = make_float4(X, Y, Z, Cc);
       const float d = sqrtf(X * X + Y * Y + Z * Z);
       const float sc = expm1f(d) / fmaxf(d, 1e-8f);
-      pts[pix * 3 + 0] = X * sc; pts[pix * 3 + 1] = Y * sc; pts[pix * 3 + 2] = Z * sc;
+      const float px = X * sc, py = Y * sc, pz = Z * sc;
+      pts[pix * 3 + 0] = px; pts[pix * 3 + 1] = py; pts[pix * 3 + 2] = pz;
       conf[pix] = 1.0f + expf(Cc);
+      if (po.col) {
+        const int hw = po.H * po.W, b = (int)(pix / hw), rem = (int)(pix - (int64_t)b * hw);
+        const int y = rem / po.W, x = rem - y * po.W;
+        const int iy = po.swap ? x : y, ix = po.swap ? y : x;
+        const int nw = (po.swap ? po.H : po.W) / po.p, nh = (po.swap ? po.W : po.H) / po.p;
+        const int ty = iy / po.p, tx = ix / po.p;
+        const int row = (b * nh + ty) * nw + tx, k = (iy - ty * po.p) * po.p + (ix - tx * po.p), pp = po.p * po.p;
+        const float v3[3] = {px, py, pz};
+#pragma unroll
+        for (int c = 0; c < 3; ++c) {
+          const int64_t o = packed_off(row, c * pp + k, 3 * pp, po.bf16 != 0);
+          if (po.bf16) reinterpret_cast<__bf16*>(po.col)[o] = (__bf16)v3[c];
+          else reinterpret_cast<float*>(po.col)[o] = v3[c];
+        }
+      }
     }
   }
 }
@@ -234,16 +254,34 @@
   return 0;
 }
 
+static int head_final_bf16_impl(const char* who, const void* feat, const float* w, const float* b, int64_t pixels, int C, float* pts,
+                                float* conf, float* raw, const PatchOut po, void* stream);
+
 extern "C" int sp3_head_final_bf16(const void* feat, const float* w, const float* b, int64_t pixels, int C, float* pts, float* conf,
                                    float* raw, void* stream) {
+  return head_final_bf16_impl("sp3_head_final_bf16", feat, w, b, pixels, C, pts, conf, raw, PatchOut{nullptr, 0, 0, 0, 0, 0}, stream);
+}
+
+extern "C" int sp3_head_final_bf16_patches(const void* feat, const float* w, const float* b, int B, int H, int W, int C, float* pts,
+                                           float* conf, float* raw, void* col, int col_bf16, int p, int swap, void* stream) {
+  SP3_CHECK(col && B > 0 && H > 0 && W > 0 && p > 0, "sp3_head_final_bf16_patches: bad arguments");
+  SP3_CHECK(H % p == 0 && W % p == 0, "Input image size (%d,%d) is not a multiple of patch size (%d)", H, W, p);
+  SP3_CHECK((int64_t)B * H * W < (1ll << 31), "sp3_head_final_bf16_patches: too many pixels");
+  return head_final_bf16_impl("sp3_head_final_bf16_patches", feat, w, b, (int64_t)B * H * W, C, pts, conf, raw,
+                              PatchOut{col, col_bf16, H, W, p, swap != 0}, stream);
+}
+
+static int head_final_bf16_impl(const char* who, const void* feat, const float* w, const float* b, int64_t pixels, int C, float* pts,
+                                float* conf, float* raw, const PatchOut po, void* stream) {
   SP3_CHECK(feat && w && b && pts && conf && pixels > 0 && C > 0 && C % 32 == 0, "sp3_head_final_bf16: bad arguments");
   if (C == 128 && (reinterpret_cast<uintptr_t>(feat) & 15) == 0 && (reinterpret_cast<uintptr_t>(w) & 15) == 0 && (!raw || (reinterpret_cast<uintptr_t>(raw) & 15) == 0)) {
     constexpr int LP = 16, PPT = 4, PPB = 256 / LP;
     hipLaunchKernelGGL((head_final_bf16x8_kernel<LP, PPT>), dim3((unsigned)((pixels + PPB * PPT - 1) / (PPB * PPT))), dim3(256), 0, ST(stream),
-                       reinterpret_cast<const __bf16*>(feat), w, b, pixels, pts, conf, raw);
+                       reinterpret_cast<const __bf16*>(feat), w, b, pixels, pts, conf, raw, po);
     SP3_LAUNCH_CHECK("sp3_head_final_bf16");
     return 0;
   }
+  SP3_CHECK(!po.col, "%s: the patch operand is written by the 128-channel kernel only (C=%d, 16-byte aligned maps)", who, C);
   const int64_t threads = pixels * 8;
   hipLaunchKernelGGL(head_final_kernel<__bf16>, dim3((unsigned)((threads + 255) / 256)), dim3(256), 0, ST(stream),
                      reinterpret_cast<const __bf16*>(feat), w, b, pixels, C, pts, conf, raw);
diff --git a/spann3r_amd/engine.py b/spann3r_amd/engine.py
--- a/spann3r_amd/engine.py
+++ b/spann3r_amd/engine.py
@@ -592,6 +592,9 @@
         t = self.ws("rcu_tmp" + tag, (B * H * W_, F), self.mdt)
         if not c1_done:
             self._rcu_c1(x, pre, B, H, W_, tag)
+        if extra_up is not None and ops.conv3x3_up_serves(w[pre + "c2.w"], self.mdt, B, H, W_, F, F):
+            ops.conv3x3_up(t, w[pre + "c2.w"], out, B=B, H=H, W_=W_, Cin=F, Cout=F, bias=w[pre + "c2.b"], res1=x, res2=extra_res, res2_up=extra_up)
+            return out
         ops.conv3x3(t, w[pre + "c2.w"], out, B=B, H=H, W_=W_, Cin=F, Cout=F, bias=w[pre + "c2.b"], res1=x, res2=extra_res,
                     splitk_ws=self._conv_ws(tag[:1]), res2_up=extra_up)
         return out
@@ -615,7 +618,10 @@
         ops.upsample2x(oc, up, B=B, H=H, W_=W_, C_=F, outH=OH, outW=OW)
         return up, OH, OW
 
-    def dpt_head(self, dec, B, nh, nw, num, want_raw=False):
+    def head_emits_patches(self):
+        return ops.HEAD_TAIL >= 2 and self.mdt == torch.bfloat16 and self.cfg.dpt_last == 128
+
+    def dpt_head(self, dec, B, nh, nw, num, want_raw=False, emit_patches=None):
         self.activate()
         cfg, w = self.cfg, self.w
         F, Lc = cfg.dpt_feat, cfg.dpt_last
@@ -673,24 +679,44 @@
             for i in range(4):
                 layer_rn(i)
         path, up, Hc, Wc = rn[3], None, h3, w3
+        H1, W1 = 2 * geo[0][0], 2 * geo[0][1]
+        tail_h0 = ops.conv3x3_up_serves(w[pre + "h0.w"], mdt, B, H1, W1, F, Lc, x_up=True)
+        tail_h2 = ops.conv3x3_up_serves(w[pre + "h2.w"], mdt, B, 2 * H1, 2 * W1, Lc, Lc, x_up=True)
         for j in range(4):
             Hn, Wn = geo[3 - j]
-            fold = lv and j < 3 and ops.conv3x3_takes_res2_up(w[refs[j + 1][0] + "u1c2.w"], mdt, B, *geo[2 - j])
+            if j < 3:
+                fold = lv and (ops.conv3x3_takes_res2_up(w[refs[j + 1][0] + "u1c2.w"], mdt, B, *geo[2 - j])
+                               or ops.conv3x3_up_serves(w[refs[j + 1][0] + "u1c2.w"], mdt, B, *geo[2 - j], F, F))
+            else:
+                fold = tail_h0
             nxt, OH_, OW_ = self._fusion(refs[j][0], B, Hn, Wn, path, rn[3 - j] if j else None, refs[j][1], crop=(nh, nw) if j == 0 else None,
                                          c1_done=lv, x0_up=up, fold_up=fold)
             path, up = nxt, ((Hn, Wn) if fold else None)
-        p1, H1, W1 = path, OH_, OW_
+        p1 = path
+        assert (H1, W1) == (OH_, OW_)
         a = self.ws("dpt%d_h0" % num, (B * H1 * W1, Lc), mdt)
-        ops.conv3x3(p1, w[pre + "h0.w"], a, B=B, H=H1, W_=W1, Cin=F, Cout=Lc, bias=w[pre + "h0.b"])
+        if tail_h0:
+            ops.conv3x3_up(p1, w[pre + "h0.w"], a, B=B, H=H1, W_=W1, Cin=F, Cout=Lc, bias=w[pre + "h0.b"], x_up=geo[0])
+        else:
+            ops.conv3x3(p1, w[pre + "h0.w"], a, B=B, H=H1, W_=W1, Cin=F, Cout=Lc, bias=w[pre + "h0.b"])
         OH, OW = 2 * H1, 2 * W1
-        u = self.ws("dpt%d_h0up" % num, (B * OH * OW, Lc), mdt)
-        ops.upsample2x(a, u, B=B, H=H1, W_=W1, C_=Lc)
         c = self.ws("dpt%d_h2" % num, (B * OH * OW, Lc), mdt)
-        ops.conv3x3(u, w[pre + "h2.w"], c, B=B, H=OH, W_=OW, Cin=Lc, Cout=Lc, bias=w[pre + "h2.b"], act=ACT_RELU)
+        if tail_h2:
+            ops.conv3x3_up(a, w[pre + "h2.w"], c, B=B, H=OH, W_=OW, Cin=Lc, Cout=Lc, bias=w[pre + "h2.b"], act=ACT_RELU, x_up=(H1, W1))
+        else:
+            u = self.ws("dpt%d_h0up" % num, (B * OH * OW, Lc), mdt)
+            ops.upsample2x(a, u, B=B, H=H1, W_=W1, C_=Lc)
+            ops.conv3x3(u, w[pre + "h2.w"], c, B=B, H=OH, W_=OW, Cin=Lc, Cout=Lc, bias=w[pre + "h2.b"], act=ACT_RELU)
         pts = self.ws("dpt_pts%d" % num, (B, OH, OW, 3))
         conf = self.ws("dpt_conf%d" % num, (B, OH, OW))
         raw = self.ws("dpt_raw%d" % num, (B, OH, OW, 4)) if want_raw else None
-        ops.head_final(c, w[pre + "h4.w"], w[pre + "h4.b"], B * OH * OW, Lc, pts, conf, raw)
+        if emit_patches is not None:
+            if emit_patches not in ("plain", "swap") or not self.head_emits_patches():
+                raise ValueError("dpt_head: emit_patches=%r is not served here (head_emits_patches() tells)" % (emit_patches,))
+            col = self.wsp("im2col_val", B * nh * nw, 3 * cfg.patch * cfg.patch)
+            ops.head_final_patches(c, w[pre + "h4.w"], w[pre + "h4.b"], B, OH, OW, Lc, pts, conf, raw, col, cfg.patch, emit_patches == "swap")
+        else:
+            ops.head_final(c, w[pre + "h4.w"], w[pre + "h4.b"], B * OH * OW, Lc, pts, conf, raw)
         return pts, conf, raw
 
     def encode_cur_value_feat(self, tok, out, res, pos32=None):
@@ -716,7 +742,7 @@
                  ln=ops.LnFold(stA, Cv, w["value_out.s"], 1e-6))
         return out
 
-    def encode_cur_value(self, pts3d, out, res):
+    def encode_cur_value(self, pts3d, out, res, col_ready=False):
         self.activate()
         cfg, w = self.cfg, self.w
         B, H, W_, _ = pts3d.shape
@@ -727,7 +753,8 @@
         _, pos32, zero_pos = self.positions(B, nh, nw)
         col = self.wsp("im2col_val", R, 3 * p * p)
         sb, sy, sx, sc = pts3d.stride()
-        ops.im2col_patch(pts3d, col, B=B, C_=3, H=H, W_=W_, p=p, strides=(sb, sc, sy, sx))
+        if not col_ready:
+            ops.im2col_patch(pts3d, col, B=B, C_=3, H=H, W_=W_, p=p, strides=(sb, sc, sy, sx))
         x, xp, st = self._vit(col, R, B, P, "pospatch", "val", cfg.val_depth, pos32 if cfg.mem_pos_enc else zero_pos, tag="_val")
         ops.gemm(xp, w["value_out.w"], out, M=R, N=E, K=E, lda=E, ldc=E, bias=w["value_out.b"], res1=res, ldr1=E,
                  ln=ops.LnFold(st, E, w["value_out.s"], 1e-6))
diff --git a/spann3r_amd/lib.py b/spann3r_amd/lib.py
--- a/spann3r_amd/lib.py
+++ b/spann3r_amd/lib.py
@@ -147,12 +147,18 @@
                          C.c_int, C.c_void_p, C.c_int, C.c_int, C.c_void_p],
     "sp3_conv3x3_tile": [C.c_void_p, C.c_int, C.c_void_p, C.c_void_p, C.c_void_p, C.c_void_p, C.c_void_p, C.c_int, C.c_int, C.c_int,
                          C.c_int, C.c_int, C.c_int, C.c_int, C.c_int, C.c_void_p],
+    "sp3_conv3x3_tile_up": [C.c_void_p, C.c_int, C.c_void_p, C.c_void_p, C.c_void_p, C.c_void_p, C.c_void_p, C.c_int, C.c_int, C.c_int,
+                            C.c_int, C.c_int, C.c_int, C.c_int, C.c_int, C.c_int, C.c_int, C.c_int, C.c_int, C.c_void_p],
+    "sp3_conv3x3_tile_kind": [C.c_int, C.c_int, C.c_int, C.c_int, C.c_int, C.c_int],
+    "sp3_up2x_window": [C.c_int, C.c_int, C.c_int, C.c_int, C.c_int, C.c_void_p, C.c_void_p, C.c_void_p, C.c_void_p, C.c_void_p, C.c_void_p],
     "sp3_upsample2x": [C.c_void_p, C.c_void_p, C.c_int, C.c_int, C.c_int, C.c_int, C.c_int, C.c_int, C.c_void_p],
     "sp3_head_final": [C.c_void_p, C.c_void_p, C.c_void_p, C.c_int64, C.c_int, C.c_void_p, C.c_void_p, C.c_void_p,
                        C.c_void_p],
     "sp3_upsample2x_bf16": [C.c_void_p, C.c_void_p, C.c_int, C.c_int, C.c_int, C.c_int, C.c_int, C.c_int, C.c_void_p],
     "sp3_head_final_bf16": [C.c_void_p, C.c_void_p, C.c_void_p, C.c_int64, C.c_int, C.c_void_p, C.c_void_p, C.c_void_p,
                             C.c_void_p],
+    "sp3_head_final_bf16_patches": [C.c_void_p, C.c_void_p, C.c_void_p, C.c_int, C.c_int, C.c_int, C.c_int, C.c_void_p, C.c_void_p, C.c_void_p,
+                                    C.c_void_p, C.c_int, C.c_int, C.c_int, C.c_void_p],
     "sp3_fill_f32": [C.c_void_p, C.c_float, C.c_int64, C.c_void_p],
     "sp3_cast_f32_to_bf16": [C.c_void_p, C.c_void_p, C.c_int64, C.c_void_p],
     "sp3_copy2d_f32": [C.c_void_p, C.c_int64, C.c_void_p, C.c_int64, C.c_int, C.c_int, C.c_void_p],
diff --git a/spann3r_amd/model.py b/spann3r_amd/model.py
--- a/spann3r_amd/model.py
+++ b/spann3r_amd/model.py
@@ -733,12 +733,13 @@
             st[2].wait_stream(main)
             with torch.cuda.stream(st[2]):
                 pts2, conf2, _ = eng.dpt_head(dec2, B, self.hh, self.hw, 2)
-        pts1, conf1, _ = eng.dpt_head(dec1, B, self.hh, self.hw, 1)
+        emit = not eng.cfg.use_feat and eng.head_emits_patches()
+        pts1, conf1, _ = eng.dpt_head(dec1, B, self.hh, self.hw, 1, emit_patches=("swap" if self.swap else "plain") if emit else None)
         if eng.cfg.use_feat:
             eng.encode_cur_value_feat(dec1[-1], self.v, self.k1,
                                       pos32=eng.positions(B, self.nh, self.nw)[1] if eng.cfg.mem_pos_enc else None)
         else:
-            eng.encode_cur_value(pts1.swapaxes(1, 2) if self.swap else pts1, self.v, self.k1)
+            eng.encode_cur_value(pts1.swapaxes(1, 2) if self.swap else pts1, self.v, self.k1, col_ready=emit)
         mem.stage_write(self.k1, self.v)
         if not self.defer2:
             main.wait_stream(st[2])
diff --git a/spann3r_amd/ops.py b/spann3r_amd/ops.py
--- a/spann3r_amd/ops.py
+++ b/spann3r_amd/ops.py
@@ -104,6 +104,7 @@
 LEAN = _os.environ.get("SP3_LEAN_GEMM", "1")[:1] != "0"
 
 HEAD_LEVELS = _os.environ.get("SP3_HEAD_LEVELS", "1")[:1] != "0"
+HEAD_TAIL = int(_os.environ.get("SP3_HEAD_TAIL", "1")[:1] or 1)
 _held = None
 
 
@@ -506,6 +507,31 @@
     return LEAN and isinstance(Wp, PackedWeight) and Wp.dtype == torch.bfloat16 and map_dtype == torch.bfloat16 and B * H * W_ < 2048
 
 
+def conv3x3_up_serves(Wp, map_dtype, B, H, W_, Cin, Cout, x_up=False):
+    return (HEAD_TAIL >= (2 if x_up else 1) and isinstance(Wp, PackedWeight) and Wp.dtype == torch.bfloat16 and map_dtype == torch.bfloat16 and B * H * W_ >= 2048
+            and Cin % 64 == 0 and Cout % 64 == 0 and Cin <= 768 and L.load().sp3_conv3x3_tile_kind(B, H, W_, Cin, Cout, 0) > 0)
+
+
+def conv3x3_up(x, Wp, out, *, B, H, W_, Cin, Cout, bias=None, res1=None, res2=None, act=ACT_NONE, relu_in=False, tile_px=None,
+               x_up=None, res2_up=None):
+    if not (isinstance(Wp, PackedWeight) and Wp.dtype == torch.bfloat16):
+        raise TypeError("conv3x3_up: bf16 packed weights only")
+    _act(x, "x")
+    rbf = [t.dtype == torch.bfloat16 for t in (res1, res2) if t is not None]
+    if rbf and (any(rbf) != all(rbf) or (any(rbf) and out.dtype != torch.bfloat16)):
+        raise TypeError("conv3x3_up: residual maps must share one dtype (bf16 only next to a bf16 output)")
+    oflag = int(out.dtype == torch.bfloat16) | (2 if any(rbf) else 0) | ({None: 0, "8x8": 1, "8x16": 2, "8x16n32": 3}[tile_px] << 2)
+    xh, xw = x_up or (0, 0)
+    rh, rw = res2_up or (0, 0)
+    _timed("conv3x3_tile", 2.0 * B * H * W_ * Cout * 9 * Cin,
+           B * (x.element_size() * Cin * (xh * xw if x_up else H * W_) + out.element_size() * Cout * H * W_) + 2.0 * 9 * Cin * Cout,
+           lambda: L.check(L.load().sp3_conv3x3_tile_up(
+               x.data_ptr(), int(x.dtype == torch.bfloat16), Wp.data_ptr(), L.ptr(bias), L.ptr(res1), L.ptr(res2),
+               out.data_ptr(), oflag, B, H, W_, Cin, Cout, int(relu_in), act, xh, xw, rh, rw,
+               L.stream_ptr()), "sp3_conv3x3_tile_up"))
+    return out
+
+
 def conv_splitk(M, N, K, wdtype):
     tiles = ((M + 31) // 32) * ((N + 31) // 32)
     nkb = K // (64 if wdtype == torch.bfloat16 else 32)
@@ -833,6 +859,15 @@
     return out
 
 
+def head_final_patches(feat, w, b, B, H, W_, C_, pts, conf, raw, col, p, swap):
+    if feat.dtype != torch.bfloat16 or not _is_packed(col):
+        raise TypeError("head_final_patches: bf16 feature map and a packed patch operand")
+    _timed("head_final", 8.0 * B * H * W_ * C_, B * H * W_ * (2.0 * C_ + 16.0 + 3.0 * col.data.element_size()),
+           lambda: L.check(L.load().sp3_head_final_bf16_patches(feat.data_ptr(), w.data_ptr(), b.data_ptr(), B, H, W_, C_, pts.data_ptr(),
+                                                                conf.data_ptr(), L.ptr(raw), col.data_ptr(), int(col.dtype == torch.bfloat16),
+                                                                p, int(swap), L.stream_ptr()), "sp3_head_final_bf16_patches"))
+
+
 def head_final(feat, w, b, pixels, C_, pts, conf, raw=None):
     fn = L.load().sp3_head_final_bf16 if feat.dtype == torch.bfloat16 else L.load().sp3_head_final
     _timed("head_final", 8.0 * pixels * C_, pixels * (float(feat.element_size()) * C_ + 16.0),
```
